# weixiaopassking/GS-LIVM

Hardware: AMD Instinct MI355X
Metric: rasterizer fwd+bwd Mpixels/s @1920x1080, 2000000 Gaussians (ms_per_step = ms/frame) (higher is better)
Workload: dtype f32; 1 GPU; C3: 2000000 Gaussians, 1920x1080, SH degree 0, 1 view per GPU per step, fwd+bwd + Adam step; view_threads=1, camera=one fixed view, near_entries=0, parallelism=view-parallel x1, adam_in_step=True, optimizer=one-kernel tail: activation chain rule + Adam + next activations (HIP), loss=seeded

## Files before the change

### gs-livm_amd/_capi.py

```python
import ctypes as C
import os

import torch

_HERE = os.path.dirname(os.path.abspath(__file__))
LIB_PATH = os.environ.get("GSR_LIB", os.path.join(_HERE, "libgsraster_hip.so"))

ALLOC_FN = C.CFUNCTYPE(C.c_void_p, C.c_void_p, C.c_size_t)


class GeometryView(C.Structure):
    _fields_ = [(n, C.c_void_p) for n in
                ("depths", "radii", "splats", "cov3D", "tiles_touched", "point_offsets", "clamped", "depth_order",
                 "num_rendered", "gpack")]


class BinningView(C.Structure):
    _fields_ = [("point_list", C.c_void_p)]


class ImageView(C.Structure):
    _fields_ = [(n, C.c_void_p) for n in ("ranges", "final_T", "n_contrib", "quad_last", "ranges_far")]


class MailboxEvent(C.Structure):
    _fields_ = [("count", C.c_uint), ("ticket_expected", C.c_uint32), ("ticket_seen_before_query", C.c_uint32),
                ("elapsed_us", C.c_double), ("ticket_seen_after_query", C.c_uint32), ("first_query_result", C.c_int),
                ("visible_at_query", C.c_int), ("queries", C.c_uint), ("longest_query_us", C.c_double),
                ("longest_poll_gap_us", C.c_double)]


class NumRendered(int):

    def __new__(cls, exact, key):
        obj = super().__new__(cls, exact)
        obj.key = int(key)
        return obj


def _key(R):
    return int(getattr(R, "key", R))


_lib = None

EXPORTS = ("gsr_forward", "gsr_backward", "gsr_backward_depth", "gsr_mark_visible", "gsr_geometry_bytes", "gsr_image_bytes",
           "gsr_binning_bytes", "gsr_geometry_view_of", "gsr_binning_view_of", "gsr_image_view_of",
           "gsr_higher_msb", "gsr_last_error", "gsr_abi_version", "gsr_kernel_count", "gsr_kernel_name",
           "gsr_profile_enable", "gsr_profile_enable_only", "gsr_profile_read", "gsr_mailbox_slow_path_hits", "gsr_activate", "gsr_activate_backward", "gsr_adam_step",
           "gsr_photometric_loss", "gsr_photometric_loss_workspace", "gsr_init_gaussians", "gsr_ply_row_floats",
           "gsr_pack_ply_rows", "gsr_model_step", "gsr_set_reference_rects", "gsr_reference_rects",
           "gsr_last_num_rendered", "gsr_set_binning_capacity_hint", "gsr_speculative_forwards",
           "gsr_speculation_overflows", "gsr_emit_guard_trips", "gsr_mailbox_slow_path_last", "gsr_set_near_far", "gsr_near_far",
           "gsr_last_near_far", "gsr_set_near_far_hints", "gsr_near_far_forwards", "gsr_set_far_speculation",
           "gsr_last_far_skipped", "gsr_far_skips", "gsr_far_skip_misses", "gsr_async_far_frames",
           "gsr_near_budget_scale", "gsr_near_budget_feedback", "gsr_near_far_pause", "gsr_set_near_far_thread",
           "gsr_set_reference_rects_thread", "gsr_async_outcomes_pending", "gsr_async_outcomes_lost",
           "gsr_frame_note_misses", "gsr_similarity_loss", "gsr_similarity_loss_workspace")


def lib():
    global _lib
    if _lib is not None:
        return _lib
    if not os.path.exists(LIB_PATH):
        raise RuntimeError(
            "libgsraster_hip.so not built: run `python gs-livm_amd/build.py` (needs hipcc). "
            "gs_livm_amd has no CPU fallback.")
    L = C.CDLL(LIB_PATH)
    vp, ci, cf, sz = C.c_void_p, C.c_int, C.c_float, C.c_size_t
    L.gsr_forward.restype = ci
    L.gsr_forward.argtypes = [ALLOC_FN, vp, ALLOC_FN, vp, ALLOC_FN, vp, ci, ci, ci, vp, ci, ci, vp, vp, vp, vp, vp, cf,
                              vp, vp, vp, vp, vp, cf, cf, ci, vp, vp, vp, vp, ci, vp]
    L.gsr_backward.restype = ci
    L.gsr_backward.argtypes = [ci, ci, ci, ci, vp, ci, ci, vp, vp, vp, vp, cf, vp, vp, vp, vp, vp, cf, cf, vp, vp, vp,
                               vp, vp, vp, vp, vp, vp, vp, vp, vp, vp, vp, vp, ci, vp]
    L.gsr_backward_depth.restype = ci
    L.gsr_backward_depth.argtypes = L.gsr_backward.argtypes[:25] + [vp] + L.gsr_backward.argtypes[25:34] + [vp, ci, vp]
    L.gsr_mark_visible.restype = ci
    L.gsr_mark_visible.argtypes = [ci, vp, vp, vp, vp, vp]
    for n in ("gsr_geometry_bytes", "gsr_binning_bytes"):
        getattr(L, n).restype = sz
        getattr(L, n).argtypes = [ci]
    L.gsr_image_bytes.restype = sz
    L.gsr_image_bytes.argtypes = [ci, ci]
    L.gsr_geometry_view_of.argtypes = [vp, ci, C.POINTER(GeometryView)]
    L.gsr_binning_view_of.argtypes = [vp, ci, C.POINTER(BinningView)]
    L.gsr_image_view_of.argtypes = [vp, ci, ci, C.POINTER(ImageView)]
    L.gsr_higher_msb.restype = C.c_uint32
    L.gsr_higher_msb.argtypes = [C.c_uint32]
    L.gsr_last_error.restype = C.c_char_p
    L.gsr_abi_version.restype = ci
    L.gsr_kernel_count.restype = ci
    L.gsr_kernel_name.restype = C.c_char_p
    L.gsr_kernel_name.argtypes = [ci]
    L.gsr_profile_enable.argtypes = [ci]
    L.gsr_profile_enable_only.argtypes = [C.POINTER(ci), ci]
    L.gsr_set_reference_rects.restype = ci
    L.gsr_set_reference_rects.argtypes = [ci]
    L.gsr_reference_rects.restype = ci
    L.gsr_reference_rects.argtypes = []
    L.gsr_last_num_rendered.restype = ci
    L.gsr_last_num_rendered.argtypes = []
    L.gsr_set_binning_capacity_hint.restype = C.c_longlong
    L.gsr_set_binning_capacity_hint.argtypes = [C.c_longlong]
    for n in ("gsr_speculative_forwards", "gsr_speculation_overflows", "gsr_emit_guard_trips"):
        getattr(L, n).restype = C.c_ulonglong
        getattr(L, n).argtypes = []
    L.gsr_set_near_far.restype = ci
    L.gsr_set_near_far.argtypes = [ci]
    L.gsr_near_far.restype = ci
    L.gsr_near_far.argtypes = []
    L.gsr_last_near_far.restype = ci
    L.gsr_last_near_far.argtypes = [C.POINTER(C.c_uint), C.POINTER(C.c_uint)]
    L.gsr_set_near_far_hints.restype = None
    L.gsr_set_near_far_hints.argtypes = [C.c_longlong, C.c_longlong]
    L.gsr_near_far_forwards.restype = C.c_ulonglong
    L.gsr_near_far_forwards.argtypes = []
    L.gsr_set_far_speculation.restype = ci
    L.gsr_set_far_speculation.argtypes = [ci]
    L.gsr_last_far_skipped.restype = ci
    L.gsr_last_far_skipped.argtypes = []
    L.gsr_near_budget_scale.restype = C.c_uint
    L.gsr_near_budget_scale.argtypes = []
    L.gsr_near_budget_feedback.restype = C.c_uint
    L.gsr_near_budget_feedback.argtypes = [C.c_uint, C.c_uint, C.c_uint]
    L.gsr_near_far_pause.restype = ci
    L.gsr_near_far_pause.argtypes = [ci]
    for n in ("gsr_far_skips", "gsr_far_skip_misses", "gsr_async_far_frames", "gsr_async_outcomes_lost",
              "gsr_frame_note_misses", "gsr_similarity_loss", "gsr_similarity_loss_workspace"):
        getattr(L, n).restype = C.c_ulonglong
        getattr(L, n).argtypes = []
    for n in ("gsr_set_near_far_thread", "gsr_set_reference_rects_thread"):
        getattr(L, n).restype = ci
        getattr(L, n).argtypes = [ci]
    L.gsr_async_outcomes_pending.restype = ci
    L.gsr_async_outcomes_pending.argtypes = []
    L.gsr_mailbox_slow_path_last.restype = ci
    L.gsr_mailbox_slow_path_last.argtypes = [C.POINTER(MailboxEvent)]
    L.gsr_mailbox_slow_path_hits.restype = C.c_ulonglong
    L.gsr_mailbox_slow_path_hits.argtypes = []
    L.gsr_profile_read.restype = ci
    L.gsr_profile_read.argtypes = [ci, C.POINTER(C.c_double), C.POINTER(ci)]
    L.gsr_activate.restype = ci
    L.gsr_activate.argtypes = [ci, ci] + [vp] * 9 + [vp]
    L.gsr_activate_backward.restype = ci
    L.gsr_activate_backward.argtypes = [ci, ci] + [vp] * 12 + [vp]
    L.gsr_photometric_loss_workspace.restype = sz
    L.gsr_photometric_loss_workspace.argtypes = [ci, ci, ci]
    L.gsr_photometric_loss.restype = ci
    L.gsr_photometric_loss.argtypes = [ci, ci, ci, vp, vp, C.POINTER(cf), cf, vp, vp, vp, sz, vp]
    L.gsr_similarity_loss_workspace.restype = sz
    L.gsr_similarity_loss_workspace.argtypes = [ci, ci]
    L.gsr_similarity_loss.restype = ci
    L.gsr_similarity_loss.argtypes = [ci, ci, ci, vp, vp, vp, vp, cf, vp, vp, vp, ci, vp, sz, vp]
    L.gsr_init_gaussians.restype = ci
    L.gsr_init_gaussians.argtypes = [ci, ci, vp, vp, vp, cf] + [vp] * 6 + [vp]
    L.gsr_ply_row_floats.restype = sz
    L.gsr_ply_row_floats.argtypes = [ci]
    L.gsr_pack_ply_rows.restype = ci
    L.gsr_pack_ply_rows.argtypes = [ci, ci] + [vp] * 7 + [vp]
    L.gsr_model_step.restype = ci
    L.gsr_model_step.argtypes = [ci, ci, C.POINTER(vp), C.POINTER(vp), C.POINTER(vp)] + [vp] * 9 + \
        [C.POINTER(cf), C.c_double, C.c_double, C.c_double, ci, vp]
    L.gsr_adam_step.restype = ci
    L.gsr_adam_step.argtypes = [ci, C.POINTER(vp), C.POINTER(vp), C.POINTER(vp), C.POINTER(vp), C.POINTER(sz),
                                C.POINTER(cf), C.c_double, C.c_double, C.c_double, ci, ci, vp]
    _lib = L
    return L


class GsrError(RuntimeError):
    pass


def _check(code):
    if code < 0:
        raise GsrError("libgsraster_hip error %d: %s" % (code, lib().gsr_last_error().decode()))
    return code


def _ptr(t):
    if t is None or t.numel() == 0:
        return None
    assert t.is_cuda and t.is_contiguous(), "expects contiguous device tensors"
    return C.c_void_p(t.data_ptr())


def _stream():
    return C.c_void_p(torch.cuda.current_stream().cuda_stream)


class _Blob:

    def __init__(self, device):
        self.device = device
        self.tensor = torch.empty(0, dtype=torch.uint8, device=device)
        self.fn = ALLOC_FN(self._alloc)

    def _alloc(self, _ctx, nbytes):
        try:
            self.tensor = torch.empty(int(nbytes), dtype=torch.uint8, device=self.device)
            return self.tensor.data_ptr()
        except Exception:
            return None


def rasterize_forward(background, means3D, colors, opacity, scales, rotations, scale_modifier, cov3D_precomp,
                      viewmatrix, projmatrix, tan_fovx, tan_fovy, image_height, image_width, sh, degree, campos,
                      prefiltered=False, debug=False, radii_out=True):
    if means3D.dim() != 2 or means3D.size(1) != 3:
        raise ValueError("means3D must have dimensions (num_points, 3)")
    dev = means3D.device
    P, H, W = int(means3D.size(0)), int(image_height), int(image_width)
    f32 = dict(dtype=torch.float32, device=dev)
    out_color = torch.empty((3, H, W), **f32)
    out_depth = torch.empty((1, H, W), **f32)
    out_acc = torch.empty((1, H, W), **f32)
    radii = torch.empty((P,), dtype=torch.int32, device=dev)
    gb, bb, ib = _Blob(dev), _Blob(dev), _Blob(dev)
    M = int(sh.size(1)) if (sh is not None and sh.numel() != 0) else 0
    L = lib()
    R = _check(L.gsr_forward(gb.fn, None, bb.fn, None, ib.fn, None, P, int(degree), M, _ptr(background), W, H,
                             _ptr(means3D), _ptr(sh), _ptr(colors), _ptr(opacity), _ptr(scales),
                             float(scale_modifier), _ptr(rotations), _ptr(cov3D_precomp), _ptr(viewmatrix),
                             _ptr(projmatrix), _ptr(campos), float(tan_fovx), float(tan_fovy), int(bool(prefiltered)),
                             _ptr(out_color), _ptr(out_depth), _ptr(out_acc), _ptr(radii) if radii_out else None,
                             int(bool(debug)), _stream()))
    R = NumRendered(L.gsr_last_num_rendered() if P else 0, R)
    return R, out_color, out_depth, out_acc, radii, gb.tensor, bb.tensor, ib.tensor


def rasterize_backward(background, means3D, radii, colors, scales, rotations, scale_modifier, cov3D_precomp,
                       viewmatrix, projmatrix, tan_fovx, tan_fovy, dL_dout_color, dL_dout_acc, sh, degree, campos,
                       geomBuffer, R, binningBuffer, imageBuffer, debug=False, return_conic=False, want_cov3D=True,
                       grad_depth=None):
    dev = means3D.device
    P = int(means3D.size(0))
    H, W = int(dL_dout_color.size(1)), int(dL_dout_color.size(2))
    M = int(sh.size(1)) if (sh is not None and sh.numel() != 0) else 0
    f32 = dict(dtype=torch.float32, device=dev)
    mk = torch.zeros if P == 0 else torch.empty
    dL_dmeans3D = mk((P, 3), **f32)
    dL_dmeans2D = mk((P, 3), **f32)
    dL_dcolors = mk((P, 3), **f32)
    dL_dconic = mk((P, 2, 2), **f32)
    dL_dopacity = mk((P, 1), **f32)
    dL_dcov3D = mk((P, 6), **f32) if want_cov3D else None
    dL_dsh = mk((P, M, 3), **f32)
    dL_dscales = mk((P, 3), **f32)
    dL_drotations = mk((P, 4), **f32)
    dL_ddepths = mk((P,), **f32) if grad_depth is not None else None
    if P != 0 and grad_depth is not None:
        dpix = dL_dout_color.contiguous()
        dacc = dL_dout_acc.contiguous()
        if grad_depth.dtype != torch.float32 or grad_depth.device != dev or grad_depth.numel() != H * W:
            raise ValueError("grad_depth must be a float32 tensor of H*W elements on the device of means3D")
        ddep = grad_depth.contiguous()
        _check(lib().gsr_backward_depth(P, int(degree), M, _key(R), _ptr(background), W, H, _ptr(means3D), _ptr(sh),
                                        _ptr(colors), _ptr(scales), float(scale_modifier), _ptr(rotations),
                                        _ptr(cov3D_precomp), _ptr(viewmatrix), _ptr(projmatrix), _ptr(campos),
                                        float(tan_fovx), float(tan_fovy), _ptr(radii), _ptr(geomBuffer),
                                        _ptr(binningBuffer), _ptr(imageBuffer), _ptr(dpix), _ptr(dacc), _ptr(ddep),
                                        _ptr(dL_dmeans2D), _ptr(dL_dconic), _ptr(dL_dopacity), _ptr(dL_dcolors),
                                        _ptr(dL_dmeans3D), _ptr(dL_dcov3D), _ptr(dL_dsh), _ptr(dL_dscales),
                                        _ptr(dL_drotations), _ptr(dL_ddepths), int(bool(debug)), _stream()))
    elif P != 0:
        dpix = dL_dout_color.contiguous()
        dacc = dL_dout_acc.contiguous()
        _check(lib().gsr_backward(P, int(degree), M, _key(R), _ptr(background), W, H, _ptr(means3D), _ptr(sh),
                                  _ptr(colors), _ptr(scales), float(scale_modifier), _ptr(rotations),
                                  _ptr(cov3D_precomp), _ptr(viewmatrix), _ptr(projmatrix), _ptr(campos),
                                  float(tan_fovx), float(tan_fovy), _ptr(radii), _ptr(geomBuffer),
                                  _ptr(binningBuffer), _ptr(imageBuffer), _ptr(dpix), _ptr(dacc), _ptr(dL_dmeans2D),
                                  _ptr(dL_dconic), _ptr(dL_dopacity), _ptr(dL_dcolors), _ptr(dL_dmeans3D),
                                  _ptr(dL_dcov3D), _ptr(dL_dsh), _ptr(dL_dscales), _ptr(dL_drotations),
                                  int(bool(debug)), _stream()))
    out = (dL_dmeans2D, dL_dcolors, dL_dopacity, dL_dmeans3D, dL_dcov3D, dL_dsh, dL_dscales, dL_drotations)
    if return_conic:
        out = out + (dL_dconic,)
    return out + (dL_ddepths,) if grad_depth is not None else out


def last_num_rendered():
    return int(lib().gsr_last_num_rendered())


def set_binning_capacity_hint(capacity):
    return int(lib().gsr_set_binning_capacity_hint(-1 if capacity is None else int(capacity)))


def speculation_stats():
    L = lib()
    return dict(speculative_forwards=int(L.gsr_speculative_forwards()), overflows=int(L.gsr_speculation_overflows()),
                near_far_forwards=int(L.gsr_near_far_forwards()), far_skips=int(L.gsr_far_skips()),
                far_skip_misses=int(L.gsr_far_skip_misses()), async_far_frames=int(L.gsr_async_far_frames()),
                async_outcomes_lost=int(L.gsr_async_outcomes_lost()), frame_note_misses=int(L.gsr_frame_note_misses()),
                near_budget_scale_q8=int(L.gsr_near_budget_scale()),
                mailbox_slow_path_hits=int(L.gsr_mailbox_slow_path_hits()))


def emit_guard_trips():
    return int(lib().gsr_emit_guard_trips())


def mailbox_slow_path_last():
    ev = MailboxEvent()
    _check(lib().gsr_mailbox_slow_path_last(C.byref(ev)))
    return {n: getattr(ev, n) for n, _ in MailboxEvent._fields_}


def set_near_far(on):
    return bool(lib().gsr_set_near_far(int(bool(on))))


def set_near_far_thread(mode):
    prev = int(lib().gsr_set_near_far_thread(-1 if mode is None else int(bool(mode))))
    return None if prev < 0 else bool(prev)


def async_outcomes_pending():
    return int(lib().gsr_async_outcomes_pending())


def set_near_far_hints(near_entries_per_tile=None, far_capacity=None):
    lib().gsr_set_near_far_hints(-1 if near_entries_per_tile is None else int(near_entries_per_tile),
                                 -1 if far_capacity is None else int(far_capacity))


def set_far_speculation(mode):
    return int(lib().gsr_set_far_speculation(-1 if mode is None else int(bool(mode))))


def last_far_skipped():
    return bool(lib().gsr_last_far_skipped())


def last_near_far():
    a, b = C.c_uint(0), C.c_uint(0)
    split = bool(lib().gsr_last_near_far(C.byref(a), C.byref(b)))
    return split, int(a.value), int(b.value)


def set_reference_rects(on):
    return bool(lib().gsr_set_reference_rects(int(bool(on))))


def set_reference_rects_thread(mode):
    prev = int(lib().gsr_set_reference_rects_thread(-1 if mode is None else int(bool(mode))))
    return None if prev < 0 else bool(prev)


def reference_rects():
    return bool(lib().gsr_reference_rects())


def mark_visible(means3D, viewmatrix, projmatrix):
    P = int(means3D.size(0))
    present = torch.zeros((P,), dtype=torch.bool, device=means3D.device)
    if P:
        _check(lib().gsr_mark_visible(P, _ptr(means3D), _ptr(viewmatrix), _ptr(projmatrix),
                                      C.c_void_p(present.data_ptr()), _stream()))
    return present


def _sub(blob, ptr, count, dtype):
    if not ptr or count == 0:
        return None
    off = int(ptr) - blob.data_ptr()
    nbytes = count * torch.empty((), dtype=dtype).element_size()
    return blob[off:off + nbytes].view(dtype)


def state_views(geomBuffer, binningBuffer, imageBuffer, P, R, W, H):
    L = lib()
    gv, bv, iv = GeometryView(), BinningView(), ImageView()
    T = ((W + 15) // 16) * ((H + 15) // 16)
    out = {}
    if P:
        _check(L.gsr_geometry_view_of(_ptr(geomBuffer), P, C.byref(gv)))
        splats = _sub(geomBuffer, gv.splats, P * 12, torch.float32).view(P, 12)
        gpack = _sub(geomBuffer, gv.gpack, P * 2, torch.int32).view(P, 2)
        out.update(depths=splats[:, 9],
                   radii=_sub(geomBuffer, gv.radii, P, torch.int32),
                   splats=splats,
                   cov3D=_sub(geomBuffer, gv.cov3D, P * 6, torch.float32).view(P, 6),
                   tiles_touched=gpack[:, 0],
                   point_offsets=_sub(geomBuffer, gv.point_offsets, P, torch.int32),
                   clamped=_sub(geomBuffer, gv.clamped, P, torch.uint8),
                   depth_order=_sub(geomBuffer, gv.depth_order, P, torch.int32))
        _check(L.gsr_image_view_of(_ptr(imageBuffer), W, H, C.byref(iv)))
        out.update(ranges=_sub(imageBuffer, iv.ranges, T * 2, torch.int32).view(T, 2),
                   final_T=_sub(imageBuffer, iv.final_T, W * H, torch.float32).view(H, W),
                   n_contrib=_sub(imageBuffer, iv.n_contrib, W * H, torch.int32).view(H, W),
                   quad_last=_sub(imageBuffer, iv.quad_last, T * 4, torch.int32).view(T, 4))
        counters = _sub(geomBuffer, gv.num_rendered, 16, torch.int32).cpu().tolist()
        split = counters[12] == 1
        exact = counters[6] + counters[8] if split else counters[0]
        out.update(num_rendered=exact, near_far=split, counters=counters)
        key = _key(R)
        if exact:
            _check(L.gsr_binning_view_of(_ptr(binningBuffer), key, C.byref(bv)))
            raw = _sub(binningBuffer, bv.point_list, key, torch.int32)
            ra = out["ranges"].long()
            rb = _sub(imageBuffer, iv.ranges_far, T * 2, torch.int32).view(T, 2).long()
            seg_start = torch.stack([ra[:, 0], rb[:, 0]], 1).reshape(-1)
            seg_len = torch.stack([ra[:, 1] - ra[:, 0], rb[:, 1] - rb[:, 0]], 1).reshape(-1)
            total = int(seg_len.sum())
            excl = torch.cumsum(seg_len, 0) - seg_len
            idx = torch.repeat_interleave(seg_start - excl, seg_len) + torch.arange(total, device=ra.device)
            point_list = raw[idx]
            ln = seg_len.view(T, 2).sum(1)
            ends = torch.cumsum(ln, 0)
            ranges = torch.stack([ends - ln, ends], 1)
            ranges[ln == 0] = 0
            out.update(ranges_near=out["ranges"], ranges_far=rb.int(), ranges=ranges.int())
            tile_ids = torch.repeat_interleave(torch.arange(T, device=ra.device), ln)
            dbits = out["depths"].view(torch.int32)[point_list.long()].long() & 0xFFFFFFFF
            out.update(tile_ids=tile_ids, point_list=point_list, keys=(tile_ids.long() << 32) | dbits)
    return out


def profile_enable(on=True, only=None):
    L = lib()
    if on and only is not None:
        names = [L.gsr_kernel_name(i).decode() for i in range(L.gsr_kernel_count())]
        ids = [names.index(k) for k in only]
        _check(L.gsr_profile_enable_only((C.c_int * len(ids))(*ids), len(ids)))
    else:
        _check(L.gsr_profile_enable(int(bool(on))))


def profile_read():
    L = lib()
    n = L.gsr_kernel_count()
    ms = (C.c_double * n)()
    cnt = (C.c_int * n)()
    _check(L.gsr_profile_read(n, ms, cnt))
    return {L.gsr_kernel_name(i).decode(): (float(ms[i]), int(cnt[i])) for i in range(n)}


def activate(scaling_raw, rotation_raw, opacity_raw, features_dc, features_rest):
    P = int(scaling_raw.size(0))
    M = 1 + (int(features_rest.size(1)) if features_rest is not None and features_rest.numel() else 0)
    f32 = dict(dtype=torch.float32, device=scaling_raw.device)
    scales, rot = torch.empty((P, 3), **f32), torch.empty((P, 4), **f32)
    opac, shs = torch.empty((P, 1), **f32), torch.empty((P, M, 3), **f32)
    _check(lib().gsr_activate(P, M, _ptr(scaling_raw), _ptr(rotation_raw), _ptr(opacity_raw), _ptr(features_dc),
                              _ptr(features_rest), _ptr(scales), _ptr(rot), _ptr(opac), _ptr(shs), _stream()))
    return scales, rot, opac, shs


def activate_backward(rotation_raw, scales, opacities, g_scales, g_rot, g_opac, g_shs):
    P, M = int(scales.size(0)), int(g_shs.size(1))
    f32 = dict(dtype=torch.float32, device=scales.device)
    gs, gr, go = torch.empty((P, 3), **f32), torch.empty((P, 4), **f32), torch.empty((P, 1), **f32)
    gdc, grest = torch.empty((P, 1, 3), **f32), torch.empty((P, M - 1, 3), **f32)
    _check(lib().gsr_activate_backward(P, M, _ptr(rotation_raw), _ptr(scales), _ptr(opacities), _ptr(g_scales),
                                       _ptr(g_rot), _ptr(g_opac), _ptr(g_shs), _ptr(gs), _ptr(gr), _ptr(go),
                                       _ptr(gdc), _ptr(grest), _stream()))
    return gs, gr, go, gdc, grest


def adam_step(params, grads, exp_avg, exp_avg_sq, lrs, beta1, beta2, eps, step, zero_grads=True):
    n = len(params)
    VP = C.c_void_p * n
    arr = lambda ts: VP(*[t.data_ptr() if t.numel() else None for t in ts])
    numel = (C.c_size_t * n)(*[int(t.numel()) for t in params])
    lr = (C.c_float * n)(*[float(x) for x in lrs])
    for t in list(params) + list(grads) + list(exp_avg) + list(exp_avg_sq):
        assert t.is_cuda and t.is_contiguous() and t.dtype == torch.float32
    _check(lib().gsr_adam_step(n, arr(params), arr(grads), arr(exp_avg), arr(exp_avg_sq), numel, lr, float(beta1),
                               float(beta2), float(eps), int(step), int(bool(zero_grads)), _stream()))


def photometric_loss(img, gt, window11, lambda_dssim, want_grad=True):
    assert img.dim() == 3 and img.shape == gt.shape and img.is_cuda
    Cn, H, W = (int(x) for x in img.shape)
    img, gt = img.contiguous(), gt.contiguous()
    nbytes = int(lib().gsr_photometric_loss_workspace(Cn, H, W))
    ws = torch.empty(nbytes, dtype=torch.uint8, device=img.device)
    out3 = torch.empty(3, dtype=torch.float32, device=img.device)
    grad = torch.empty_like(img) if want_grad else None
    win = (C.c_float * 11)(*[float(x) for x in window11])
    _check(lib().gsr_photometric_loss(Cn, H, W, _ptr(img), _ptr(gt), win, float(lambda_dssim), _ptr(out3), _ptr(grad),
                                      _ptr(ws), nbytes, _stream()))
    return out3, grad


def similarity_loss(points, sel, xyz, scaling, lambda_, grad_xyz=None, grad_scaling=None, accumulate=False):
    P, m, n = int(xyz.size(0)), int(points.size(0)), int(sel.size(0))
    assert xyz.is_cuda and xyz.shape == (P, 3) and scaling.shape == (P, 3) and points.shape == (m, 3)
    assert sel.dtype == torch.int32 and sel.dim() == 1
    for t in (points, xyz, scaling, grad_xyz, grad_scaling):
        assert t is None or (t.is_cuda and t.is_contiguous() and t.dtype == torch.float32)
    assert sel.is_cuda and sel.is_contiguous()
    for g in (grad_xyz, grad_scaling):
        assert g is None or g.shape == (P, 3)
    nbytes = int(lib().gsr_similarity_loss_workspace(m, n))
    ws = torch.empty(max(nbytes, 1), dtype=torch.uint8, device=xyz.device)
    out3 = torch.empty(3, dtype=torch.float32, device=xyz.device)
    _check(lib().gsr_similarity_loss(P, m, n, _ptr(points), _ptr(sel), _ptr(xyz), _ptr(scaling), float(lambda_),
                                     _ptr(out3), _ptr(grad_xyz), _ptr(grad_scaling), int(bool(accumulate)), _ptr(ws),
                                     nbytes, _stream()))
    return out3


def init_gaussians(xyz, covs, rgbs, scale_factor, out_xyz, out_features_dc, out_features_rest, out_scaling,
                   out_rotation, out_opacity):
    n = int(xyz.size(0))
    M = 1 + (int(out_features_rest.size(1)) if out_features_rest is not None and out_features_rest.numel() else 0)
    for t in (xyz, covs, rgbs, out_xyz, out_features_dc, out_scaling, out_rotation, out_opacity):
        assert t.is_cuda and t.is_contiguous() and t.dtype == torch.float32
    assert covs.shape == (n, 3, 3) and rgbs.shape == (n, 3)
    _check(lib().gsr_init_gaussians(n, M, _ptr(xyz), _ptr(covs), _ptr(rgbs), float(scale_factor), _ptr(out_xyz),
                                    _ptr(out_features_dc), _ptr(out_features_rest), _ptr(out_scaling),
                                    _ptr(out_rotation), _ptr(out_opacity), _stream()))


def pack_ply_rows(xyz, features_dc, features_rest, opacity, scaling, rotation):
    P = int(xyz.size(0))
    M = 1 + (int(features_rest.size(1)) if features_rest is not None and features_rest.numel() else 0)
    rf = int(lib().gsr_ply_row_floats(M))
    rows = torch.empty((P, rf), dtype=torch.float32, device=xyz.device)
    args = [t.contiguous() for t in (xyz, features_dc, features_rest, opacity, scaling, rotation)]
    _check(lib().gsr_pack_ply_rows(P, M, *[_ptr(t) for t in args], _ptr(rows), _stream()))
    return rows


def model_step(params6, exp_avg6, exp_avg_sq6, g_xyz, g_scales, g_rot, g_opac, g_shs, lrs6, beta1, beta2, eps, step,
               want_activated=True):
    xyz, fdc, frest = params6[0], params6[1], params6[2]
    P = int(xyz.size(0))
    M = 1 + (int(frest.size(1)) if frest.numel() else 0)
    for t in list(params6) + list(exp_avg6) + list(exp_avg_sq6) + [g_xyz, g_scales, g_rot, g_opac, g_shs]:
        assert t.is_cuda and t.is_contiguous() and t.dtype == torch.float32
    outs = None
    if want_activated:
        f32 = dict(dtype=torch.float32, device=xyz.device)
        outs = (torch.empty((P, 3), **f32), torch.empty((P, 4), **f32), torch.empty((P, 1), **f32),
                torch.empty((P, M, 3), **f32))
    VP = C.c_void_p * 6
    arr = lambda ts: VP(*[t.data_ptr() if t.numel() else None for t in ts])
    lr = (C.c_float * 6)(*[float(x) for x in lrs6])
    o = outs if outs is not None else (None, None, None, None)
    _check(lib().gsr_model_step(P, M, arr(params6), arr(exp_avg6), arr(exp_avg_sq6), _ptr(g_xyz), _ptr(g_scales),
                                _ptr(g_rot), _ptr(g_opac), _ptr(g_shs), _ptr(o[0]), _ptr(o[1]), _ptr(o[2]), _ptr(o[3]), lr,
                                float(beta1), float(beta2), float(eps), int(step), _stream()))
    return outs
# ... 1 lines not shown
```

### gs-livm_amd/csrc/api.hip

```cpp
#include "../../include/gsraster.h"

#include <algorithm>
#include <atomic>
#include <mutex>
#include <cstdarg>
#include <cstdio>
#include <cstdlib>
#include <cstring>
#include <chrono>
#include <unordered_map>
#include <vector>

#include "gsr_internal.hpp"

using namespace gsr;

static thread_local char g_err[512] = "";

static int fail(int code, const char* fmt, ...) {
  va_list ap;
  va_start(ap, fmt);
  vsnprintf(g_err, sizeof(g_err), fmt, ap);
  va_end(ap);
  return code;
// ... 862 lines not shown
    capB = (uint32_t)c.far_hint_override;
    c.far_hint_override = -1;
  } else if (f.h.have_far) {
    capB = f.h.recent_far.max();
    capB = (uint32_t)std::min<unsigned long long>(0x7fffffffull - capA, (unsigned long long)capB * 3 / 2 + 131072);
    capB = std::min(round_capacity(capB), 0x7fffffffu - capA);
  } else {
    capB = behind;
  }
  const bool lazy_cap = async_far && !capB_forced;
  const uint32_t far_expect = std::max<uint32_t>(capB, 1u << 20);
  if (lazy_cap) capB = std::max(capB, behind);
  if (capB < 4096u) capB = 4096u;
  if ((unsigned long long)capA + capB > 0x7fffffffull) capB = 0x7fffffffu - capA;
  r->key = (int)(capA + capB);
  BinningState b;
  int rc;
  if ((rc = carve_binning(f, r->key, &b)) != GSR_OK) return rc;
  AsyncWords aw;
  if (async_far) {
    if (c.async_seq >= 0x3FFFFFF0u) {
      HIP_TRY(hipStreamSynchronize(stream));
      HIP_TRY(hipStreamSynchronize(c.far_stream));
      HIP_TRY(hipMemset(c.sig_decide, 0, 8));
      HIP_TRY(hipMemset(c.sig_go, 0, 8));
      HIP_TRY(hipMemset(c.done_counter + 2, 0, 8));
      c.async_seq = 0;
    }
    aw.decide = c.sig_decide;
    aw.go = c.sig_go;
    aw.gate_dev = reinterpret_cast<uint32_t*>(c.done_counter + 2);
    aw.seq = ++c.async_seq;
  }
  if (lazy_cap) {
    c.w_live = 16 + 2 * (int)(++c.lazy_seq & 7u);
    c.w_far = c.w_live + 1;
  }
  if ((rc = enqueue_chain(f, b, Chain{1, Count{g.total + 6, (int)capA}, budget, 0u}, stream, aw)) != GSR_OK) return rc;
  Chain far_chain{2, Count{g.total + 8, (int)capB}, 0xFFFFFFFFu, capA, far_expect};
  far_chain.cnt.bounded = lazy_cap;
  uint32_t live = 0;
  c.last_far_skipped = false;
  if (async_far) {
    far_chain.cnt.gate = aw.gate_dev;
    far_chain.cnt.gate_open = 2u * aw.seq + 1u;
    HIP_TRY(launch_decide_far(g.total + 13, aw, stream));
    HIP_TRY(hipStreamWaitValue32(c.far_stream, c.sig_decide, 2u * aw.seq, hipStreamWaitValueGte));
    t_prof_suppress = true;
    rc = enqueue_chain(f, b, far_chain, c.far_stream);
    t_prof_suppress = false;
    if (rc != GSR_OK) return rc;
    HIP_TRY(launch_release_go(far_chain.cnt, c.sig_go, aw.seq, c.far_stream));
    HIP_TRY(hipStreamWaitValue32(stream, c.sig_go, aw.seq, hipStreamWaitValueGte));
    HIP_TRY(launch_tile_order(f.fp, f.im, stream));
    order_remember(f.iblob);
    ++g_async_frames;
  } else if (skip_far) {
    if (launch_tile_order(f.fp, f.im, stream) != hipSuccess) return fail(GSR_ERR_HIP, "k_tile_order launch failed");
  } else {
    if ((rc = enqueue_chain(f, b, far_chain, stream)) != GSR_OK) return rc;
  }
  const std::chrono::steady_clock::time_point tw = std::chrono::steady_clock::now();
  if ((rc = wait_num_rendered(c, stream, &r->R)) != GSR_OK) return rc;
  if ((rc = wait_num_rendered(c, stream, &r->near, 2)) != GSR_OK) return rc;
  bool know_far = true;
  if (lazy_cap && (unsigned long long)r->R - r->near <= (unsigned long long)capB) {
    know_far = false;
    lazy_push(c, c.ticket, r->near, r->R, async_far);
  } else {
    if ((rc = wait_num_rendered(c, stream, &live, c.w_live)) != GSR_OK) return rc;
    if (p.speculate_far && live == 0u) {
      if (skip_far) order_remember(f.iblob);
    } else {
      if (skip_far && (rc = enqueue_chain(f, b, far_chain, stream)) != GSR_OK) return rc;
      if ((rc = wait_num_rendered(c, stream, &r->far, c.w_far)) != GSR_OK) return rc;
    }
    record_far_outcome(c, &f.h, live, r->near, r->far, r->R, p.speculate_far, true);
  }
  if (env().host_trace)
    fprintf(stderr, "[gsr] near/far forward: capacity %u + %u, near %u, far %u of %u instances, %u unfinished quads%s, "
                    "enqueue %.1f us, then waited %.1f us\n", capA, capB, r->near, r->far, r->R, live,
            async_far ? (know_far ? " (asynchronous far chain, checked by the host)" : " (asynchronous far chain)")
            : skip_far ? (live ? " (far chain enqueued late)" : " (far chain not enqueued)")
            : "",
            std::chrono::duration<double, std::micro>(tw - f.t_enq).count(),
            std::chrono::duration<double, std::micro>(std::chrono::steady_clock::now() - tw).count());
  ++g_speculative_forwards;
  ++g_near_far_forwards;
  c.last_was_near_far = true;
  r->redo = r->far > capB;
  if (!r->redo) frame_note(f.iblob, NOTE_SPLIT);
  return GSR_OK;
}

static int redo_frame(const Forward& f, FrameResult* r) {
  GeomState& g = f.g;
  const hipStream_t stream = f.stream;
  ++g_speculation_overflows;
  order_forget(f.iblob);
  const size_t nscan = ((size_t)f.fp.P + SCAN_TILE - 1) / SCAN_TILE;
  HIP_TRY(hipMemsetAsync(g.dsort.tickets() + 4, 0, 2 * sizeof(uint32_t), stream));
  HIP_TRY(hipMemsetAsync(g.dsort.scan_status(), 0, sizeof(unsigned long long) * 2 * nscan, stream));
  HIP_TRY(hipMemsetAsync(g.total + 11, 0, sizeof(uint32_t), stream));
  const int rc = enqueue_exact(f, r->R, false);
  if (rc != GSR_OK) return rc;
  f.c.last_was_near_far = false;
  r->key = (int)r->R;
  r->near = r->R;
  r->far = 0;
  return GSR_OK;
}

int gsr_forward(gsr_alloc_fn geometry_alloc, void* geometry_ctx, gsr_alloc_fn binning_alloc, void* binning_ctx,
                gsr_alloc_fn image_alloc, void* image_ctx, int P, int D, int M, const float* background, int width,
                int height, const float* means3D, const float* shs, const float* colors_precomp,
                const float* opacities, const float* scales, float scale_modifier, const float* rotations,
                const float* cov3D_precomp, const float* viewmatrix, const float* projmatrix, const float* cam_pos,
                float tan_fovx, float tan_fovy, int prefiltered, float* out_color, float* out_depth, float* out_acc,
                int* radii, int debug, void* stream_) {
  (void)prefiltered;
  hipStream_t stream = (hipStream_t)stream_;
  g_err[0] = 0;
  if (P < 0 || width <= 0 || height <= 0) return fail(GSR_ERR_INVALID_ARGUMENT, "bad P/width/height");
  if (!out_color || !out_depth || !out_acc) return fail(GSR_ERR_INVALID_ARGUMENT, "null output image");
  const size_t N = (size_t)width * height;
  if (P == 0) {
    HIP_TRY(hipMemsetAsync(out_color, 0, 3 * N * sizeof(float), stream));
    HIP_TRY(hipMemsetAsync(out_depth, 0, N * sizeof(float), stream));
    HIP_TRY(hipMemsetAsync(out_acc, 0, N * sizeof(float), stream));
    g_ctx.last_R = 0;
    return 0;
  }
  if (!geometry_alloc || !binning_alloc || !image_alloc) return fail(GSR_ERR_INVALID_ARGUMENT, "null allocator");
  if (!means3D || !opacities || !background || !viewmatrix || !projmatrix || !cam_pos)
    return fail(GSR_ERR_INVALID_ARGUMENT, "null required input");
  if (!colors_precomp && !shs)
    return fail(GSR_ERR_INVALID_ARGUMENT, "provide SHs or precomputed colours");
  if (!cov3D_precomp && (!scales || !rotations))
    return fail(GSR_ERR_INVALID_ARGUMENT, "provide scales+rotations or a precomputed 3D covariance");
  if (!colors_precomp && (D < 0 || D > 3 || M < (D + 1) * (D + 1) || M > 16))
    return fail(GSR_ERR_UNSUPPORTED, "SH degree %d with %d coefficients is not supported (D<=3, (D+1)^2<=M<=16)", D, M);
  if (width > 1023 * TILE || height > 1023 * TILE) return fail(GSR_ERR_UNSUPPORTED, "image larger than 16368 px");
  if (P >= (1 << 30)) return fail(GSR_ERR_UNSUPPORTED, "2^30 or more Gaussians");
  if (!(tan_fovx > 0.f) || !(tan_fovy > 0.f)) return fail(GSR_ERR_INVALID_ARGUMENT, "tan_fov must be > 0");

  const FrameParams fp = make_params(P, D, M, width, height, tan_fovx, tan_fovy, scale_modifier);
  char* gblob = geometry_alloc(geometry_ctx, gsr_geometry_bytes(P));
  if (!gblob) return fail(GSR_ERR_ALLOC, "geometry allocator returned NULL");
  char* iblob = image_alloc(image_ctx, gsr_image_bytes(width, height));
  if (!iblob) return fail(GSR_ERR_ALLOC, "image allocator returned NULL");
  GeomState g = GeomState::carve(gblob, (size_t)P);
  ImageState im = ImageState::carve(iblob, width, height);
  order_forget(iblob);

  ThreadCtx& c = g_ctx;
  const bool multi_thread = several_threads_render(&c);
  lazy_resolve(c);
  c.w_live = 3;
  c.w_far = 1;
  if (c.near_count_pending) {
    uint32_t nn = 0;
    ViewHist& hv = c.views[c.near_count_view];
    if (peek_word(c, 4, c.near_count_ticket, &nn) && hv.generation == c.near_count_gen)
      hv.near_list_too_long = (unsigned long long)nn * 3ull > (unsigned long long)P;
    c.near_count_pending = false;
  }
  ViewHist& h = view_hist(c, viewmatrix, width, height);
  int rc = ctx_prepare(c, stream);
  if (rc != GSR_OK) return rc;
  const bool own_hist_pass = env().depth_hist_pass || !preprocess_counts_depth_digits(fp, shs, colors_precomp);
  uint32_t* const ghist2 = reinterpret_cast<uint32_t*>(reinterpret_cast<char*>(c.done_counter) + 64);
  if (!own_hist_pass) c.hist_flip ^= 1u;
  uint32_t* const ghist_acc = own_hist_pass ? nullptr : ghist2 + 1280 * c.hist_flip;
  uint32_t* const ghist_clear = own_hist_pass ? nullptr : ghist2 + 1280 * (c.hist_flip ^ 1u);
  STAGE(launch_preprocess(fp, means3D, scales, rotations, opacities, shs, cov3D_precomp, colors_precomp, viewmatrix,
                          projmatrix, cam_pos, g, radii, debug != 0, c.done_counter, c.mailbox_dev, c.ticket,
                          ghist_acc, ghist_clear, stream));
  c.top_hist = ghist_acc ? ghist_acc + 3 * 256 : nullptr;
  if (debug) STAGE(launch_point_offsets(fp, g, stream));

  const FramePlan plan = plan_frame(c, h, fp, debug);
  Forward f{fp, g, im, c, h, DepthOrder{}, background, out_color, out_depth, out_acc, debug, stream, iblob,
            binning_alloc, binning_ctx, std::chrono::steady_clock::now()};
  c.last_was_near_far = false;
  if ((rc = enqueue_depth_order(f, plan, ghist_acc)) != GSR_OK) return rc;
  FrameResult r;
  rc = !plan.speculate ? sync_frame(f, &r)
       : plan.near_far ? near_far_frame(f, plan, multi_thread, &r)
                       : one_chain_frame(f, plan.hint, &r);
  if (rc != GSR_OK) return rc;
  if (r.R > 0x7fffffffu) return fail(GSR_ERR_UNSUPPORTED, "more than 2^31 splat instances");
  if (r.redo && (rc = redo_frame(f, &r)) != GSR_OK) return rc;
  c.last_near = r.near;
  c.last_far = r.far;
  if (env().host_trace)
    fprintf(stderr, "[gsr] forward returns at %.1f us (process clock)\n",
            std::chrono::duration<double, std::micro>(std::chrono::steady_clock::now().time_since_epoch()).count());
  frame_note(iblob, NOTE_PRESENT);
  h.recent.push(r.R);
  c.last_R = c.last_near + c.last_far;
  return r.key;
}

int gsr_last_num_rendered(void) {
  lazy_resolve(g_ctx);
  return (int)g_ctx.last_R;
}
int gsr_set_near_far(int on) { return near_far_flag().exchange(on != 0 ? 1 : 0); }
int gsr_set_near_far_thread(int mode) {
  const int prev = t_near_far;
  t_near_far = mode < 0 ? -1 : (mode ? 1 : 0);
  return prev;
}
int gsr_near_far(void) { return t_near_far >= 0 ? t_near_far : near_far_flag().load(); }
int gsr_last_near_far(unsigned* near_instances, unsigned* far_instances) {
  lazy_resolve(g_ctx);
  if (near_instances) *near_instances = g_ctx.last_near;
  if (far_instances) *far_instances = g_ctx.last_far;
  return g_ctx.last_was_near_far ? 1 : 0;
}
void gsr_set_near_far_hints(long long near_entries_per_tile, long long far_capacity) {
  g_ctx.near_entries_override = near_entries_per_tile < 0 ? -1 : near_entries_per_tile;
  g_ctx.far_hint_override = far_capacity < 0 ? -1 : (far_capacity > 0x7fffffffll ? 0x7fffffffll : far_capacity);
  if (far_capacity < 0)
    for (auto& v : g_ctx.views) v.have_far = false;
}
unsigned long long gsr_near_far_forwards(void) { return g_near_far_forwards.load(); }
int gsr_set_far_speculation(int mode) {
  const int prev = g_ctx.far_skip_override;
  g_ctx.far_skip_override = mode < 0 ? -1 : (mode ? 1 : 0);
  if (mode < 0)
    for (auto& v : g_ctx.views) v.far_idle_streak = 0;
  return prev;
}
int gsr_last_far_skipped(void) {
  lazy_resolve(g_ctx);
  return g_ctx.last_far_skipped ? 1 : 0;
}
unsigned long long gsr_async_far_frames(void) { return g_async_frames.load(); }
unsigned gsr_near_budget_scale(void) {
  lazy_resolve(g_ctx);
  return g_ctx.views[g_ctx.cur].near_scale_q8;
}
unsigned gsr_near_budget_feedback(unsigned unfinished_quads, unsigned near_instances, unsigned far_instances) {
  budget_feedback(g_ctx, g_ctx.views[g_ctx.cur], unfinished_quads, near_instances, far_instances);
  return g_ctx.views[g_ctx.cur].near_scale_q8;
}
int gsr_near_far_pause(int frames) {
  const int prev = g_ctx.views[g_ctx.cur].split_pause;
  if (frames >= 0) g_ctx.views[g_ctx.cur].split_pause = frames;
  return prev;
}
unsigned long long gsr_far_skips(void) { return g_far_skips.load(); }
unsigned long long gsr_far_skip_misses(void) { return g_far_skip_misses.load(); }
long long gsr_set_binning_capacity_hint(long long capacity) {
  const long long prev = g_ctx.hint_override;
  g_ctx.hint_override = capacity < 0 ? -1 : (capacity > 0x7fffffffll ? 0x7fffffffll : capacity);
  if (capacity == 0)
    for (auto& v : g_ctx.views) v.recent.clear();
  return prev;
}
unsigned long long gsr_speculative_forwards(void) { return g_speculative_forwards.load(); }
unsigned long long gsr_speculation_overflows(void) { return g_speculation_overflows.load(); }
unsigned long long gsr_emit_guard_trips(void) { return emit_guard_trips(); }
int gsr_mailbox_slow_path_last(gsr_mailbox_event* out) {
  if (!out) return fail(GSR_ERR_INVALID_ARGUMENT, "null pointer");
  std::lock_guard<std::mutex> lk(g_slow_mu);
  *out = g_slow_last;
  return GSR_OK;
}

int gsr_set_reference_rects(int on) { return reference_rects_flag().exchange(on != 0 ? 1 : 0); }
int gsr_reference_rects(void) { return t_reference_rects >= 0 ? t_reference_rects : reference_rects_flag().load(); }
int gsr_set_reference_rects_thread(int mode) {
  const int prev = t_reference_rects;
  t_reference_rects = mode < 0 ? -1 : (mode ? 1 : 0);
  return prev;
}
unsigned long long gsr_frame_note_misses(void) { return g_note_misses.load(); }
unsigned long long gsr_async_outcomes_lost(void) { return g_async_outcomes_lost.load(); }
int gsr_async_outcomes_pending(void) {
  lazy_resolve(g_ctx);
  return g_ctx.pending_n;
}

unsigned long long gsr_mailbox_slow_path_hits(void) { return g_mailbox_slow_hits.load(); }

static int backward_impl(bool with_depth, int P, int D, int M, int R, const float* background, int width, int height,
                         const float* means3D, const float* shs, const float* colors_precomp, const float* scales,
                         float scale_modifier, const float* rotations, const float* cov3D_precomp,
                         const float* viewmatrix, const float* projmatrix, const float* campos, float tan_fovx,
                         float tan_fovy, const int* radii, char* geom_buffer, char* binning_buffer, char* image_buffer,
                         const float* dL_dpix, const float* dL_dacc, const float* dL_ddepth, float* dL_dmean2D,
                         float* dL_dconic, float* dL_dopacity, float* dL_dcolor, float* dL_dmean3D, float* dL_dcov3D,
                         float* dL_dsh, float* dL_dscale, float* dL_drot, float* dL_ddepths, int debug,
                         void* stream_) {
  hipStream_t stream = (hipStream_t)stream_;
  g_err[0] = 0;
  if (P < 0 || R < 0 || width <= 0 || height <= 0) return fail(GSR_ERR_INVALID_ARGUMENT, "bad P/R/width/height");
  if (P == 0) return GSR_OK;
  if (!geom_buffer || !binning_buffer || !image_buffer) return fail(GSR_ERR_INVALID_ARGUMENT, "null state blob");
  if (!means3D || !background || !viewmatrix || !projmatrix || !campos || !dL_dpix || !dL_dacc)
    return fail(GSR_ERR_INVALID_ARGUMENT, "null required input");
  if (!dL_dmean2D || !dL_dconic || !dL_dopacity || !dL_dcolor || !dL_dmean3D || (!dL_dcov3D && cov3D_precomp) ||
      !dL_dscale || !dL_drot || (M > 0 && !dL_dsh))
    return fail(GSR_ERR_INVALID_ARGUMENT, "null gradient output");
  if (with_depth && !dL_ddepth) return fail(GSR_ERR_INVALID_ARGUMENT, "null dL_ddepth");
  if (with_depth && !dL_ddepths) return fail(GSR_ERR_INVALID_ARGUMENT, "null dL_ddepths");
  if (env().host_trace)
    fprintf(stderr, "[gsr] backward entered at %.1f us (process clock)\n",
            std::chrono::duration<double, std::micro>(std::chrono::steady_clock::now().time_since_epoch()).count());
  const FrameParams fp = make_params(P, D, M, width, height, tan_fovx, tan_fovy, scale_modifier);
  GeomState g = GeomState::carve(geom_buffer, (size_t)P);
  BinningState b = BinningState::carve(binning_buffer, (size_t)R);
  ImageState im = ImageState::carve(image_buffer, width, height);
  if (!radii) radii = g.radii;

  if (R > 0) {
    const unsigned notes = frame_notes(image_buffer);
    STAGE(launch_blend_backward(fp, g, b, im, background, dL_dpix, dL_dacc, dL_ddepth, (notes & NOTE_ORDER) != 0u,
                                stream));
    STAGE(launch_gather_records(fp, g, b, dL_dmean2D, dL_dconic, dL_dopacity, dL_dcolor, dL_ddepths,
                                (notes & NOTE_SPLIT) != 0u, stream));
  }
  STAGE(launch_gaussian_backward(fp, g, b, radii, means3D, scales, rotations, colors_precomp ? nullptr : shs,
                                 cov3D_precomp, viewmatrix, projmatrix, campos, colors_precomp != nullptr, dL_dmean2D,
                                 dL_dconic, dL_dopacity, dL_dcolor, dL_dmean3D, dL_dcov3D, dL_dsh, dL_dscale, dL_drot,
                                 dL_ddepths, stream));
  return GSR_OK;
}

int gsr_backward(int P, int D, int M, int R, const float* background, int width, int height, const float* means3D,
                 const float* shs, const float* colors_precomp, const float* scales, float scale_modifier,
                 const float* rotations, const float* cov3D_precomp, const float* viewmatrix,
                 const float* projmatrix, const float* campos, float tan_fovx, float tan_fovy, const int* radii,
                 char* geom_buffer, char* binning_buffer, char* image_buffer, const float* dL_dpix,
                 const float* dL_dacc, float* dL_dmean2D, float* dL_dconic, float* dL_dopacity, float* dL_dcolor,
                 float* dL_dmean3D, float* dL_dcov3D, float* dL_dsh, float* dL_dscale, float* dL_drot, int debug,
                 void* stream_) {
  return backward_impl(false, P, D, M, R, background, width, height, means3D, shs, colors_precomp, scales,
                       scale_modifier, rotations, cov3D_precomp, viewmatrix, projmatrix, campos, tan_fovx, tan_fovy, radii,
                       geom_buffer, binning_buffer, image_buffer, dL_dpix, dL_dacc, nullptr, dL_dmean2D, dL_dconic,
                       dL_dopacity, dL_dcolor, dL_dmean3D, dL_dcov3D, dL_dsh, dL_dscale, dL_drot, nullptr, debug, stream_);
}

int gsr_backward_depth(int P, int D, int M, int R, const float* background, int width, int height,
                       const float* means3D, const float* shs, const float* colors_precomp, const float* scales,
                       float scale_modifier, const float* rotations, const float* cov3D_precomp,
                       const float* viewmatrix, const float* projmatrix, const float* campos, float tan_fovx,
                       float tan_fovy, const int* radii, char* geom_buffer, char* binning_buffer, char* image_buffer,
                       const float* dL_dpix, const float* dL_dacc, const float* dL_ddepth, float* dL_dmean2D,
                       float* dL_dconic, float* dL_dopacity, float* dL_dcolor, float* dL_dmean3D, float* dL_dcov3D,
                       float* dL_dsh, float* dL_dscale, float* dL_drot, float* dL_ddepths, int debug, void* stream_) {
  return backward_impl(true, P, D, M, R, background, width, height, means3D, shs, colors_precomp, scales, scale_modifier,
                       rotations, cov3D_precomp, viewmatrix, projmatrix, campos, tan_fovx, tan_fovy, radii, geom_buffer,
                       binning_buffer, image_buffer, dL_dpix, dL_dacc, dL_ddepth, dL_dmean2D, dL_dconic, dL_dopacity,
                       dL_dcolor, dL_dmean3D, dL_dcov3D, dL_dsh, dL_dscale, dL_drot, dL_ddepths, debug, stream_);
}

int gsr_mark_visible(int P, const float* means3D, const float* viewmatrix, const float* projmatrix,
                     unsigned char* present, void* stream_) {
  (void)projmatrix;
  g_err[0] = 0;
  if (P < 0) return fail(GSR_ERR_INVALID_ARGUMENT, "bad P");
  if (P == 0) return GSR_OK;
  if (!means3D || !viewmatrix || !present) return fail(GSR_ERR_INVALID_ARGUMENT, "null pointer");
  HIP_TRY(launch_mark_visible(P, means3D, viewmatrix, present, (hipStream_t)stream_));
  return GSR_OK;
}

int gsr_activate(int P, int M, const float* scaling_raw, const float* rotation_raw, const float* opacity_raw,
                 const float* features_dc, const float* features_rest, float* scales, float* rotations,
                 float* opacities, float* shs, void* stream_) {
  g_err[0] = 0;
  if (P < 0 || M < 1 || M > 16) return fail(GSR_ERR_INVALID_ARGUMENT, "bad P/M");
  if (P == 0) return GSR_OK;
  if (!scaling_raw || !rotation_raw || !opacity_raw || !features_dc || (M > 1 && !features_rest) || !scales ||
      !rotations || !opacities || !shs)
    return fail(GSR_ERR_INVALID_ARGUMENT, "null pointer");
  HIP_TRY(launch_activate(P, M, scaling_raw, rotation_raw, opacity_raw, features_dc, features_rest, scales, rotations,
                          opacities, shs, (hipStream_t)stream_));
  return GSR_OK;
}

int gsr_activate_backward(int P, int M, const float* rotation_raw, const float* scales, const float* opacities,
                          const float* dL_dscales, const float* dL_drotations, const float* dL_dopacities,
                          const float* dL_dshs, float* dL_dscaling_raw, float* dL_drotation_raw,
                          float* dL_dopacity_raw, float* dL_dfeatures_dc, float* dL_dfeatures_rest, void* stream_) {
  g_err[0] = 0;
  if (P < 0 || M < 1 || M > 16) return fail(GSR_ERR_INVALID_ARGUMENT, "bad P/M");
  if (P == 0) return GSR_OK;
  if (!rotation_raw || !scales || !opacities || !dL_dscales || !dL_drotations || !dL_dopacities || !dL_dshs ||
      !dL_dscaling_raw || !dL_drotation_raw || !dL_dopacity_raw || !dL_dfeatures_dc || (M > 1 && !dL_dfeatures_rest))
    return fail(GSR_ERR_INVALID_ARGUMENT, "null pointer");
  HIP_TRY(launch_activate_backward(P, M, rotation_raw, scales, opacities, dL_dscales, dL_drotations, dL_dopacities,
                                   dL_dshs, dL_dscaling_raw, dL_drotation_raw, dL_dopacity_raw, dL_dfeatures_dc,
                                   dL_dfeatures_rest, (hipStream_t)stream_));
  return GSR_OK;
}

int gsr_adam_step(int n_tensors, float* const* params, float* const* grads, float* const* exp_avg,
                  float* const* exp_avg_sq, const size_t* numel, const float* lr, double beta1, double beta2, double eps,
                  int step, int zero_grads, void* stream_) {
  g_err[0] = 0;
  if (n_tensors < 0 || n_tensors > 8) return fail(GSR_ERR_INVALID_ARGUMENT, "1..8 tensors per call");
  if (step < 1) return fail(GSR_ERR_INVALID_ARGUMENT, "step counts from 1");
  if (n_tensors == 0) return GSR_OK;
  if (!params || !grads || !exp_avg || !exp_avg_sq || !numel || !lr) return fail(GSR_ERR_INVALID_ARGUMENT, "null array");
  for (int k = 0; k < n_tensors; k++)
    if (numel[k] && (!params[k] || !grads[k] || !exp_avg[k] || !exp_avg_sq[k]))
      return fail(GSR_ERR_INVALID_ARGUMENT, "null tensor pointer");
  HIP_TRY(launch_adam(n_tensors, params, grads, exp_avg, exp_avg_sq, numel, lr, beta1, beta2, eps, step, zero_grads,
                      (hipStream_t)stream_));
  return GSR_OK;
}

size_t gsr_photometric_loss_workspace(int channels, int height, int width) {
  if (channels <= 0 || height <= 0 || width <= 0) return 0;
  return loss_workspace_bytes(channels, height, width);
}

int gsr_photometric_loss(int channels, int height, int width, const float* img, const float* gt,
                         const float* window11_host, float lambda_dssim, float* loss_out3, float* dL_dimg,
                         char* workspace, size_t workspace_bytes, void* stream_) {
  g_err[0] = 0;
  if (channels <= 0 || height <= 0 || width <= 0) return fail(GSR_ERR_INVALID_ARGUMENT, "bad image shape");
  if ((unsigned long long)height * (unsigned long long)width >= 0x7fffffffull)
    return fail(GSR_ERR_INVALID_ARGUMENT, "image plane too large");
  if (!img || !gt || !window11_host || !loss_out3 || !workspace) return fail(GSR_ERR_INVALID_ARGUMENT, "null pointer");
  if (workspace_bytes < loss_workspace_bytes(channels, height, width))
    return fail(GSR_ERR_INVALID_ARGUMENT, "workspace too small: need %zu bytes",
                loss_workspace_bytes(channels, height, width));
  HIP_TRY(launch_photometric_loss(channels, height, width, img, gt, window11_host, lambda_dssim, loss_out3, dL_dimg,
                                  workspace, (hipStream_t)stream_));
  return GSR_OK;
}

size_t gsr_similarity_loss_workspace(int m, int n) {
  if (m <= 0 || n <= 0 || n > 0x7fffffff - 1024) return 0;
  return simi_workspace_bytes(m, n);
}

int gsr_similarity_loss(int P, int m, int n, const float* points, const int* sel, const float* xyz,
                        const float* scaling, float lambda, float* out3, float* grad_xyz, float* grad_scaling,
                        int accumulate, char* workspace, size_t workspace_bytes, void* stream_) {
  g_err[0] = 0;
  if (P < 0 || m < 0 || n < 0) return fail(GSR_ERR_INVALID_ARGUMENT, "bad P/m/n");
  if (n > P) return fail(GSR_ERR_INVALID_ARGUMENT, "n = %d selected rows of P = %d (the selection is unique)", n, P);
  if (n > 0x7fffffff - 1024) return fail(GSR_ERR_INVALID_ARGUMENT, "n too large");
  if (!out3) return fail(GSR_ERR_INVALID_ARGUMENT, "null pointer");
  if (m > 0 && n > 0) {
    if (!points || !sel || !xyz || !scaling || !workspace) return fail(GSR_ERR_INVALID_ARGUMENT, "null pointer");
    if (workspace_bytes < simi_workspace_bytes(m, n))
      return fail(GSR_ERR_INVALID_ARGUMENT, "workspace too small: need %zu bytes", simi_workspace_bytes(m, n));
  }
  HIP_TRY(launch_similarity_loss(P, m, n, points, sel, xyz, scaling, lambda, out3, grad_xyz, grad_scaling,
                                 accumulate ? 1 : 0, workspace, (hipStream_t)stream_));
  return GSR_OK;
}

int gsr_model_step(int P, int M, float* const* params6, float* const* exp_avg6, float* const* exp_avg_sq6,
                   const float* dL_dxyz, const float* dL_dscales, const float* dL_drotations, const float* dL_dopacities,
                   const float* dL_dshs, float* scales_out, float* rotations_out, float* opacities_out, float* shs_out,
                   const float* lr6, double beta1, double beta2, double eps, int step, void* stream_) {
  g_err[0] = 0;
  if (P < 0 || M < 1 || M > 16) return fail(GSR_ERR_INVALID_ARGUMENT, "bad P/M");
  if (step < 1) return fail(GSR_ERR_INVALID_ARGUMENT, "step counts from 1");
  if (P == 0) return GSR_OK;
  if (!params6 || !exp_avg6 || !exp_avg_sq6 || !lr6 || !dL_dxyz || !dL_dscales || !dL_drotations || !dL_dopacities ||
      !dL_dshs)
    return fail(GSR_ERR_INVALID_ARGUMENT, "null pointer");
  for (int k = 0; k < 6; k++)
    if ((k != 2 || M > 1) && (!params6[k] || !exp_avg6[k] || !exp_avg_sq6[k]))
      return fail(GSR_ERR_INVALID_ARGUMENT, "null tensor pointer (group %d)", k);
  HIP_TRY(launch_model_step(P, M, params6, exp_avg6, exp_avg_sq6, dL_dxyz, dL_dscales, dL_drotations, dL_dopacities,
                            dL_dshs, scales_out, rotations_out, opacities_out, shs_out, lr6, beta1, beta2, eps, step,
                            (hipStream_t)stream_));
  return GSR_OK;
}

int gsr_init_gaussians(int n, int M, const float* xyz, const float* covs, const float* rgbs, float scale_factor,
                       float* xyz_out, float* features_dc_out, float* features_rest_out, float* scaling_out,
                       float* rotation_out, float* opacity_out, void* stream_) {
  g_err[0] = 0;
  if (n < 0 || M < 1 || M > 16) return fail(GSR_ERR_INVALID_ARGUMENT, "bad n/M");
  if (n == 0) return GSR_OK;
  if (!xyz || !covs || !rgbs || !xyz_out || !features_dc_out || (M > 1 && !features_rest_out) || !scaling_out ||
      !rotation_out || !opacity_out)
    return fail(GSR_ERR_INVALID_ARGUMENT, "null pointer");
  HIP_TRY(launch_init_gaussians(n, M, xyz, covs, rgbs, scale_factor, xyz_out, features_dc_out, features_rest_out,
                                scaling_out, rotation_out, opacity_out, (hipStream_t)stream_));
  return GSR_OK;
}

size_t gsr_ply_row_floats(int M) { return M >= 1 ? (size_t)(14 + 3 * M) : 0; }

int gsr_pack_ply_rows(int P, int M, const float* xyz, const float* features_dc, const float* features_rest,
                      const float* opacity, const float* scaling, const float* rotation, float* rows, void* stream_) {
  g_err[0] = 0;
  if (P < 0 || M < 1 || M > 16) return fail(GSR_ERR_INVALID_ARGUMENT, "bad P/M");
  if (P == 0) return GSR_OK;
  if (!xyz || !features_dc || (M > 1 && !features_rest) || !opacity || !scaling || !rotation || !rows)
    return fail(GSR_ERR_INVALID_ARGUMENT, "null pointer");
  HIP_TRY(launch_pack_ply_rows(P, M, xyz, features_dc, features_rest, opacity, scaling, rotation, rows,
                               (hipStream_t)stream_));
  return GSR_OK;
}

int gsr_geometry_view_of(char* geom_buffer, int P, gsr_geometry_view* out) {
  if (!geom_buffer || !out || P < 0) return fail(GSR_ERR_INVALID_ARGUMENT, "bad argument");
  GeomState g = GeomState::carve(geom_buffer, (size_t)P);
  out->depths = nullptr;
  out->radii = g.radii;
  out->splats = reinterpret_cast<const float*>(g.splats);
  out->cov3D = g.cov3D;
  out->tiles_touched = nullptr;
  out->gpack = reinterpret_cast<const uint32_t*>(g.gpack);
  out->point_offsets = g.point_offsets;
  out->clamped = g.clamped;
  out->depth_order = g.order;
  out->num_rendered = g.total;
  return GSR_OK;
}

int gsr_binning_view_of(char* binning_buffer, int R, gsr_binning_view* out) {
  if (!binning_buffer || !out || R < 0) return fail(GSR_ERR_INVALID_ARGUMENT, "bad argument");
  BinningState b = BinningState::carve(binning_buffer, (size_t)R);
  out->point_list = b.point_list;
  return GSR_OK;
}

int gsr_image_view_of(char* image_buffer, int width, int height, gsr_image_view* out) {
  if (!image_buffer || !out || width <= 0 || height <= 0) return fail(GSR_ERR_INVALID_ARGUMENT, "bad argument");
  ImageState im = ImageState::carve(image_buffer, width, height);
  out->ranges = reinterpret_cast<const uint32_t*>(im.ranges);
  out->final_T = im.final_T;
  out->n_contrib = im.n_contrib;
  out->quad_last = im.quad_last;
  out->ranges_far = reinterpret_cast<const uint32_t*>(im.rangesB);
  return GSR_OK;
}

}
```

### gs-livm_amd/csrc/preprocess.hip

```cpp

#include "gsr_internal.hpp"
#include "sort_core.hpp"

namespace gsr {

__device__ __forceinline__ float fmin_(float a, float b) { return fminf(a, b); }
__device__ __forceinline__ float fmax_(float a, float b) { return fmaxf(a, b); }

__device__ __forceinline__ float ndc_to_pix(float v, int S) {
  return (float)((((double)v + 1.0) * (double)S - 1.0) * 0.5);
}

__device__ __forceinline__ uint32_t wave_sum_u32(uint32_t v) {
#pragma unroll
  for (int o = 32; o > 0; o >>= 1) v += __shfl_xor(v, o, 64);
  return v;
}

__device__ __forceinline__ unsigned long long wave_sum_u64(unsigned long long v) {
#pragma unroll
  for (int o = 32; o > 0; o >>= 1) v += __shfl_xor(v, o, 64);
  return v;
}

__device__ __forceinline__ uint32_t wave_incl_scan_u32(uint32_t v, int lane) {
#pragma unroll
  for (int o = 1; o < 64; o <<= 1) {
    uint32_t t = __shfl_up(v, o, 64);
    if (lane >= o) v += t;
  }
  return v;
}

constexpr float SH0 = 0.28209479177387814f;
constexpr float SH1 = 0.4886025119029199f;
__device__ const float SH2c[5] = {1.0925484305920792f, -1.0925484305920792f, 0.31539156525252005f,
                                  -1.0925484305920792f, 0.5462742152960396f};
__device__ const float SH3c[7] = {-0.5900435899266435f, 2.890611442640554f, -0.4570457994644658f, 0.3731763325901154f,
                                  -0.4570457994644658f, 1.445305721320277f,  -0.5900435899266435f};

__device__ __forceinline__ void cov3d_from_scale_rot(const float s0, const float s1, const float s2, const float4 q,
                                                     float* c6) {
  const float r = q.x, x = q.y, y = q.z, z = q.w;
  const float R00 = 1.f - 2.f * (y * y + z * z), R01 = 2.f * (x * y - r * z), R02 = 2.f * (x * z + r * y);
  const float R10 = 2.f * (x * y + r * z), R11 = 1.f - 2.f * (x * x + z * z), R12 = 2.f * (y * z - r * x);
  const float R20 = 2.f * (x * z - r * y), R21 = 2.f * (y * z + r * x), R22 = 1.f - 2.f * (x * x + y * y);
  const float M00 = s0 * R00, M01 = s1 * R01, M02 = s2 * R02;
  const float M10 = s0 * R10, M11 = s1 * R11, M12 = s2 * R12;
  const float M20 = s0 * R20, M21 = s1 * R21, M22 = s2 * R22;
  c6[0] = M00 * M00 + M01 * M01 + M02 * M02;
  c6[1] = M10 * M00 + M11 * M01 + M12 * M02;
  c6[2] = M20 * M00 + M21 * M01 + M22 * M02;
  c6[3] = M10 * M10 + M11 * M11 + M12 * M12;
  c6[4] = M20 * M10 + M21 * M11 + M22 * M12;
  c6[5] = M20 * M20 + M21 * M21 + M22 * M22;
}

struct Ewa {
  float T00, T01, T02, T10, T11, T12;
  float tx, ty, tz, txtz, tytz;
  float cxx, cxy, cyy;
};

__device__ __forceinline__ Ewa ewa_project(const float mx, const float my, const float mz, const FrameParams& fp,
                                           const float* __restrict__ c6, const float* __restrict__ V) {
  Ewa e;
  float t0 = V[0] * mx + V[4] * my + V[8] * mz + V[12];
  float t1 = V[1] * mx + V[5] * my + V[9] * mz + V[13];
  const float t2 = V[2] * mx + V[6] * my + V[10] * mz + V[14];
  const float limx = 1.3f * fp.tan_fovx, limy = 1.3f * fp.tan_fovy;
  e.txtz = t0 / t2;
  e.tytz = t1 / t2;
  t0 = fmin_(limx, fmax_(-limx, e.txtz)) * t2;
  t1 = fmin_(limy, fmax_(-limy, e.tytz)) * t2;
  e.tx = t0; e.ty = t1; e.tz = t2;
  const float J00 = fp.focal_x / t2, J02 = -(fp.focal_x * t0) / (t2 * t2);
  const float J11 = fp.focal_y / t2, J12 = -(fp.focal_y * t1) / (t2 * t2);
  e.T00 = V[0] * J00 + V[2] * J02;
  e.T01 = V[4] * J00 + V[6] * J02;
  e.T02 = V[8] * J00 + V[10] * J02;
  e.T10 = V[1] * J11 + V[2] * J12;
  e.T11 = V[5] * J11 + V[6] * J12;
  e.T12 = V[9] * J11 + V[10] * J12;
  const float S00 = c6[0], S01 = c6[1], S02 = c6[2], S11 = c6[3], S12 = c6[4], S22 = c6[5];
  const float A00 = e.T00 * S00 + e.T01 * S01 + e.T02 * S02;
  const float A10 = e.T00 * S01 + e.T01 * S11 + e.T02 * S12;
  const float A20 = e.T00 * S02 + e.T01 * S12 + e.T02 * S22;
  const float A01 = e.T10 * S00 + e.T11 * S01 + e.T12 * S02;
  const float A11 = e.T10 * S01 + e.T11 * S11 + e.T12 * S12;
  const float A21 = e.T10 * S02 + e.T11 * S12 + e.T12 * S22;
  e.cxx = A00 * e.T00 + A10 * e.T01 + A20 * e.T02;
  e.cxy = A01 * e.T00 + A11 * e.T01 + A21 * e.T02;
  e.cyy = A01 * e.T10 + A11 * e.T11 + A21 * e.T12;
  return e;
}

__device__ __forceinline__ int sh_row_stride(int C) { return C | 1; }

__device__ __forceinline__ void rows_to_lds(float* lds, const float* __restrict__ src, const int nrows, const int C) {
  const int n = nrows * C, S = sh_row_stride(C);
  if ((C & 3) == 0 && (reinterpret_cast<uintptr_t>(src) & 15u) == 0) {
    const int C4 = C >> 2, n4 = n >> 2;
    const int dr = PRE_BLOCK / C4, dc = PRE_BLOCK - dr * C4;
    int r = (int)threadIdx.x / C4, c4 = (int)threadIdx.x - r * C4;
    for (int j = threadIdx.x; j < n4; j += PRE_BLOCK) {
      const float4 v = reinterpret_cast<const float4*>(src)[j];
      float* d = lds + r * S + 4 * c4;
      d[0] = v.x; d[1] = v.y; d[2] = v.z; d[3] = v.w;
      r += dr; c4 += dc;
      if (c4 >= C4) { c4 -= C4; r++; }
    }
  } else {
    const int dr = PRE_BLOCK / C, dc = PRE_BLOCK - dr * C;
    int r = (int)threadIdx.x / C, c = (int)threadIdx.x - r * C;
    for (int e = threadIdx.x; e < n; e += PRE_BLOCK) {
      lds[r * S + c] = src[e];
      r += dr; c += dc;
      if (c >= C) { c -= C; r++; }
    }
  }
}

__device__ __forceinline__ void lds_to_rows(float* __restrict__ dst, const float* lds, const int nrows, const int C) {
  const int n = nrows * C, S = sh_row_stride(C);
  if ((C & 3) == 0 && (reinterpret_cast<uintptr_t>(dst) & 15u) == 0) {
    const int C4 = C >> 2, n4 = n >> 2;
    const int dr = PRE_BLOCK / C4, dc = PRE_BLOCK - dr * C4;
    int r = (int)threadIdx.x / C4, c4 = (int)threadIdx.x - r * C4;
    for (int j = threadIdx.x; j < n4; j += PRE_BLOCK) {
      const float* d = lds + r * S + 4 * c4;
      reinterpret_cast<float4*>(dst)[j] = make_float4(d[0], d[1], d[2], d[3]);
      r += dr; c4 += dc;
      if (c4 >= C4) { c4 -= C4; r++; }
    }
  } else {
    const int dr = PRE_BLOCK / C, dc = PRE_BLOCK - dr * C;
    int r = (int)threadIdx.x / C, c = (int)threadIdx.x - r * C;
    for (int e = threadIdx.x; e < n; e += PRE_BLOCK) {
      dst[e] = lds[r * S + c];
      r += dr; c += dc;
      if (c >= C) { c -= C; r++; }
    }
  }
}

__device__ __forceinline__ void listed_rows_to_lds(float* lds, const float* __restrict__ src, const uint32_t* list,
                                                   const int nlist, const int C) {
  const int S = sh_row_stride(C);
  if ((C & 3) == 0 && (reinterpret_cast<uintptr_t>(src) & 15u) == 0) {
    const int C4 = C >> 2;
    for (int k = threadIdx.x; k < nlist * C4; k += PRE_BLOCK) {
      const int r = (int)list[k / C4], c4 = k % C4;
      const float4 v = reinterpret_cast<const float4*>(src + (size_t)r * C)[c4];
      float* d = lds + r * S + 4 * c4;
      d[0] = v.x; d[1] = v.y; d[2] = v.z; d[3] = v.w;
    }
  } else {
    for (int k = threadIdx.x; k < nlist * C; k += PRE_BLOCK) {
      const int r = (int)list[k / C], c = k % C;
      lds[r * S + c] = src[(size_t)r * C + c];
    }
  }
}

static inline size_t sh_stage_bytes(int M) {
  if (M <= 1) return 0;
  const size_t b = (size_t)PRE_BLOCK * (size_t)((3 * M) | 1) * sizeof(float);
  return b <= 64 * 1024 ? b : 0;
}

template <bool STAGED, bool PLAIN = false, bool PIN = PLAIN, int ROWK = 0>
__global__ __launch_bounds__(PRE_BLOCK) void k_preprocess(
    const FrameParams fp, const float* __restrict__ means3D, const float* __restrict__ scales,
    const float* __restrict__ rotations, const float* __restrict__ opacities, const float* __restrict__ shs,
    const float* __restrict__ cov3D_precomp, const float* __restrict__ colors_precomp,
    const float* __restrict__ V, const float* __restrict__ Pm, const float* __restrict__ campos, GeomState g,
    int* __restrict__ radii_out, const bool write_cov3D, unsigned long long* __restrict__ done_word,
    unsigned long long* __restrict__ publish,
    const uint32_t ticket, uint32_t* __restrict__ ghist_acc, uint32_t* __restrict__ ghist_clear) {
  if (blockIdx.x == 0 && threadIdx.x == 0) { g.total[2] = 0u; g.total[11] = 0u; }
  float Vc[16], Pc[16];
#pragma unroll
  for (int k = 0; k < 16; k++) { Vc[k] = V[k]; Pc[k] = Pm[k]; }
  const float cam0 = campos[0], cam1 = campos[1], cam2 = campos[2];
  extern __shared__ float sh_rows[];
  __shared__ uint32_t dhist[5][256];
  __shared__ float4 s_rec[PRE_BLOCK / 64][64 * SPLAT_F4];
  if (ghist_acc) {
#pragma unroll
    for (int k = 0; k < 5; k++) dhist[k][threadIdx.x] = 0u;
    if (blockIdx.x == 0)
#pragma unroll
      for (int k = 0; k < 5; k++) ghist_clear[k * 256 + threadIdx.x] = 0u;
    __syncthreads();
  }
  struct In { float mx, my, mz, s0, s1, s2, op, dc0, dc1, dc2; float4 q; };
  const bool dc_direct = PLAIN || (!STAGED && shs && !colors_precomp);
  const int D = PLAIN ? 0 : fp.D;
  auto fetch = [&](const int i_) {
    In v;
    const int i = i_ < fp.P ? i_ : fp.P - 1;
    v.s0 = v.s1 = v.s2 = v.dc0 = v.dc1 = v.dc2 = 0.f;
    v.q = make_float4(0.f, 0.f, 0.f, 0.f);
    v.mx = means3D[3 * i]; v.my = means3D[3 * i + 1]; v.mz = means3D[3 * i + 2];
    if (PIN || scales) { v.s0 = scales[3 * i]; v.s1 = scales[3 * i + 1]; v.s2 = scales[3 * i + 2]; }
    if (PIN || !cov3D_precomp) v.q = reinterpret_cast<const float4*>(rotations)[i];
    v.op = opacities[i];
    if (dc_direct) {
      const float* r = shs + (size_t)i * fp.M * 3;
      v.dc0 = r[0]; v.dc1 = r[1]; v.dc2 = r[2];
    }
    return v;
  };
  uint32_t tiles_wg = 0;
  const int nblk = (fp.P + PRE_BLOCK - 1) / PRE_BLOCK;
  auto work = [&](const In& in, const int blk, auto&& before_stores) {
  const int idx_raw = blk * PRE_BLOCK + threadIdx.x;
  const bool dup = idx_raw >= fp.P;
  const int idx = dup ? fp.P - 1 : idx_raw;
  if (STAGED && !(ROWK > 0 && (blk + 1) * PRE_BLOCK <= fp.P)) {
    const int row0 = blk * PRE_BLOCK;
    if (blk != (int)blockIdx.x) __syncthreads();
    if (row0 < fp.P) rows_to_lds(sh_rows, shs + (size_t)row0 * fp.M * 3, min(PRE_BLOCK, fp.P - row0), fp.M * 3);
    __syncthreads();
  }
  uint32_t tiles = 0, rect_packed = 0, dkey = 0xFFFFFFFFu;
  int radius = 0;
  float4 rec0 = make_float4(0.f, 0.f, 0.f, 0.f), rec1 = rec0, rec2 = rec0;
  uint8_t clamp_out = 0;
  {
    const float mx = in.mx, my = in.my, mz = in.mz;
    const float pvz = Vc[2] * mx + Vc[6] * my + Vc[10] * mz + Vc[14];
    bool alive = !(pvz <= 0.2f);
    float s0 = 0, s1 = 0, s2 = 0;
    if (alive && (PIN || scales)) {
      s0 = fp.scale_modifier * in.s0;
      s1 = fp.scale_modifier * in.s1;
      s2 = fp.scale_modifier * in.s2;
      alive = !(s0 > 0.3f || s1 > 0.3f || s2 > 0.3f);
    }
    if (alive) {
      const float ph0 = Pc[0] * mx + Pc[4] * my + Pc[8] * mz + Pc[12];
      const float ph1 = Pc[1] * mx + Pc[5] * my + Pc[9] * mz + Pc[13];
      const float ph3 = Pc[3] * mx + Pc[7] * my + Pc[11] * mz + Pc[15];
      const float pw = 1.0f / (ph3 + 0.0000001f);
      const float ppx = ph0 * pw, ppy = ph1 * pw;
      float c6[6];
      if (!PIN && cov3D_precomp) {
#pragma unroll
        for (int k = 0; k < 6; k++) c6[k] = cov3D_precomp[6 * idx + k];
      } else {
        cov3d_from_scale_rot(s0, s1, s2, in.q, c6);
        if (!PIN && write_cov3D) {
#pragma unroll
          for (int k = 0; k < 6; k++) g.cov3D[6 * (size_t)idx + k] = c6[k];
        }
      }
      const Ewa e = ewa_project(mx, my, mz, fp, c6, Vc);
      const float cx = e.cxx + 0.3f, cy = e.cxy, cz = e.cyy + 0.3f;
      const float det = cx * cz - cy * cy;
      if (det != 0.0f) {
        const float det_inv = 1.f / det;
        const float conx = cz * det_inv, cony = -cy * det_inv, conz = cx * det_inv;
        const float mid = 0.5f * (cx + cz);
        const float disc = sqrtf(fmax_(0.1f, mid * mid - det));
        const float lambda1 = mid + disc, lambda2 = mid - disc;
        const float my_radius = ceilf(3.f * sqrtf(fmax_(lambda1, lambda2)));
        const float pixx = ndc_to_pix(ppx, fp.W), pixy = ndc_to_pix(ppy, fp.H);
        int x0, y0, x1, y1;
        tile_rect(pixx, pixy, (int)my_radius, fp.gx, fp.gy, x0, y0, x1, y1);
        const int area = (x1 - x0) * (y1 - y0);
        if (area != 0) {
          float rgb[3];
          uint8_t clampbits = 0;
          if (!PIN && colors_precomp) {
            rgb[0] = colors_precomp[3 * idx];
            rgb[1] = colors_precomp[3 * idx + 1];
            rgb[2] = colors_precomp[3 * idx + 2];
          } else {
            float x = 0.f, y = 0.f, z = 0.f;
            if (D > 0) {
              const float d0 = mx - cam0, d1 = my - cam1, d2 = mz - cam2;
              const float len = sqrtf(d0 * d0 + d1 * d1 + d2 * d2);
              x = d0 / len; y = d1 / len; z = d2 / len;
            }
            const float* sh = STAGED ? sh_rows + (idx - blk * PRE_BLOCK) * sh_row_stride(fp.M * 3)
                                     : shs + (size_t)idx * fp.M * 3;
            const float dc[3] = {dc_direct ? in.dc0 : sh[0], dc_direct ? in.dc1 : sh[1], dc_direct ? in.dc2 : sh[2]};
#pragma unroll
            for (int ch = 0; ch < 3; ch++) {
              float res = SH0 * dc[ch];
              if (D > 0) {
                res = res - SH1 * y * sh[3 + ch] + SH1 * z * sh[6 + ch] - SH1 * x * sh[9 + ch];
                if (D > 1) {
                  const float xx = x * x, yy = y * y, zz = z * z, xy = x * y, yz = y * z, xz = x * z;
                  res = res + SH2c[0] * xy * sh[12 + ch] + SH2c[1] * yz * sh[15 + ch] +
                        SH2c[2] * (2.0f * zz - xx - yy) * sh[18 + ch] + SH2c[3] * xz * sh[21 + ch] +
                        SH2c[4] * (xx - yy) * sh[24 + ch];
                  if (D > 2) {
                    res = res + SH3c[0] * y * (3.0f * xx - yy) * sh[27 + ch] + SH3c[1] * xy * z * sh[30 + ch] +
                          SH3c[2] * y * (4.0f * zz - xx - yy) * sh[33 + ch] +
                          SH3c[3] * z * (2.0f * zz - 3.0f * xx - 3.0f * yy) * sh[36 + ch] +
                          SH3c[4] * x * (4.0f * zz - xx - yy) * sh[39 + ch] + SH3c[5] * z * (xx - yy) * sh[42 + ch] +
                          SH3c[6] * x * (xx - 3.0f * yy) * sh[45 + ch];
                  }
                }
              }
              res += 0.5f;
              if (res < 0) clampbits |= (uint8_t)(1u << ch);
              rgb[ch] = fmax_(res, 0.0f);
            }
          }
          const float op = in.op;
          float hx, hy;
          if (op < 1.0f / 255.0f) {
            hx = hy = -1e30f;
          } else {
            const float tau = footprint_tau(op);
            const float dc = conx * conz - cony * cony;
            if (conx > 0.0f && conz > 0.0f && dc > 0.0f) {
              hx = sqrtf(2.0f * tau * conz / dc) + 0.05f;
              hy = sqrtf(2.0f * tau * conx / dc) + 0.05f;
            } else {
              hx = hy = 1e30f;
            }
          }
          if (fp.ref_rects) {
          } else if (hx < 0.0f) {
            x1 = x0;
          } else if (hx < 1e6f) {
            const float lim = 1e6f;
            const int bx0 = (int)ceilf(fmax_(-lim, fmin_(lim, (pixx - hx - 15.0f) * 0.0625f)));
            const int bx1 = (int)floorf(fmax_(-lim, fmin_(lim, (pixx + hx) * 0.0625f))) + 1;
            const int by0 = (int)ceilf(fmax_(-lim, fmin_(lim, (pixy - hy - 15.0f) * 0.0625f)));
            const int by1 = (int)floorf(fmax_(-lim, fmin_(lim, (pixy + hy) * 0.0625f))) + 1;
            x0 = max(x0, bx0); x1 = min(x1, bx1);
            y0 = max(y0, by0); y1 = min(y1, by1);
          }
          radius = (int)my_radius;
          tiles = (x1 > x0 && y1 > y0) ? (uint32_t)((x1 - x0) * (y1 - y0)) : 0u;
          rect_packed = (uint32_t)x0 | ((uint32_t)y0 << 10) | ((uint32_t)(x1 - x0) << 20);
          if (tiles) dkey = __float_as_uint(pvz);
          rec0 = make_float4(pixx, pixy, conx, cony);
          rec1 = make_float4(conz, op, rgb[0], rgb[1]);
          rec2 = make_float4(rgb[2], pvz, hx, hy);
          clamp_out = clampbits;

        }
      }
    }
  }
  before_stores();
  radii_out[idx] = radius;
  g.gpack[idx] = make_uint2(tiles, tiles ? rect_packed : 0u);
  g.touched[idx] = 0;
  g.clamped[idx] = clamp_out;
  g.dkeysA[idx] = dkey;
  if (dup) { tiles = 0u; dkey = 0xFFFFFFFFu; }
  {
    float4* img = s_rec[threadIdx.x >> 6];
    const int lane = threadIdx.x & 63;
    img[3 * lane + 0] = rec0;
    img[3 * lane + 1] = rec1;
    img[3 * lane + 2] = rec2;
    __builtin_amdgcn_fence(__ATOMIC_RELEASE, "wavefront");
    __builtin_amdgcn_wave_barrier();
    __builtin_amdgcn_fence(__ATOMIC_ACQUIRE, "wavefront");
    const int first = min(blk * PRE_BLOCK + (int)(threadIdx.x & ~63u), fp.P - 1);
    const int nrec = min(64, fp.P - first) * SPLAT_F4;
    float4* dst = g.splats + (size_t)first * SPLAT_F4;
#pragma unroll
    for (int k = 0; k < 3; k++) {
      const int j = min(lane + 64 * k, nrec - 1);
      dst[j] = img[j];
    }
    __builtin_amdgcn_fence(__ATOMIC_RELEASE, "wavefront");
    __builtin_amdgcn_wave_barrier();
  }
  if (ghist_acc) {
    const bool has = !dup, none = has && dkey == 0xFFFFFFFFu;
    const uint64_t nm = __ballot(none);
    if (has && !none) {
#pragma unroll
      for (int k = 0; k < 4; k++) atomicAdd(&dhist[k][(dkey >> (8 * k)) & 255u], 1u);
      atomicAdd(&dhist[4][dkey >> 24], tiles);
    }
    if (nm != 0ull && (threadIdx.x & 63) == 0) {
      const uint32_t c = (uint32_t)__popcll(nm);
#pragma unroll
      for (int k = 0; k < 4; k++) atomicAdd(&dhist[k][255], c);
    }
  }
  tiles_wg += tiles;
  };
  {
    auto pin = [](In& v) {
      asm volatile("" : "+v"(v.mx), "+v"(v.my), "+v"(v.mz), "+v"(v.s0), "+v"(v.s1), "+v"(v.s2), "+v"(v.op));
      asm volatile("" : "+v"(v.dc0), "+v"(v.dc1), "+v"(v.dc2), "+v"(v.q.x), "+v"(v.q.y), "+v"(v.q.z), "+v"(v.q.w));
    };
    In a = fetch(blockIdx.x * PRE_BLOCK + threadIdx.x);
    pin(a);
    constexpr int NPRE = ROWK > 0 ? ROWK : 1;
    float4 pre[NPRE];
    const int lane_ = threadIdx.x & 63, wave0 = (int)(threadIdx.x & ~63u);
    auto rows_fetch = [&](const int blk) {
      const int first = min(blk * PRE_BLOCK + wave0, fp.P - 1);
      const int n4 = min(64, fp.P - first) * NPRE;
      const float4* src = reinterpret_cast<const float4*>(shs + (size_t)first * (4 * NPRE));
#pragma unroll
      for (int k = 0; k < NPRE; k++) pre[k] = src[min(lane_ + 64 * k, n4 - 1)];
    };
    auto rows_commit = [&]() {
      float* img = sh_rows + wave0 * sh_row_stride(4 * NPRE);
      __builtin_amdgcn_fence(__ATOMIC_RELEASE, "wavefront");
      __builtin_amdgcn_wave_barrier();
#pragma unroll
      for (int k = 0; k < NPRE; k++) {
        const int j = lane_ + 64 * k, r = j / NPRE, c4 = j - r * NPRE;
        float* d = img + r * sh_row_stride(4 * NPRE) + 4 * c4;
        d[0] = pre[k].x; d[1] = pre[k].y; d[2] = pre[k].z; d[3] = pre[k].w;
      }
      __builtin_amdgcn_fence(__ATOMIC_RELEASE, "wavefront");
      __builtin_amdgcn_wave_barrier();
      __builtin_amdgcn_fence(__ATOMIC_ACQUIRE, "wavefront");
    };
    if constexpr (ROWK > 0) rows_fetch(blockIdx.x);
    for (int blk = blockIdx.x; blk < nblk; blk += (int)gridDim.x) {
      if constexpr (ROWK > 0) {
        if ((blk + 1) * PRE_BLOCK <= fp.P) rows_commit();
      }
      const In n = fetch((blk + (int)gridDim.x) * PRE_BLOCK + threadIdx.x);
      if constexpr (ROWK > 0) rows_fetch(blk + (int)gridDim.x);
      work(a, blk, [&] {
        a = n;
        pin(a);
      });
    }
  }
  for (size_t w = (size_t)blockIdx.x * PRE_BLOCK + threadIdx.x; w < g.dsort.nwords; w += (size_t)gridDim.x * PRE_BLOCK)
    g.dsort.words[w] = 0u;
  __shared__ uint32_t wsum[PRE_BLOCK / 64];
  const uint32_t ws = wave_sum_u32(tiles_wg);
  if ((threadIdx.x & 63) == 0) wsum[threadIdx.x >> 6] = ws;
  __syncthreads();
  if (ghist_acc) {
#pragma unroll
    for (int k = 0; k < 5; k++) {
      const uint32_t c = dhist[k][threadIdx.x];
      if (c) (void)__hip_atomic_fetch_add(ghist_acc + k * 256 + threadIdx.x, c, __ATOMIC_RELAXED, __HIP_MEMORY_SCOPE_AGENT);
    }
  }
  if (threadIdx.x == 0) {
    const uint32_t mine = wsum[0] + wsum[1] + wsum[2] + wsum[3];
    const unsigned long long old = atomicAdd(done_word, (1ull << 40) | (unsigned long long)mine);
    if ((old >> 40) == (unsigned long long)gridDim.x - 1ull) {
      const unsigned long long tot = (old & ((1ull << 40) - 1ull)) + mine;
      const uint32_t r = tot > 0xFFFFFFFFull ? 0xFFFFFFFFu : (uint32_t)tot;
      g.total[0] = r;
      __hip_atomic_store(done_word, 0ull, __ATOMIC_RELAXED, __HIP_MEMORY_SCOPE_AGENT);
      if (publish)
        __hip_atomic_store(publish, ((unsigned long long)ticket << 32) | r, __ATOMIC_RELAXED,
                           __HIP_MEMORY_SCOPE_SYSTEM);
// ... 528 lines not shown
      *reinterpret_cast<uint4*>(sm.L.lval + sl) = make_uint4(iv[r][0], iv[r][1], iv[r][2], iv[r][3]);
      *reinterpret_cast<uint4*>(sm.L.lval + sl + 4) = make_uint4(iv[r][4], iv[r][5], iv[r][6], iv[r][7]);
    } else {
      for (int k = 0; k < 8 && t0 + k < (size_t)R; k++) {
        sm.L.lkey[sl + k] = (uint16_t)tk[r][k];
        sm.L.lval[sl + k] = iv[r][k];
      }
    }
  }
  __syncthreads();
  uint32_t key[NSTEP], val[NSTEP];
#pragma unroll
  for (int s = 0; s < NSTEP; s++) {
    const uint32_t p = (uint32_t)(w * (TSORT_TILE / TSORT_WAVES) + s * 64 + lane);
    const bool valid = (size_t)tile * TSORT_TILE + p < (size_t)R;
    key[s] = valid ? (uint32_t)sm.L.lkey[p] : 0u;
    val[s] = valid ? sm.L.lval[p] : 0u;
  }
  __syncthreads();
  scatter_core<uint16_t, false, ARANK, TSORT_WAVES, TSORT_TILE>(sm.L, key, val, tile, keys_out, vals_out, R, shift0, nbits0,
                                                                counts, chunk_base, digit_total, nullptr);
  });
}

template <typename K, bool STORE>
__global__ __launch_bounds__(256) void k_emit(const FrameParams fp, const uint4* __restrict__ sdesc, const Count cnt,
                                              const uint32_t* __restrict__ chunk_first,
                                              K* __restrict__ tkeys_out, uint32_t* __restrict__ ivals_out,
                                              uint8_t* __restrict__ inst_flag, uint32_t* __restrict__ counts0,
                                              const uint32_t digit_shift0, const uint32_t digit_mask0) {
  __shared__ EmitStage st;
  __shared__ uint32_t hist[256];
  const int tid = threadIdx.x;
  if (cnt.closed()) return;
  const int R = cnt.get();
  for_each_unit(units_of(R, EMIT_CHUNK), [&](const int chunk) {
  hist[tid] = 0;
  const uint32_t c0 = (uint32_t)chunk * EMIT_CHUNK;
  const uint32_t c1 = c0 + EMIT_CHUNK < (uint32_t)R ? c0 + EMIT_CHUNK : (uint32_t)R;
  const int S = emit_stage(sdesc, chunk_first, chunk, c1, R, fp.P, tid, st);
  __syncthreads();
  const uint32_t t0 = c0 + (uint32_t)tid * 8u;
  if (t0 < c1) {
  uint32_t tk[8], iv[8];
  emit_walk8(t0, c1, S, st, (uint32_t)fp.gx, tk, iv);
  if (!STORE) {
    if (t0 + 8u <= c1) {
      *reinterpret_cast<uint2*>(inst_flag + t0) = make_uint2(0u, 0u);
    } else {
      for (int k = 0; k < 8 && t0 + (uint32_t)k < c1; k++) inst_flag[t0 + k] = 0;
    }
  } else if (t0 + 8u <= c1) {
    uint4* vo = reinterpret_cast<uint4*>(ivals_out + t0);
    if (sizeof(K) == 2) {
      *reinterpret_cast<uint4*>(tkeys_out + t0) = make_uint4(tk[0] | (tk[1] << 16), tk[2] | (tk[3] << 16),
                                                             tk[4] | (tk[5] << 16), tk[6] | (tk[7] << 16));
    } else {
      uint4* ko = reinterpret_cast<uint4*>(tkeys_out + t0);
      ko[0] = make_uint4(tk[0], tk[1], tk[2], tk[3]);
      ko[1] = make_uint4(tk[4], tk[5], tk[6], tk[7]);
    }
    vo[0] = make_uint4(iv[0], iv[1], iv[2], iv[3]);
    vo[1] = make_uint4(iv[4], iv[5], iv[6], iv[7]);
    *reinterpret_cast<uint2*>(inst_flag + t0) = make_uint2(0u, 0u);
  } else {
    for (int k = 0; k < 8 && t0 + (uint32_t)k < c1; k++) {
      tkeys_out[t0 + k] = (K)tk[k];
      ivals_out[t0 + k] = iv[k];
      inst_flag[t0 + k] = 0;
    }
  }
#pragma unroll
  for (int k = 0; k < 8; k++)
    if (t0 + (uint32_t)k < c1) atomicAdd(&hist[(tk[k] >> digit_shift0) & digit_mask0], 1u);
  }
  __syncthreads();
  const uint32_t hc = hist[tid];
  if (hc) atomicAdd(&counts0[(size_t)(c0 / TSORT_TILE) * 256 + tid], hc);
  });
}

__global__ __launch_bounds__(PRE_BLOCK) void k_compact_touched(const int P, const uint8_t* __restrict__ touched,
                                                               uint32_t* __restrict__ list,
                                                               uint32_t* __restrict__ count) {
  __shared__ uint32_t wtot[PRE_BLOCK / 64];
  __shared__ uint32_t wg_base;
  const int idx0 = (blockIdx.x * PRE_BLOCK + threadIdx.x) * 16;
  const int lane = threadIdx.x & 63, w = threadIdx.x >> 6;
  uint32_t f[4] = {0u, 0u, 0u, 0u};
  if (idx0 + 15 < P) {
    const uint4 v = *reinterpret_cast<const uint4*>(touched + idx0);
    f[0] = v.x; f[1] = v.y; f[2] = v.z; f[3] = v.w;
  } else {
    for (int k = 0; k < 16 && idx0 + k < P; k++) f[k >> 2] |= (uint32_t)touched[idx0 + k] << (8 * (k & 3));
  }
  uint32_t c = 0;
#pragma unroll
  for (int k = 0; k < 16; k++) c += ((f[k >> 2] >> (8 * (k & 3))) & 0xFFu) ? 1u : 0u;
  const uint32_t inc = wave_incl_scan_u32(c, lane);
  if (lane == 63) wtot[w] = inc;
  __syncthreads();
  if (threadIdx.x == 0) {
    const uint32_t tot = wtot[0] + wtot[1] + wtot[2] + wtot[3];
    wg_base = tot ? atomicAdd(count, tot) : 0u;
  }
  __syncthreads();
  if (!c) return;
  uint32_t base = wg_base + inc - c;
  for (int k = 0; k < w; k++) base += wtot[k];
#pragma unroll
  for (int k = 0; k < 16; k++)
    if ((f[k >> 2] >> (8 * (k & 3))) & 0xFFu) list[base++] = (uint32_t)(idx0 + k);
}

template <int CTRL, int ROW_MASK>
__device__ __forceinline__ float dpp_get_(float v) {
  return __int_as_float(__builtin_amdgcn_update_dpp(0, __float_as_int(v), CTRL, ROW_MASK, 0xF, false));
}
__device__ __forceinline__ float row_allsum_(float v) {
  v += dpp_get_<0xB1, 0xF>(v);
  v += dpp_get_<0x4E, 0xF>(v);
  v += dpp_get_<0x124, 0xF>(v);
  v += dpp_get_<0x128, 0xF>(v);
  return v;
}
__device__ __forceinline__ void swap_add32_(float& a, float& b) {
  const auto r = __builtin_amdgcn_permlane32_swap(__float_as_uint(a), __float_as_uint(b), false, false);
  a = __uint_as_float(r[0]) + __uint_as_float(r[1]);
}
__device__ __forceinline__ void swap_add16_(float& a, float& b) {
  const auto r = __builtin_amdgcn_permlane16_swap(__float_as_uint(a), __float_as_uint(b), false, false);
  a = __uint_as_float(r[0]) + __uint_as_float(r[1]);
}

struct RecordSums {
  static constexpr bool depth = false;
  float v0 = 0, v1 = 0, v2 = 0, v3 = 0, v4 = 0, v5 = 0, v6 = 0, v7 = 0, v8 = 0;
};
struct RecordSumsDepth : RecordSums {
  static constexpr bool depth = true;
  float v9 = 0;
};
constexpr uint32_t GATHER_CHUNK = 512;
constexpr uint32_t GATHER_SHARED_FROM = 2048;
template <class Sums>
__device__ __forceinline__ void gather_chunk(const size_t first, const uint32_t n, const uint32_t base, const int lane,
                                             const float4* __restrict__ grad_inst, uint8_t* __restrict__ inst_flag,
                                             Sums& r) {
  uint8_t f[8];
#pragma unroll
  for (int j = 0; j < 8; j++) {
    const uint32_t k = base + 64 * j + lane;
    f[j] = k < n ? inst_flag[first + k] : (uint8_t)0;
  }
#pragma unroll
  for (int q = 0; q < 2; q++) {
    if (base + 256u * q >= n) break;
    float4 a[4], b[4], c[4];
#pragma unroll
    for (int j = 0; j < 4; j++) {
      if (f[4 * q + j]) {
        const size_t slot = first + base + 64 * (4 * q + j) + lane;
        inst_flag[slot] = 0;
        a[j] = grad_inst[slot * GRAD_F4 + 0];
        b[j] = grad_inst[slot * GRAD_F4 + 1];
        c[j] = grad_inst[slot * GRAD_F4 + 2];
      }
    }
#pragma unroll
    for (int j = 0; j < 4; j++) {
      if (f[4 * q + j]) {
        r.v0 += a[j].x; r.v1 += a[j].y; r.v2 += a[j].z; r.v3 += a[j].w;
        r.v4 += b[j].x; r.v5 += b[j].y; r.v6 += b[j].z; r.v7 += b[j].w;
        if constexpr (Sums::depth) {
          r.v8 += c[j].x + c[j].y;
          r.v9 += c[j].z + c[j].w;
        } else {
          r.v8 += (c[j].x + c[j].y) + (c[j].z + c[j].w);
        }
      }
    }
  }
}
template <class Sums>
__device__ __forceinline__ void gather_finish(Sums r, const uint32_t id, const int lane, const float cx, const float cy,
                                              const float cz, const float op, const float ddelx_dx, const float ddely_dy,
                                              float* __restrict__ dL_dmean2D, float* __restrict__ dL_dconic,
                                              float* __restrict__ dL_dopacity, float* __restrict__ dL_dcolor,
                                              float* __restrict__ dL_ddepths) {
  swap_add32_(r.v0, r.v4);
  swap_add32_(r.v1, r.v5);
  swap_add32_(r.v2, r.v6);
  swap_add32_(r.v3, r.v7);
  swap_add16_(r.v0, r.v2);
  swap_add16_(r.v1, r.v3);
  const float w0 = row_allsum_(r.v0), w1 = row_allsum_(r.v1);
  float v8 = row_allsum_(r.v8);
  v8 += dpp_get_<0x142, 0xA>(v8);
  v8 += dpp_get_<0x143, 0xC>(v8);
  const float S3 = __int_as_float(__builtin_amdgcn_readlane(__float_as_int(w1), 16));
  const float S4 = __int_as_float(__builtin_amdgcn_readlane(__float_as_int(w0), 32));
  const float mc = -0.5f * op;
  if (lane == 0) { dL_dcolor[3 * id] = w0; dL_dcolor[3 * id + 1] = w1; }
  if (lane == 16) { dL_dcolor[3 * id + 2] = w0; dL_dmean2D[3 * id] = -(cx * S3 + cy * S4) * (op * ddelx_dx); }
  if (lane == 32) { dL_dmean2D[3 * id + 1] = -(cz * S4 + cy * S3) * (op * ddely_dy); dL_dconic[4 * id] = w1 * mc; }
  if (lane == 48) { dL_dconic[4 * id + 1] = w0 * mc; dL_dconic[4 * id + 3] = w1 * mc; }
  if (lane == 63) dL_dopacity[id] = v8;
  if constexpr (Sums::depth) {
    float v9 = row_allsum_(r.v9);
    v9 += dpp_get_<0x142, 0xA>(v9);
    v9 += dpp_get_<0x143, 0xC>(v9);
    if (lane == 63) dL_ddepths[id] = v9;
  }
}

template <class Sums = RecordSums>
__global__ __launch_bounds__(PRE_BLOCK) __attribute__((amdgpu_num_vgpr(96))) void k_gather_records(
    GeomState g, const float4* __restrict__ grad_inst, uint8_t* __restrict__ inst_flag,
    float* __restrict__ dL_dmean2D, float* __restrict__ dL_dconic, float* __restrict__ dL_dopacity,
    float* __restrict__ dL_dcolor, const float ddelx_dx, const float ddely_dy, const int P, const bool from_descriptors,
    float* __restrict__ dL_ddepths) {
  constexpr int NW = PRE_BLOCK / 64;
  constexpr int NS = Sums::depth ? 10 : 9;
  __shared__ uint32_t s_long[PRE_BLOCK];
  __shared__ uint32_t s_nlong;
  __shared__ float s_part[NW][NS][64];
  const int lane = threadIdx.x & 63, w = threadIdx.x >> 6;
  const uint32_t nwaves = gridDim.x * NW;
  const uint32_t nA = from_descriptors ? g.total[7] : 0u;
  const uint32_t count = from_descriptors ? nA + g.total[10] : g.total[2];
  for (uint32_t base = 0; base < count; base += 64u * nwaves) {
    if (threadIdx.x == 0) s_nlong = 0u;
    __syncthreads();
    const uint32_t qc = base + ((uint32_t)lane * NW + (uint32_t)w) * gridDim.x + blockIdx.x;
    uint32_t cand = 0xFFFFFFFFu;
    if (qc < count) cand = !from_descriptors ? g.tlist[qc] : qc < nA ? g.sdesc[qc].y : g.sdescB[qc - nA].y;
    const bool has = cand < (uint32_t)P && (!from_descriptors || g.touched[cand] != 0);
    uint32_t my_first = 0u, my_n = 0u;
    float4 my_ra = make_float4(0.f, 0.f, 0.f, 0.f), my_rb = my_ra;
    if (has) {
      my_first = g.slotinfo[cand].x;
      my_n = g.gpack[cand].x;
      my_ra = g.splats[(size_t)cand * SPLAT_F4 + 0];
      my_rb = g.splats[(size_t)cand * SPLAT_F4 + 1];
    }
    const bool is_long = has && my_n > GATHER_SHARED_FROM;
    if (is_long) s_long[atomicAdd(&s_nlong, 1u)] = cand;
    for (uint64_t todo = __ballot(has && !is_long); todo != 0ull; todo &= todo - 1ull) {
      const int src = __builtin_ctzll(todo);
      const uint32_t id = (uint32_t)__builtin_amdgcn_readlane((int)cand, src);
      const size_t first = (uint32_t)__builtin_amdgcn_readlane((int)my_first, src);
      const uint32_t n = (uint32_t)__builtin_amdgcn_readlane((int)my_n, src);
      Sums r;
      for (uint32_t cb = 0; cb < n; cb += GATHER_CHUNK) gather_chunk(first, n, cb, lane, grad_inst, inst_flag, r);
      gather_finish(r, id, lane, __int_as_float(__builtin_amdgcn_readlane(__float_as_int(my_ra.z), src)),
                    __int_as_float(__builtin_amdgcn_readlane(__float_as_int(my_ra.w), src)),
                    __int_as_float(__builtin_amdgcn_readlane(__float_as_int(my_rb.x), src)),
                    __int_as_float(__builtin_amdgcn_readlane(__float_as_int(my_rb.y), src)), ddelx_dx, ddely_dy, dL_dmean2D,
                    dL_dconic, dL_dopacity, dL_dcolor, dL_ddepths);
    }
    __syncthreads();
    const uint32_t nlong = s_nlong;
    for (uint32_t i = 0; i < nlong; i++) {
      const uint32_t id = s_long[i];
      const size_t first = g.slotinfo[id].x;
      const uint32_t n = g.gpack[id].x;
      Sums r;
      for (uint32_t cb = (uint32_t)w * GATHER_CHUNK; cb < n; cb += NW * GATHER_CHUNK)
        gather_chunk(first, n, cb, lane, grad_inst, inst_flag, r);
      s_part[w][0][lane] = r.v0; s_part[w][1][lane] = r.v1; s_part[w][2][lane] = r.v2;
      s_part[w][3][lane] = r.v3; s_part[w][4][lane] = r.v4; s_part[w][5][lane] = r.v5;
      s_part[w][6][lane] = r.v6; s_part[w][7][lane] = r.v7; s_part[w][8][lane] = r.v8;
      if constexpr (Sums::depth) s_part[w][9][lane] = r.v9;
      __syncthreads();
      if (w == 0) {
        Sums t;
        float* tv[9] = {&t.v0, &t.v1, &t.v2, &t.v3, &t.v4, &t.v5, &t.v6, &t.v7, &t.v8};
#pragma unroll
        for (int k = 0; k < 9; k++) {
          float acc = s_part[0][k][lane];
#pragma unroll
          for (int ww = 1; ww < NW; ww++) acc += s_part[ww][k][lane];
          *tv[k] = acc;
        }
        if constexpr (Sums::depth) {
          float acc = s_part[0][9][lane];
#pragma unroll
          for (int ww = 1; ww < NW; ww++) acc += s_part[ww][9][lane];
          t.v9 = acc;
        }
        const float4 ra = g.splats[(size_t)id * SPLAT_F4 + 0];
        const float4 rb = g.splats[(size_t)id * SPLAT_F4 + 1];
        gather_finish(t, id, lane, ra.z, ra.w, rb.x, rb.y, ddelx_dx, ddely_dy, dL_dmean2D, dL_dconic, dL_dopacity, dL_dcolor,
                      dL_ddepths);
      }
      __syncthreads();
    }
    __syncthreads();
  }
}

template <bool DEPTH>
__device__ __forceinline__ void gaussian_backward_one(
    const int idx, float* row,
    const FrameParams& fp, GeomState& g, const int* __restrict__ radii, const float* __restrict__ means3D, const float* __restrict__ scales,
    const float* __restrict__ rotations, const float* __restrict__ shs, const float* __restrict__ cov3D_precomp,
    const float* __restrict__ V, const float* __restrict__ Pm, const float* __restrict__ campos,
    const int colors_are_precomp, float* dL_dmean2D, float* dL_dconic, float* dL_dopacity, float* dL_dcolor,
    float* __restrict__ dL_dmean3D,
    float* __restrict__ dL_dcov3D, float* __restrict__ dL_dsh, float* __restrict__ dL_dscale,
    float* __restrict__ dL_drot, float* dL_ddepths, const bool skip_recordless) {
  const int rad_in = radii[idx];
  const uint8_t touched_in = g.touched[idx];
  const bool vis = rad_in > 0;
  const int M = fp.M;
  float* gs = row ? row : dL_dsh + (size_t)idx * fp.M * 3;
  if (idx == 0) g.total[2] = 0u;
  const bool was_touched = touched_in != 0;
  if (was_touched) g.touched[idx] = 0;
  const bool rec = vis && was_touched;
  if (!rec && (skip_recordless || !vis)) {
    dL_dmean2D[3 * idx] = 0.f; dL_dmean2D[3 * idx + 1] = 0.f; dL_dmean2D[3 * idx + 2] = 0.f;
    dL_dconic[4 * idx] = 0.f; dL_dconic[4 * idx + 1] = 0.f; dL_dconic[4 * idx + 2] = 0.f; dL_dconic[4 * idx + 3] = 0.f;
    dL_dopacity[idx] = 0.f;
    if constexpr (DEPTH) dL_ddepths[idx] = 0.f;
    dL_dcolor[3 * idx] = 0.f; dL_dcolor[3 * idx + 1] = 0.f; dL_dcolor[3 * idx + 2] = 0.f;
    dL_dmean3D[3 * idx] = 0.f; dL_dmean3D[3 * idx + 1] = 0.f; dL_dmean3D[3 * idx + 2] = 0.f;
    if (dL_dcov3D) {
#pragma unroll
      for (int k = 0; k < 6; k++) dL_dcov3D[6 * (size_t)idx + k] = 0.f;
    }
    for (int k = 0; k < 3 * M; k++) gs[k] = 0.f;
    dL_dscale[3 * idx] = 0.f; dL_dscale[3 * idx + 1] = 0.f; dL_dscale[3 * idx + 2] = 0.f;
    dL_drot[4 * idx] = 0.f; dL_drot[4 * idx + 1] = 0.f; dL_drot[4 * idx + 2] = 0.f; dL_drot[4 * idx + 3] = 0.f;
    return;
  }
  const float gcol0 = rec ? dL_dcolor[3 * idx] : 0.f, gcol1 = rec ? dL_dcolor[3 * idx + 1] : 0.f, gcol2 = rec ? dL_dcolor[3 * idx + 2] : 0.f;
  const float gmx = rec ? dL_dmean2D[3 * idx] : 0.f, gmy = rec ? dL_dmean2D[3 * idx + 1] : 0.f;
  const float gca = rec ? dL_dconic[4 * idx] : 0.f, gcb = rec ? dL_dconic[4 * idx + 1] : 0.f, gcc = rec ? dL_dconic[4 * idx + 3] : 0.f;
  float gz = 0.f;
  if constexpr (DEPTH) {
    if (rec) gz = dL_ddepths[idx];
    else dL_ddepths[idx] = 0.f;
  }
  if (!rec) {
    dL_dmean2D[3 * idx] = 0.f; dL_dmean2D[3 * idx + 1] = 0.f;
    dL_dconic[4 * idx] = 0.f; dL_dconic[4 * idx + 1] = 0.f; dL_dconic[4 * idx + 3] = 0.f;
    dL_dopacity[idx] = 0.f;
    dL_dcolor[3 * idx] = 0.f; dL_dcolor[3 * idx + 1] = 0.f; dL_dcolor[3 * idx + 2] = 0.f;
  }
  const float mx = means3D[3 * idx], my = means3D[3 * idx + 1], mz = means3D[3 * idx + 2];
  const uint8_t clamped_in = g.clamped[idx];
  float4 q_in = make_float4(0.f, 0.f, 0.f, 0.f);
  float sc_in[3] = {0.f, 0.f, 0.f};
  if (scales) {
    q_in = reinterpret_cast<const float4*>(rotations)[idx];
    sc_in[0] = scales[3 * idx]; sc_in[1] = scales[3 * idx + 1]; sc_in[2] = scales[3 * idx + 2];
  }
  float c6[6];
  if (cov3D_precomp) {
#pragma unroll
    for (int k = 0; k < 6; k++) c6[k] = cov3D_precomp[6 * (size_t)idx + k];
  } else {
    cov3d_from_scale_rot(fp.scale_modifier * sc_in[0], fp.scale_modifier * sc_in[1], fp.scale_modifier * sc_in[2], q_in, c6);
  }
  const float* sh = row ? row : shs + (size_t)idx * fp.M * 3;
  dL_dmean2D[3 * idx + 2] = 0.f;
  dL_dconic[4 * idx + 2] = 0.f;
  const Ewa e = ewa_project(mx, my, mz, fp, c6, V);
  const float limx = 1.3f * fp.tan_fovx, limy = 1.3f * fp.tan_fovy;
  const float xmul = (e.txtz < -limx || e.txtz > limx) ? 0.f : 1.f;
  const float ymul = (e.tytz < -limy || e.tytz > limy) ? 0.f : 1.f;
  const float a = e.cxx + 0.3f, b = e.cxy, c = e.cyy + 0.3f;
  const float denom = a * c - b * b;
  float dL_da = 0, dL_db = 0, dL_dc = 0;
  const float denom2inv = 1.0f / ((denom * denom) + 0.0000001f);
  float dcov[6] = {0, 0, 0, 0, 0, 0};
  if (denom2inv != 0) {
    dL_da = denom2inv * (-c * c * gca + 2 * b * c * gcb + (denom - a * c) * gcc);
    dL_dc = denom2inv * (-a * a * gcc + 2 * a * b * gcb + (denom - a * c) * gca);
    dL_db = denom2inv * 2 * (b * c * gca - (denom + 2 * b * b) * gcb + a * b * gcc);
    dcov[0] = (e.T00 * e.T00 * dL_da + e.T00 * e.T10 * dL_db + e.T10 * e.T10 * dL_dc);
    dcov[3] = (e.T01 * e.T01 * dL_da + e.T01 * e.T11 * dL_db + e.T11 * e.T11 * dL_dc);
    dcov[5] = (e.T02 * e.T02 * dL_da + e.T02 * e.T12 * dL_db + e.T12 * e.T12 * dL_dc);
    dcov[1] = 2 * e.T00 * e.T01 * dL_da + (e.T00 * e.T11 + e.T01 * e.T10) * dL_db + 2 * e.T10 * e.T11 * dL_dc;
    dcov[2] = 2 * e.T00 * e.T02 * dL_da + (e.T00 * e.T12 + e.T02 * e.T10) * dL_db + 2 * e.T10 * e.T12 * dL_dc;
    dcov[4] = 2 * e.T02 * e.T01 * dL_da + (e.T01 * e.T12 + e.T02 * e.T11) * dL_db + 2 * e.T11 * e.T12 * dL_dc;
  }
  if (dL_dcov3D) {
#pragma unroll
    for (int k = 0; k < 6; k++) dL_dcov3D[6 * (size_t)idx + k] = dcov[k];
  }
  const float S00 = c6[0], S01 = c6[1], S02 = c6[2], S11 = c6[3], S12 = c6[4], S22 = c6[5];
  const float u0 = e.T00 * S00 + e.T01 * S01 + e.T02 * S02, u1 = e.T00 * S01 + e.T01 * S11 + e.T02 * S12,
              u2 = e.T00 * S02 + e.T01 * S12 + e.T02 * S22;
  const float v0 = e.T10 * S00 + e.T11 * S01 + e.T12 * S02, v1 = e.T10 * S01 + e.T11 * S11 + e.T12 * S12,
              v2 = e.T10 * S02 + e.T11 * S12 + e.T12 * S22;
  const float dT00 = 2 * u0 * dL_da + v0 * dL_db, dT01 = 2 * u1 * dL_da + v1 * dL_db, dT02 = 2 * u2 * dL_da + v2 * dL_db;
  const float dT10 = 2 * v0 * dL_dc + u0 * dL_db, dT11 = 2 * v1 * dL_dc + u1 * dL_db, dT12 = 2 * v2 * dL_dc + u2 * dL_db;
  const float dJ00 = V[0] * dT00 + V[4] * dT01 + V[8] * dT02;
  const float dJ02 = V[2] * dT00 + V[6] * dT01 + V[10] * dT02;
  const float dJ11 = V[1] * dT10 + V[5] * dT11 + V[9] * dT12;
  const float dJ12 = V[2] * dT10 + V[6] * dT11 + V[10] * dT12;
  const float tz = 1.f / e.tz, tz2 = tz * tz, tz3 = tz2 * tz;
  const float hx = fp.focal_x, hy = fp.focal_y;
  const float dtx = xmul * -hx * tz2 * dJ02;
  const float dty = ymul * -hy * tz2 * dJ12;
  const float dtz = -hx * tz2 * dJ00 - hy * tz2 * dJ11 + (2 * hx * e.tx) * tz3 * dJ02 + (2 * hy * e.ty) * tz3 * dJ12;
  float dm0 = V[0] * dtx + V[1] * dty + V[2] * dtz;
  float dm1 = V[4] * dtx + V[5] * dty + V[6] * dtz;
  float dm2 = V[8] * dtx + V[9] * dty + V[10] * dtz;
  {
    const float mh3 = Pm[3] * mx + Pm[7] * my + Pm[11] * mz + Pm[15];
    const float m_w = 1.0f / (mh3 + 0.0000001f);
    const float mul1 = (Pm[0] * mx + Pm[4] * my + Pm[8] * mz + Pm[12]) * m_w * m_w;
    const float mul2 = (Pm[1] * mx + Pm[5] * my + Pm[9] * mz + Pm[13]) * m_w * m_w;
    dm0 += (Pm[0] * m_w - Pm[3] * mul1) * gmx + (Pm[1] * m_w - Pm[3] * mul2) * gmy;
    dm1 += (Pm[4] * m_w - Pm[7] * mul1) * gmx + (Pm[5] * m_w - Pm[7] * mul2) * gmy;
    dm2 += (Pm[8] * m_w - Pm[11] * mul1) * gmx + (Pm[9] * m_w - Pm[11] * mul2) * gmy;
  }
  if (shs && !colors_are_precomp) {
    const uint8_t cb = clamped_in;
    const float gr[3] = {(cb & 1) ? 0.f : gcol0, (cb & 2) ? 0.f : gcol1, (cb & 4) ? 0.f : gcol2};
    const float q0 = mx - campos[0], q1 = my - campos[1], q2 = mz - campos[2];
    const float len = sqrtf(q0 * q0 + q1 * q1 + q2 * q2);
    const float x = q0 / len, y = q1 / len, z = q2 / len;
    float ddx = 0, ddy = 0, ddz = 0;
    const int D = fp.D;
    const int used = (D + 1) * (D + 1);
#pragma unroll
    for (int ch = 0; ch < 3; ch++) {
      const float gch = gr[ch];
      float c_[16];
#pragma unroll
      for (int k = 1; k < 16; k++) c_[k] = k < used ? sh[3 * k + ch] : 0.f;
      float dx_ = 0, dy_ = 0, dz_ = 0;
      gs[ch] = SH0 * gch;
      if (D > 0) {
        gs[3 + ch] = (-SH1 * y) * gch;
        gs[6 + ch] = (SH1 * z) * gch;
        gs[9 + ch] = (-SH1 * x) * gch;
        dx_ = -SH1 * c_[3];
        dy_ = -SH1 * c_[1];
        dz_ = SH1 * c_[2];
        if (D > 1) {
          const float xx = x * x, yy = y * y, zz = z * z, xy = x * y, yz = y * z, xz = x * z;
          gs[12 + ch] = (SH2c[0] * xy) * gch;
          gs[15 + ch] = (SH2c[1] * yz) * gch;
          gs[18 + ch] = (SH2c[2] * (2.f * zz - xx - yy)) * gch;
          gs[21 + ch] = (SH2c[3] * xz) * gch;
          gs[24 + ch] = (SH2c[4] * (xx - yy)) * gch;
          dx_ += SH2c[0] * y * c_[4] + SH2c[2] * 2.f * -x * c_[6] + SH2c[3] * z * c_[7] +
                 SH2c[4] * 2.f * x * c_[8];
          dy_ += SH2c[0] * x * c_[4] + SH2c[1] * z * c_[5] + SH2c[2] * 2.f * -y * c_[6] +
                 SH2c[4] * 2.f * -y * c_[8];
          dz_ += SH2c[1] * y * c_[5] + SH2c[2] * 2.f * 2.f * z * c_[6] + SH2c[3] * x * c_[7];
          if (D > 2) {
            gs[27 + ch] = (SH3c[0] * y * (3.f * xx - yy)) * gch;
            gs[30 + ch] = (SH3c[1] * xy * z) * gch;
            gs[33 + ch] = (SH3c[2] * y * (4.f * zz - xx - yy)) * gch;
            gs[36 + ch] = (SH3c[3] * z * (2.f * zz - 3.f * xx - 3.f * yy)) * gch;
            gs[39 + ch] = (SH3c[4] * x * (4.f * zz - xx - yy)) * gch;
            gs[42 + ch] = (SH3c[5] * z * (xx - yy)) * gch;
            gs[45 + ch] = (SH3c[6] * x * (xx - 3.f * yy)) * gch;
            dx_ += (SH3c[0] * c_[9] * 3.f * 2.f * xy + SH3c[1] * c_[10] * yz +
                    SH3c[2] * c_[11] * -2.f * xy + SH3c[3] * c_[12] * -3.f * 2.f * xz +
                    SH3c[4] * c_[13] * (-3.f * xx + 4.f * zz - yy) + SH3c[5] * c_[14] * 2.f * xz +
                    SH3c[6] * c_[15] * 3.f * (xx - yy));
            dy_ += (SH3c[0] * c_[9] * 3.f * (xx - yy) + SH3c[1] * c_[10] * xz +
                    SH3c[2] * c_[11] * (-3.f * yy + 4.f * zz - xx) + SH3c[3] * c_[12] * -3.f * 2.f * yz +
                    SH3c[4] * c_[13] * -2.f * xy + SH3c[5] * c_[14] * -2.f * yz +
                    SH3c[6] * c_[15] * -3.f * 2.f * xy);
            dz_ += (SH3c[1] * c_[10] * xy + SH3c[2] * c_[11] * 4.f * 2.f * yz +
                    SH3c[3] * c_[12] * 3.f * (2.f * zz - xx - yy) + SH3c[4] * c_[13] * 4.f * 2.f * xz +
                    SH3c[5] * c_[14] * (xx - yy));
          }
        }
      }
      ddx += dx_ * gch;
      ddy += dy_ * gch;
      ddz += dz_ * gch;
    }
    for (int k = used * 3; k < M * 3; k++) gs[k] = 0.f;
    const float sum2 = q0 * q0 + q1 * q1 + q2 * q2;
    const float inv32 = 1.0f / sqrtf(sum2 * sum2 * sum2);
    dm0 += ((+sum2 - q0 * q0) * ddx - q1 * q0 * ddy - q2 * q0 * ddz) * inv32;
    dm1 += (-q0 * q1 * ddx + (sum2 - q1 * q1) * ddy - q2 * q1 * ddz) * inv32;
    dm2 += (-q0 * q2 * ddx - q1 * q2 * ddy + (sum2 - q2 * q2) * ddz) * inv32;
  } else {
    for (int k = 0; k < M * 3; k++) gs[k] = 0.f;
  }
  if constexpr (DEPTH) {
    dm0 += V[2] * gz; dm1 += V[6] * gz; dm2 += V[10] * gz;
  }
  dL_dmean3D[3 * idx] = dm0; dL_dmean3D[3 * idx + 1] = dm1; dL_dmean3D[3 * idx + 2] = dm2;
  if (scales) {
    const float4 q = q_in;
    const float r = q.x, x = q.y, y = q.z, z = q.w;
    const float s[3] = {fp.scale_modifier * sc_in[0], fp.scale_modifier * sc_in[1], fp.scale_modifier * sc_in[2]};
    float R[3][3];
    R[0][0] = 1.f - 2.f * (y * y + z * z); R[0][1] = 2.f * (x * y - r * z); R[0][2] = 2.f * (x * z + r * y);
    R[1][0] = 2.f * (x * y + r * z); R[1][1] = 1.f - 2.f * (x * x + z * z); R[1][2] = 2.f * (y * z - r * x);
    R[2][0] = 2.f * (x * z - r * y); R[2][1] = 2.f * (y * z + r * x); R[2][2] = 1.f - 2.f * (x * x + y * y);
    const float dS[3][3] = {{dcov[0], 0.5f * dcov[1], 0.5f * dcov[2]},
                            {0.5f * dcov[1], dcov[3], 0.5f * dcov[4]},
                            {0.5f * dcov[2], 0.5f * dcov[4], dcov[5]}};
    float dMt[3][3];
#pragma unroll
    for (int cc = 0; cc < 3; cc++)
#pragma unroll
      for (int rr = 0; rr < 3; rr++) {
        const float v = (2.0f * (s[rr] * R[0][rr])) * dS[cc][0] + (2.0f * (s[rr] * R[1][rr])) * dS[cc][1] +
                        (2.0f * (s[rr] * R[2][rr])) * dS[cc][2];
        dMt[rr][cc] = v;
      }
    float ds[3];
#pragma unroll
    for (int k = 0; k < 3; k++) ds[k] = R[0][k] * dMt[k][0] + R[1][k] * dMt[k][1] + R[2][k] * dMt[k][2];
    dL_dscale[3 * idx] = ds[0]; dL_dscale[3 * idx + 1] = ds[1]; dL_dscale[3 * idx + 2] = ds[2];
#pragma unroll
    for (int k = 0; k < 3; k++)
#pragma unroll
      for (int rr = 0; rr < 3; rr++) dMt[k][rr] *= s[k];
#define Dm(ci, ri) dMt[ci][ri]
    const float dq0 = 2 * z * (Dm(0, 1) - Dm(1, 0)) + 2 * y * (Dm(2, 0) - Dm(0, 2)) + 2 * x * (Dm(1, 2) - Dm(2, 1));
    const float dq1 = 2 * y * (Dm(1, 0) + Dm(0, 1)) + 2 * z * (Dm(2, 0) + Dm(0, 2)) + 2 * r * (Dm(1, 2) - Dm(2, 1)) -
                      4 * x * (Dm(2, 2) + Dm(1, 1));
    const float dq2 = 2 * x * (Dm(1, 0) + Dm(0, 1)) + 2 * r * (Dm(2, 0) - Dm(0, 2)) + 2 * z * (Dm(1, 2) + Dm(2, 1)) -
                      4 * y * (Dm(2, 2) + Dm(0, 0));
    const float dq3 = 2 * r * (Dm(0, 1) - Dm(1, 0)) + 2 * x * (Dm(2, 0) + Dm(0, 2)) + 2 * y * (Dm(1, 2) + Dm(2, 1)) -
                      4 * z * (Dm(1, 1) + Dm(0, 0));
#undef Dm
    dL_drot[4 * idx] = dq0; dL_drot[4 * idx + 1] = dq1; dL_drot[4 * idx + 2] = dq2; dL_drot[4 * idx + 3] = dq3;
  } else {
    dL_dscale[3 * idx] = 0.f; dL_dscale[3 * idx + 1] = 0.f; dL_dscale[3 * idx + 2] = 0.f;
    dL_drot[4 * idx] = 0.f; dL_drot[4 * idx + 1] = 0.f; dL_drot[4 * idx + 2] = 0.f; dL_drot[4 * idx + 3] = 0.f;
  }
}

template <bool STAGED, bool DEPTH = false>
__global__ __launch_bounds__(PRE_BLOCK) void k_gaussian_backward(
    const FrameParams fp, GeomState g, const int* __restrict__ radii, const float* __restrict__ means3D, const float* __restrict__ scales,
    const float* __restrict__ rotations, const float* __restrict__ shs, const float* __restrict__ cov3D_precomp,
    const float* __restrict__ V, const float* __restrict__ Pm, const float* __restrict__ campos,
    const int colors_are_precomp, float* dL_dmean2D, float* dL_dconic, float* dL_dopacity, float* dL_dcolor,
    float* __restrict__ dL_dmean3D,
    float* __restrict__ dL_dcov3D, float* __restrict__ dL_dsh, float* __restrict__ dL_dscale,
    float* __restrict__ dL_drot, const bool skip_recordless, float* dL_ddepths) {
  extern __shared__ float sh_rows[];
  __shared__ uint32_t s_rec[PRE_BLOCK];
  __shared__ uint32_t s_nrec;
  const int row0 = blockIdx.x * PRE_BLOCK, idx = row0 + threadIdx.x;
  const int C = fp.M * 3, nrows = min(PRE_BLOCK, fp.P - row0);
  if (STAGED) {
    if (threadIdx.x == 0) s_nrec = 0u;
    __syncthreads();
    if (idx < fp.P && radii[idx] > 0 && (g.touched[idx] != 0 || !skip_recordless)) s_rec[atomicAdd(&s_nrec, 1u)] = threadIdx.x;
    __syncthreads();
    listed_rows_to_lds(sh_rows, shs + (size_t)row0 * C, s_rec, (int)s_nrec, C);
    __syncthreads();
  }
  if (idx < fp.P)
    gaussian_backward_one<DEPTH>(idx, STAGED ? sh_rows + threadIdx.x * sh_row_stride(C) : nullptr, fp, g, radii, means3D,
                                 scales, rotations, shs, cov3D_precomp, V, Pm, campos, colors_are_precomp, dL_dmean2D,
                                 dL_dconic, dL_dopacity, dL_dcolor, dL_dmean3D, dL_dcov3D, dL_dsh, dL_dscale, dL_drot,
                                 dL_ddepths, skip_recordless);
  if (STAGED) {
    __syncthreads();
    lds_to_rows(dL_dsh + (size_t)row0 * C, sh_rows, nrows, C);
  }
}

__global__ __launch_bounds__(PRE_BLOCK) void k_mark_visible(int P, const float* __restrict__ means3D,
                                                            const float* __restrict__ V,
                                                            unsigned char* __restrict__ present) {
  const int idx = blockIdx.x * PRE_BLOCK + threadIdx.x;
  if (idx >= P) return;
  const float z = V[2] * means3D[3 * idx] + V[6] * means3D[3 * idx + 1] + V[10] * means3D[3 * idx + 2] + V[14];
  present[idx] = !(z <= 0.2f);
}

bool preprocess_counts_depth_digits(const FrameParams& fp, const float* shs, const float* colors_precomp) {
  const long given = env().pre_hist_min_p;
  const bool staged = shs && !colors_precomp && sh_stage_bytes(fp.M) != 0;
  return fp.P > (given >= 0 ? given : staged ? (1L << 20) : (1L << 17));
}

hipError_t launch_preprocess(const FrameParams& fp, const float* means3D, const float* scales, const float* rotations,
                             const float* opacities, const float* shs, const float* cov3D_precomp,
                             const float* colors_precomp, const float* view, const float* proj, const float* campos,
                             GeomState g, int* radii_out, bool write_cov3D, unsigned long long* done_word,
                             unsigned long long* publish, uint32_t ticket, uint32_t* ghist_acc, uint32_t* ghist_clear,
                             hipStream_t s) {
  if (!radii_out) radii_out = g.radii;
  const int nb = (fp.P + PRE_BLOCK - 1) / PRE_BLOCK;
  ProfScope ps_k_preprocess(K_PREPROCESS, s);
  const size_t stage = (shs && !colors_precomp) ? sh_stage_bytes(fp.M) : 0;
  const bool few_wg = ghist_acc != nullptr && fp.P <= (1 << 20);
  const int max_wg = (few_wg && !stage ? 1 : 3) * 256, rounds = (nb + max_wg - 1) / max_wg;
  const dim3 grid(rounds ? (nb + rounds - 1) / rounds : 1);
  const bool plain_in = shs && scales && rotations && !cov3D_precomp && !colors_precomp && !write_cov3D;
  const bool rows16 = plain_in && (reinterpret_cast<uintptr_t>(shs) & 15u) == 0;
  if (stage && rows16 && fp.M == 16)
    hipLaunchKernelGGL((k_preprocess<true, false, true, 12>), grid, dim3(PRE_BLOCK), stage, s, fp, means3D, scales, rotations,
                       opacities, shs, cov3D_precomp, colors_precomp, view, proj, campos, g, radii_out, write_cov3D,
                       done_word, publish, ticket, ghist_acc, ghist_clear);
  else if (stage && rows16 && fp.M == 4)
    hipLaunchKernelGGL((k_preprocess<true, false, true, 3>), grid, dim3(PRE_BLOCK), stage, s, fp, means3D, scales, rotations,
                       opacities, shs, cov3D_precomp, colors_precomp, view, proj, campos, g, radii_out, write_cov3D,
                       done_word, publish, ticket, ghist_acc, ghist_clear);
  else if (stage)
    hipLaunchKernelGGL(k_preprocess<true>, grid, dim3(PRE_BLOCK), stage, s, fp, means3D, scales, rotations, opacities,
                       shs, cov3D_precomp, colors_precomp, view, proj, campos, g, radii_out, write_cov3D, done_word, publish, ticket,
                       ghist_acc, ghist_clear);
  else if (fp.D == 0 && shs && scales && rotations && !cov3D_precomp && !colors_precomp && !write_cov3D)
    hipLaunchKernelGGL((k_preprocess<false, true>), grid, dim3(PRE_BLOCK), 0, s, fp, means3D, scales, rotations, opacities,
                       shs, cov3D_precomp, colors_precomp, view, proj, campos, g, radii_out, write_cov3D, done_word, publish, ticket,
                       ghist_acc, ghist_clear);
  else
    hipLaunchKernelGGL(k_preprocess<false>, grid, dim3(PRE_BLOCK), 0, s, fp, means3D, scales, rotations, opacities,
                       shs, cov3D_precomp, colors_precomp, view, proj, campos, g, radii_out, write_cov3D, done_word, publish, ticket,
                       ghist_acc, ghist_clear);
  return hipGetLastError();
}

hipError_t launch_point_offsets(const FrameParams& fp, GeomState g, hipStream_t s) {
  ProfScope ps(K_POINT_OFFSETS, s);
  hipLaunchKernelGGL(k_point_offsets, dim3(1), dim3(1024), 0, s, fp.P, g.gpack, g.point_offsets);
  return hipGetLastError();
}

hipError_t launch_scan_offsets(const FrameParams& fp, GeomState g, Count R, uint32_t* chunk_first, uint2* ranges,
                               uint2* rangesB, uint32_t* counts0, uint32_t near_budget,
                               unsigned long long* publish_near, uint32_t ticket, const uint32_t* top_hist,
                               const uint32_t* order, bool order_is_near_list, hipStream_t s) {
  const size_t ncounts0 = (size_t)((R.cap + TSORT_TILE - 1) / TSORT_TILE) * 256;
  ProfScope ps(K_SCAN_OFFSETS, s);
  hipLaunchKernelGGL(k_scan_offsets, dim3((fp.P + SCAN_TILE - 1) / SCAN_TILE), dim3(PRE_BLOCK), 0, s, fp, g, R,
                     chunk_first, ranges, rangesB, counts0, ncounts0, near_budget, publish_near, ticket, top_hist, order,
                     order_is_near_list);
  return hipGetLastError();
}

hipError_t launch_compact_near(const FrameParams& fp, GeomState g, const uint32_t* top_hist, uint32_t near_budget,
                               uint32_t* keys_out, uint32_t* vals_out, uint32_t* n_out, uint32_t* ghist_near,
                               unsigned long long* publish, uint32_t ticket, hipStream_t s) {
  ProfScope ps(K_COMPACT_NEAR, s);
  hipLaunchKernelGGL(k_compact_near, dim3((fp.P + COMPACT_TILE - 1) / COMPACT_TILE), dim3(PRE_BLOCK), 0, s, fp.P, g.dkeysA,
                     top_hist, near_budget, keys_out, vals_out, n_out, ghist_near, g.dsort.scanC_status(),
                     g.dsort.tickets() + 6, publish, ticket);
  return hipGetLastError();
}

hipError_t launch_scan_offsets_far(const FrameParams& fp, GeomState g, Count capB, uint32_t slot_base, const uint32_t* sat,
                                   uint32_t* chunk_firstB, uint32_t* counts0, unsigned long long* publish,
                                   uint32_t ticket, hipStream_t s) {
  const size_t ncounts0 = (size_t)((capB.cap + TSORT_TILE - 1) / TSORT_TILE) * 256;
  ProfScope ps(K_SCAN_OFFSETS, s);
  hipLaunchKernelGGL(k_scan_offsets_far, dim3((fp.P + SCAN_TILE - 1) / SCAN_TILE), dim3(PRE_BLOCK), 0, s, fp, g, capB,
                     slot_base, sat, chunk_firstB, counts0, ncounts0, publish, ticket);
  return hipGetLastError();
}

hipError_t launch_emit(const FrameParams& fp, const uint4* sdesc, Count R, uint32_t* chunk_first, uint32_t* tkeys_out,
                       uint32_t* ivals_out, uint8_t* inst_flag, uint32_t* counts0, uint32_t digit_shift0,
                       uint32_t digit_mask0, bool key16, bool store_pairs, hipStream_t s) {
  if (R.cap <= 0) return hipSuccess;
  ProfScope ps(K_EMIT, s);
  const dim3 grid(chain_grid(R, EMIT_CHUNK));
  if (key16 && store_pairs)
    hipLaunchKernelGGL((k_emit<uint16_t, true>), grid, dim3(256), 0, s, fp, sdesc, R, chunk_first,
                       reinterpret_cast<uint16_t*>(tkeys_out), ivals_out, inst_flag, counts0, digit_shift0, digit_mask0);
  else if (key16)
    hipLaunchKernelGGL((k_emit<uint16_t, false>), grid, dim3(256), 0, s, fp, sdesc, R, chunk_first,
                       reinterpret_cast<uint16_t*>(tkeys_out), ivals_out, inst_flag, counts0, digit_shift0, digit_mask0);
  else
    hipLaunchKernelGGL((k_emit<uint32_t, true>), grid, dim3(256), 0, s, fp, sdesc, R, chunk_first, tkeys_out, ivals_out,
                       inst_flag, counts0, digit_shift0, digit_mask0);
  return hipGetLastError();
}

hipError_t launch_emit_scatter(const EmitFusion& ef, uint16_t* keys_out, uint32_t* vals_out, int shift0, int nbits0,
                               const uint32_t* counts, const uint32_t* chunk_base, const uint32_t* digit_total,
                               bool arank, hipStream_t s) {
  const dim3 grid(chain_grid(ef.R, TSORT_TILE));
  if (arank)
    hipLaunchKernelGGL(k_emit_scatter<true>, grid, dim3(256), 0, s, ef.fp, ef.sdesc, ef.R, ef.chunk_first, keys_out, vals_out,
                       shift0, nbits0, counts, chunk_base, digit_total);
  else
    hipLaunchKernelGGL(k_emit_scatter<false>, grid, dim3(256), 0, s, ef.fp, ef.sdesc, ef.R, ef.chunk_first, keys_out,
                       vals_out, shift0, nbits0, counts, chunk_base, digit_total);
  return hipGetLastError();
}

hipError_t launch_gather_records(const FrameParams& fp, GeomState g, BinningState b, float* dL_dmean2D,
                                 float* dL_dconic, float* dL_dopacity, float* dL_dcolor, float* dL_ddepths,
                                 bool split_frame, hipStream_t s) {
  const int nb = (fp.P + PRE_BLOCK - 1) / PRE_BLOCK;
  if (!split_frame) {
    ProfScope ps(K_COMPACT_TOUCHED, s);
    hipLaunchKernelGGL(k_compact_touched, dim3((nb + 15) / 16), dim3(PRE_BLOCK), 0, s, fp.P, g.touched, g.tlist,
                       g.total + 2);
  }
  {
    ProfScope ps(K_GATHER_RECORDS, s);
    const int want = (fp.P + PRE_BLOCK / 64 - 1) / (PRE_BLOCK / 64);
    const int grid = want < 4096 ? want : 4096;
    if (dL_ddepths)
      hipLaunchKernelGGL(k_gather_records<RecordSumsDepth>, dim3(grid), dim3(PRE_BLOCK), 0, s, g, b.grad_inst,
                         b.inst_flag, dL_dmean2D, dL_dconic, dL_dopacity, dL_dcolor, 0.5f * (float)fp.W,
                         0.5f * (float)fp.H, fp.P, split_frame, dL_ddepths);
    else
      hipLaunchKernelGGL(k_gather_records<>, dim3(grid), dim3(PRE_BLOCK), 0, s, g, b.grad_inst, b.inst_flag, dL_dmean2D,
                         dL_dconic, dL_dopacity, dL_dcolor, 0.5f * (float)fp.W, 0.5f * (float)fp.H, fp.P, split_frame,
                         nullptr);
  }
  return hipGetLastError();
}

hipError_t launch_gaussian_backward(const FrameParams& fp, GeomState g, BinningState b, const int* radii,
                                    const float* means3D, const float* scales, const float* rotations,
                                    const float* shs, const float* cov3D_precomp, const float* view, const float* proj,
                                    const float* campos, bool colors_precomp, float* dL_dmean2D, float* dL_dconic,
                                    float* dL_dopacity, float* dL_dcolor, float* dL_dmean3D, float* dL_dcov3D,
                                    float* dL_dsh, float* dL_dscale, float* dL_drot, float* dL_ddepths,
                                    hipStream_t s) {
  const int nb = (fp.P + PRE_BLOCK - 1) / PRE_BLOCK;
  ProfScope ps_k_gaussian_bwd(K_GAUSSIAN_BWD, s);
  const size_t stage = (shs && !colors_precomp) ? sh_stage_bytes(fp.M) : 0;
  const bool skip_recordless = !env().gbwd_all;
  if (dL_ddepths) {
    if (stage)
      hipLaunchKernelGGL((k_gaussian_backward<true, true>), dim3(nb), dim3(PRE_BLOCK), stage, s, fp, g, radii, means3D,
                         scales, rotations, shs, cov3D_precomp, view, proj, campos, 0, dL_dmean2D, dL_dconic, dL_dopacity,
                         dL_dcolor, dL_dmean3D, dL_dcov3D, dL_dsh, dL_dscale, dL_drot, skip_recordless, dL_ddepths);
    else
      hipLaunchKernelGGL((k_gaussian_backward<false, true>), dim3(nb), dim3(PRE_BLOCK), 0, s, fp, g, radii, means3D,
                         scales, rotations, shs, cov3D_precomp, view, proj, campos, colors_precomp ? 1 : 0, dL_dmean2D,
                         dL_dconic, dL_dopacity, dL_dcolor, dL_dmean3D, dL_dcov3D, dL_dsh, dL_dscale, dL_drot,
                         skip_recordless, dL_ddepths);
  } else if (stage)
    hipLaunchKernelGGL(k_gaussian_backward<true>, dim3(nb), dim3(PRE_BLOCK), stage, s, fp, g, radii,
                       means3D, scales, rotations, shs, cov3D_precomp, view, proj, campos, 0,
                       dL_dmean2D, dL_dconic, dL_dopacity, dL_dcolor, dL_dmean3D, dL_dcov3D, dL_dsh, dL_dscale, dL_drot,
                       skip_recordless, nullptr);
  else
    hipLaunchKernelGGL(k_gaussian_backward<false>, dim3(nb), dim3(PRE_BLOCK), 0, s, fp, g, radii,
                       means3D, scales, rotations, shs, cov3D_precomp, view, proj, campos, colors_precomp ? 1 : 0,
                       dL_dmean2D, dL_dconic, dL_dopacity, dL_dcolor, dL_dmean3D, dL_dcov3D, dL_dsh, dL_dscale, dL_drot,
                       skip_recordless, nullptr);
  return hipGetLastError();
}

hipError_t launch_mark_visible(int P, const float* means3D, const float* view, unsigned char* present,
                               hipStream_t s) {
  const int nb = (P + PRE_BLOCK - 1) / PRE_BLOCK;
  ProfScope ps_k_mark_visible(K_MARK_VISIBLE, s);
  hipLaunchKernelGGL(k_mark_visible, dim3(nb), dim3(PRE_BLOCK), 0, s, P, means3D, view, present);
  return hipGetLastError();
}

}
```

### gs-livm_amd/csrc/torch_binding.cpp

```cpp
#include <torch/extension.h>

#include <c10/hip/HIPStream.h>

#include <stdexcept>
#include <string>
#include <tuple>

#include "gsraster.h"
#include "gsr_torch_next.hpp"

#ifdef GSR_REFERENCE_HEADER
#include GSR_REFERENCE_HEADER
#else
#include "gsr_torch_surface.hpp"
#endif

namespace {

void* current_stream() { return static_cast<void*>(c10::hip::getCurrentHIPStream().stream()); }

const float* fptr(const torch::Tensor& t) { return t.defined() && t.numel() ? t.data_ptr<float>() : nullptr; }

void check(int code, const char* what) {
  if (code < 0) throw std::runtime_error(std::string(what) + ": " + gsr_last_error());
}

char* resize_blob(void* ctx, size_t bytes) {
  auto* t = static_cast<torch::Tensor*>(ctx);
  if (t->numel() != 0)
    *t = torch::empty({static_cast<long long>(bytes)}, t->options());
  else
    t->resize_({static_cast<long long>(bytes)});
  return reinterpret_cast<char*>(t->data_ptr());
}

thread_local bool t_depth_gradient = false;

}

bool gsr_torch::set_depth_gradient(bool on) {
  const bool prev = t_depth_gradient;
  t_depth_gradient = on;
  return prev;
}

std::tuple<int, torch::Tensor, torch::Tensor, torch::Tensor, torch::Tensor, torch::Tensor, torch::Tensor, torch::Tensor>
RasterizeGaussiansCUDA(const torch::Tensor& background, const torch::Tensor& means3D, const torch::Tensor& colors,
                       const torch::Tensor& opacity, const torch::Tensor& scales, const torch::Tensor& rotations,
                       const float scale_modifier, const torch::Tensor& cov3D_precomp, const torch::Tensor& viewmatrix,
                       const torch::Tensor& projmatrix, const float tan_fovx, const float tan_fovy,
                       const int image_height, const int image_width, const torch::Tensor& sh, const int degree,
                       const torch::Tensor& campos, const bool prefiltered, const bool debug) {
  if (means3D.ndimension() != 2 || means3D.size(1) != 3) {
    AT_ERROR("means3D must have dimensions (num_points, 3)");
  }
  const int P = means3D.size(0);
  const int H = image_height;
  const int W = image_width;
  auto float_opts = means3D.options().dtype(torch::kFloat32);
  torch::Tensor out_color = torch::empty({3, H, W}, float_opts);
  torch::Tensor out_depth = torch::empty({1, H, W}, float_opts);
  torch::Tensor out_acc = torch::empty({1, H, W}, float_opts);
  torch::Tensor radii = P ? torch::empty({P}, means3D.options().dtype(torch::kInt32))
                          : torch::zeros({0}, means3D.options().dtype(torch::kInt32));
  auto byte_opts = means3D.options().dtype(torch::kByte);
  torch::Tensor geomBuffer = torch::empty({0}, byte_opts);
  torch::Tensor binningBuffer = torch::empty({0}, byte_opts);
  torch::Tensor imgBuffer = torch::empty({0}, byte_opts);

  int M = 0;
  if (sh.defined() && sh.numel() != 0) M = sh.size(1);
  auto bg = background.contiguous(), m3 = means3D.contiguous(), shc = sh.contiguous(), col = colors.contiguous(),
       op = opacity.contiguous(), sc = scales.contiguous(), rot = rotations.contiguous(),
       cov = cov3D_precomp.contiguous(), view = viewmatrix.contiguous(), proj = projmatrix.contiguous(),
       cam = campos.contiguous();
  const int rendered = gsr_forward(
      resize_blob, &geomBuffer, resize_blob, &binningBuffer, resize_blob, &imgBuffer, P, degree, M, fptr(bg), W, H,
      fptr(m3), fptr(shc), fptr(col), fptr(op), fptr(sc), scale_modifier, fptr(rot), fptr(cov), fptr(view), fptr(proj),
      fptr(cam), tan_fovx, tan_fovy, prefiltered ? 1 : 0, out_color.data_ptr<float>(), out_depth.data_ptr<float>(),
      out_acc.data_ptr<float>(), P ? radii.data_ptr<int>() : nullptr, debug ? 1 : 0, current_stream());
  check(rendered, "gsr_forward");
  return std::make_tuple(rendered, out_color, out_depth, out_acc, radii, geomBuffer, binningBuffer, imgBuffer);
}

static std::tuple<torch::Tensor, torch::Tensor, torch::Tensor, torch::Tensor, torch::Tensor, torch::Tensor, torch::Tensor,
                  torch::Tensor, torch::Tensor>
rasterize_backward_impl(const torch::Tensor& background, const torch::Tensor& means3D, const torch::Tensor& radii,
                        const torch::Tensor& colors, const torch::Tensor& scales, const torch::Tensor& rotations,
                        const float scale_modifier, const torch::Tensor& cov3D_precomp, const torch::Tensor& viewmatrix,
                        const torch::Tensor& projmatrix, const float tan_fovx, const float tan_fovy,
                        const torch::Tensor& dL_dout_color, const torch::Tensor& dL_dout_acc, const torch::Tensor& sh,
                        const int degree, const torch::Tensor& campos, const torch::Tensor& geomBuffer, const int R,
                        const torch::Tensor& binningBuffer, const torch::Tensor& imageBuffer, const bool debug,
                        const bool want_cov3D, const torch::Tensor& dL_dout_depth = torch::Tensor()) {
  const int P = means3D.size(0);
  const int H = dL_dout_color.size(1);
  const int W = dL_dout_color.size(2);
  int M = 0;
  if (sh.defined() && sh.numel() != 0) M = sh.size(1);
  auto o = means3D.options();
  auto mk = [&](std::initializer_list<int64_t> shape) { return P ? torch::empty(shape, o) : torch::zeros(shape, o); };
  torch::Tensor dL_dmeans3D = mk({P, 3});
  torch::Tensor dL_dmeans2D = mk({P, 3});
  torch::Tensor dL_dcolors = mk({P, 3});
  torch::Tensor dL_dconic = mk({P, 2, 2});
  torch::Tensor dL_dopacity = mk({P, 1});
  torch::Tensor dL_dcov3D = want_cov3D ? mk({P, 6}) : torch::Tensor();
  torch::Tensor dL_dsh = mk({P, M, 3});
  torch::Tensor dL_dscales = mk({P, 3});
  torch::Tensor dL_drotations = mk({P, 4});
  const bool with_depth = dL_dout_depth.defined();
  torch::Tensor dL_ddepths = with_depth ? mk({P}) : torch::Tensor();
  if (with_depth && dL_dout_depth.numel() != static_cast<int64_t>(H) * W) {
    AT_ERROR("dL_dout_depth must have H*W elements");
  }
  if (P != 0) {
    auto bg = background.contiguous(), m3 = means3D.contiguous(), shc = sh.contiguous(), col = colors.contiguous(),
         sc = scales.contiguous(), rot = rotations.contiguous(), cov = cov3D_precomp.contiguous(),
         view = viewmatrix.contiguous(), proj = projmatrix.contiguous(), cam = campos.contiguous(),
         dpix = dL_dout_color.contiguous(), dacc = dL_dout_acc.contiguous(), rad = radii.contiguous();
    if (with_depth) {
      auto ddep = dL_dout_depth.contiguous();
      check(gsr_backward_depth(P, degree, M, R, fptr(bg), W, H, fptr(m3), fptr(shc), fptr(col), fptr(sc), scale_modifier,
                               fptr(rot), fptr(cov), fptr(view), fptr(proj), fptr(cam), tan_fovx, tan_fovy,
                               rad.data_ptr<int>(), reinterpret_cast<char*>(geomBuffer.data_ptr()),
                               reinterpret_cast<char*>(binningBuffer.data_ptr()),
                               reinterpret_cast<char*>(imageBuffer.data_ptr()), fptr(dpix), fptr(dacc), fptr(ddep),
                               dL_dmeans2D.data_ptr<float>(), dL_dconic.data_ptr<float>(),
                               dL_dopacity.data_ptr<float>(), dL_dcolors.data_ptr<float>(),
                               dL_dmeans3D.data_ptr<float>(),
                               dL_dcov3D.defined() ? dL_dcov3D.data_ptr<float>() : nullptr,
                               M ? dL_dsh.data_ptr<float>() : nullptr, dL_dscales.data_ptr<float>(),
                               dL_drotations.data_ptr<float>(), dL_ddepths.data_ptr<float>(), debug ? 1 : 0,
                               current_stream()),
            "gsr_backward_depth");
    } else
    check(gsr_backward(P, degree, M, R, fptr(bg), W, H, fptr(m3), fptr(shc), fptr(col), fptr(sc), scale_modifier,
                       fptr(rot), fptr(cov), fptr(view), fptr(proj), fptr(cam), tan_fovx, tan_fovy,
                       rad.data_ptr<int>(), reinterpret_cast<char*>(geomBuffer.data_ptr()),
                       reinterpret_cast<char*>(binningBuffer.data_ptr()),
                       reinterpret_cast<char*>(imageBuffer.data_ptr()), fptr(dpix), fptr(dacc),
                       dL_dmeans2D.data_ptr<float>(), dL_dconic.data_ptr<float>(), dL_dopacity.data_ptr<float>(),
                       dL_dcolors.data_ptr<float>(), dL_dmeans3D.data_ptr<float>(),
                       dL_dcov3D.defined() ? dL_dcov3D.data_ptr<float>() : nullptr,
                       M ? dL_dsh.data_ptr<float>() : nullptr, dL_dscales.data_ptr<float>(),
                       dL_drotations.data_ptr<float>(), debug ? 1 : 0, current_stream()),
          "gsr_backward");
  }
  return std::make_tuple(dL_dmeans2D, dL_dcolors, dL_dopacity, dL_dmeans3D, dL_dcov3D, dL_dsh, dL_dscales,
                         dL_drotations, dL_ddepths);
}

std::tuple<torch::Tensor, torch::Tensor, torch::Tensor, torch::Tensor, torch::Tensor, torch::Tensor, torch::Tensor,
           torch::Tensor>
RasterizeGaussiansBackwardCUDA(const torch::Tensor& background, const torch::Tensor& means3D, const torch::Tensor& radii,
                               const torch::Tensor& colors, const torch::Tensor& scales, const torch::Tensor& rotations,
                               const float scale_modifier, const torch::Tensor& cov3D_precomp,
                               const torch::Tensor& viewmatrix, const torch::Tensor& projmatrix, const float tan_fovx,
                               const float tan_fovy, const torch::Tensor& dL_dout_color,
                               const torch::Tensor& dL_dout_acc, const torch::Tensor& sh, const int degree,
                               const torch::Tensor& campos, const torch::Tensor& geomBuffer, const int R,
                               const torch::Tensor& binningBuffer, const torch::Tensor& imageBuffer, const bool debug) {
  auto [g0, g1, g2, g3, g4, g5, g6, g7, unused] =
      rasterize_backward_impl(background, means3D, radii, colors, scales, rotations, scale_modifier, cov3D_precomp,
                              viewmatrix, projmatrix, tan_fovx, tan_fovy, dL_dout_color, dL_dout_acc, sh, degree, campos,
                              geomBuffer, R, binningBuffer, imageBuffer, debug, true);
  (void)unused;
  return std::make_tuple(g0, g1, g2, g3, g4, g5, g6, g7);
}

std::tuple<torch::Tensor, torch::Tensor, torch::Tensor, torch::Tensor, torch::Tensor, torch::Tensor, torch::Tensor,
           torch::Tensor, torch::Tensor>
RasterizeGaussiansBackwardDepthCUDA(const torch::Tensor& background, const torch::Tensor& means3D,
                                    const torch::Tensor& radii, const torch::Tensor& colors, const torch::Tensor& scales,
                                    const torch::Tensor& rotations, const float scale_modifier,
                                    const torch::Tensor& cov3D_precomp, const torch::Tensor& viewmatrix,
                                    const torch::Tensor& projmatrix, const float tan_fovx, const float tan_fovy,
                                    const torch::Tensor& dL_dout_color, const torch::Tensor& dL_dout_acc,
                                    const torch::Tensor& dL_dout_depth, const torch::Tensor& sh, const int degree,
                                    const torch::Tensor& campos, const torch::Tensor& geomBuffer, const int R,
                                    const torch::Tensor& binningBuffer, const torch::Tensor& imageBuffer,
                                    const bool debug) {
  if (!dL_dout_depth.defined()) AT_ERROR("dL_dout_depth must be defined");
  return rasterize_backward_impl(background, means3D, radii, colors, scales, rotations, scale_modifier, cov3D_precomp,
                                 viewmatrix, projmatrix, tan_fovx, tan_fovy, dL_dout_color, dL_dout_acc, sh, degree, campos,
                                 geomBuffer, R, binningBuffer, imageBuffer, debug, true, dL_dout_depth);
}

torch::Tensor markVisible(torch::Tensor& means3D, torch::Tensor& viewmatrix, torch::Tensor& projmatrix) {
  const int P = means3D.size(0);
  torch::Tensor present = torch::full({P}, false, means3D.options().dtype(at::kBool));
  if (P != 0) {
    auto m3 = means3D.contiguous(), view = viewmatrix.contiguous(), proj = projmatrix.contiguous();
    check(gsr_mark_visible(P, fptr(m3), fptr(view), fptr(proj),
                           reinterpret_cast<unsigned char*>(present.data_ptr<bool>()), current_stream()),
          "gsr_mark_visible");
  }
  return present;
}

torch::autograd::tensor_list _RasterizeGaussians::forward(
    torch::autograd::AutogradContext* ctx, torch::Tensor means3D, torch::Tensor means2D, torch::Tensor sh,
    torch::Tensor colors_precomp, torch::Tensor opacities, torch::Tensor scales, torch::Tensor rotations,
    torch::Tensor cov3Ds_precomp, torch::Tensor image_height, torch::Tensor image_width, torch::Tensor tanfovx,
    torch::Tensor tanfovy, torch::Tensor bg, torch::Tensor scale_modifier, torch::Tensor viewmatrix,
    torch::Tensor projmatrix, torch::Tensor sh_degree, torch::Tensor camera_center, torch::Tensor prefiltered) {
  const int image_height_val = image_height.item<int>();
  const int image_width_val = image_width.item<int>();
  const float tanfovx_val = tanfovx.item<float>();
  const float tanfovy_val = tanfovy.item<float>();
  const float scale_modifier_val = scale_modifier.item<float>();
  const int sh_degree_val = sh_degree.item<int>();
  const bool prefiltered_val = prefiltered.item<bool>();
  auto [num_rendered, color, out_depth, out_acc, radii, geomBuffer, binningBuffer, imgBuffer] =
      RasterizeGaussiansCUDA(bg, means3D, colors_precomp, opacities, scales, rotations, scale_modifier_val,
                             cov3Ds_precomp, viewmatrix, projmatrix, tanfovx_val, tanfovy_val, image_height_val,
                             image_width_val, sh, sh_degree_val, camera_center, prefiltered_val, false);
  ctx->save_for_backward(
      {colors_precomp, means3D, scales, rotations, cov3Ds_precomp, radii, sh, geomBuffer, binningBuffer, imgBuffer});
  ctx->saved_data["num_rendered"] = num_rendered;
  ctx->saved_data["background"] = bg;
  ctx->saved_data["scale_modifier"] = scale_modifier_val;
  ctx->saved_data["viewmatrix"] = viewmatrix;
  ctx->saved_data["projmatrix"] = projmatrix;
  ctx->saved_data["tanfovx"] = tanfovx_val;
  ctx->saved_data["tanfovy"] = tanfovy_val;
  ctx->saved_data["image_height"] = image_height_val;
  ctx->saved_data["image_width"] = image_width_val;
  ctx->saved_data["sh_degree"] = sh_degree_val;
  ctx->saved_data["camera_center"] = camera_center;
  ctx->saved_data["prefiltered"] = prefiltered_val;
  ctx->saved_data["depth_gradient"] = t_depth_gradient;
  ctx->mark_non_differentiable({radii});
  ctx->set_materialize_grads(false);
  return {color, radii, out_depth, out_acc};
}

torch::autograd::tensor_list _RasterizeGaussians::backward(torch::autograd::AutogradContext* ctx,
                                                           torch::autograd::tensor_list grad_outputs) {
  auto grad_out_color = grad_outputs[0];
  auto grad_acc = grad_outputs[3];
  const torch::Tensor grad_depth = ctx->saved_data["depth_gradient"].toBool() ? grad_outputs[2] : torch::Tensor();
  const int num_rendered = ctx->saved_data["num_rendered"].to<int>();
  auto saved = ctx->get_saved_variables();
  auto colors_precomp = saved[0], means3D = saved[1], scales = saved[2], rotations = saved[3],
       cov3Ds_precomp = saved[4], radii = saved[5], sh = saved[6], geomBuffer = saved[7], binningBuffer = saved[8],
       imgBuffer = saved[9];
  const int H = ctx->saved_data["image_height"].to<int>(), W = ctx->saved_data["image_width"].to<int>();
  if (!grad_out_color.defined()) grad_out_color = torch::zeros({3, H, W}, means3D.options());
  if (!grad_acc.defined()) grad_acc = torch::zeros({1, H, W}, means3D.options());
  auto [grad_means2D, grad_colors_precomp, grad_opacities, grad_means3D, grad_cov3Ds_precomp, grad_sh, grad_scales,
        grad_rotations, grad_depths] =
      rasterize_backward_impl(
          ctx->saved_data["background"].to<torch::Tensor>(), means3D, radii, colors_precomp, scales, rotations,
          ctx->saved_data["scale_modifier"].to<double>(), cov3Ds_precomp,
          ctx->saved_data["viewmatrix"].to<torch::Tensor>(), ctx->saved_data["projmatrix"].to<torch::Tensor>(),
          ctx->saved_data["tanfovx"].to<double>(), ctx->saved_data["tanfovy"].to<double>(), grad_out_color, grad_acc,
          sh, ctx->saved_data["sh_degree"].to<int>(), ctx->saved_data["camera_center"].to<torch::Tensor>(),
          geomBuffer, num_rendered, binningBuffer, imgBuffer, false, cov3Ds_precomp.numel() != 0,
          grad_depth);
  (void)grad_depths;
  auto opt = [](const torch::Tensor& g, const torch::Tensor& x) { return x.numel() ? g : torch::Tensor(); };
  return {grad_means3D,
          grad_means2D,
          opt(grad_sh, sh),
          opt(grad_colors_precomp, colors_precomp),
          grad_opacities,
          opt(grad_scales, scales),
          opt(grad_rotations, rotations),
          opt(grad_cov3Ds_precomp, cov3Ds_precomp),
          torch::Tensor(), torch::Tensor(), torch::Tensor(), torch::Tensor(), torch::Tensor(), torch::Tensor(),
          torch::Tensor(), torch::Tensor(), torch::Tensor(), torch::Tensor(), torch::Tensor()};
}

torch::Tensor GaussianRasterizer::mark_visible(torch::Tensor positions) {
  torch::NoGradGuard no_grad;
  return markVisible(positions, raster_settings_.viewmatrix, raster_settings_.projmatrix);
}

torch::autograd::tensor_list GaussianRasterizer::rasterize_gaussians(
    torch::Tensor means3D, torch::Tensor means2D, torch::Tensor sh, torch::Tensor colors_precomp,
    torch::Tensor opacities, torch::Tensor scales, torch::Tensor rotations, torch::Tensor cov3Ds_precomp,
    GaussianRasterizationSettings raster_settings) {
  torch::Device device = means3D.is_cuda() ? means3D.device() : torch::Device(torch::kCUDA);
  auto image_height = torch::tensor(raster_settings.image_height);
  auto image_width = torch::tensor(raster_settings.image_width);
  auto tanfovx = torch::tensor(raster_settings.tanfovx);
  auto tanfovy = torch::tensor(raster_settings.tanfovy);
  auto scale_modifier = torch::tensor(raster_settings.scale_modifier);
  auto sh_degree = torch::tensor(raster_settings.sh_degree);
  auto prefiltered = torch::tensor(raster_settings.prefiltered);
  auto mv = [&](torch::Tensor t) { return (t.defined() && t.device() != device) ? t.to(device) : t; };
  return _RasterizeGaussians::apply(mv(means3D), mv(means2D), mv(sh), mv(colors_precomp), mv(opacities), mv(scales),
                                    mv(rotations), mv(cov3Ds_precomp), image_height, image_width, tanfovx, tanfovy,
                                    mv(raster_settings.bg), scale_modifier, mv(raster_settings.viewmatrix),
                                    mv(raster_settings.projmatrix), sh_degree, mv(raster_settings.camera_center),
                                    prefiltered);
}

std::tuple<torch::Tensor, torch::Tensor, torch::Tensor, torch::Tensor> GaussianRasterizer::forward(
    torch::Tensor means3D, torch::Tensor means2D, torch::Tensor opacities, torch::Tensor shs,
    torch::Tensor colors_precomp, torch::Tensor scales, torch::Tensor rotations, torch::Tensor cov3D_precomp) {
  if ((shs.defined() && colors_precomp.defined()) || (!shs.defined() && !colors_precomp.defined())) {
    throw std::invalid_argument("Please provide exactly one of either SHs or precomputed colors!");
  }
  if (((scales.defined() || rotations.defined()) && cov3D_precomp.defined()) ||
      (!scales.defined() && !rotations.defined() && !cov3D_precomp.defined())) {
    throw std::invalid_argument(
        "Please provide exactly one of either scale/rotation pair or "
        "precomputed 3D covariance!");
  }
  if ((scales.defined() != rotations.defined()) && !cov3D_precomp.defined()) {
    throw std::invalid_argument("scales and rotations must be provided together");
  }
  auto empty = [&]() { return torch::empty({0}, means3D.options().dtype(torch::kFloat32)); };
  if (!shs.defined()) shs = empty();
  if (!colors_precomp.defined()) colors_precomp = empty();
  if (!scales.defined()) scales = empty();
  if (!rotations.defined()) rotations = empty();
  if (!cov3D_precomp.defined()) cov3D_precomp = empty();
  auto result = rasterize_gaussians(means3D, means2D, shs, colors_precomp, opacities, scales, rotations,
                                    cov3D_precomp, raster_settings_);
  return {result[0], result[1], result[2], result[3]};
}

#ifndef GSR_NO_PYBIND
namespace py = pybind11;

PYBIND11_MODULE(TORCH_EXTENSION_NAME, m) {
  m.doc() = "C++/LibTorch operator surface of gs_livm_amd (mirror of GS-LIVM's src/gs/rasterizer.cu)";
  m.def("RasterizeGaussiansCUDA", &RasterizeGaussiansCUDA);
  m.def("RasterizeGaussiansBackwardCUDA", &RasterizeGaussiansBackwardCUDA);
  m.def("RasterizeGaussiansBackwardDepthCUDA", &RasterizeGaussiansBackwardDepthCUDA);
  m.def("set_depth_gradient", &gsr_torch::set_depth_gradient, py::arg("on"));
  m.def("markVisible", [](torch::Tensor a, torch::Tensor b, torch::Tensor c) { return markVisible(a, b, c); });
  m.def("last_num_rendered", []() { return gsr_last_num_rendered(); });
  py::class_<GaussianRasterizationSettings>(m, "GaussianRasterizationSettings")
      .def(py::init([](int h, int w, float tx, float ty, torch::Tensor bg, float sm, torch::Tensor view,
                       torch::Tensor proj, int deg, torch::Tensor cam, bool pre) {
             return GaussianRasterizationSettings{h, w, tx, ty, bg, sm, view, proj, deg, cam, pre};
           }),
           py::arg("image_height"), py::arg("image_width"), py::arg("tanfovx"), py::arg("tanfovy"), py::arg("bg"),
           py::arg("scale_modifier"), py::arg("viewmatrix"), py::arg("projmatrix"), py::arg("sh_degree"),
           py::arg("camera_center"), py::arg("prefiltered") = false);
  auto opt = [](const py::object& o) { return o.is_none() ? torch::Tensor() : o.cast<torch::Tensor>(); };
  struct PyRasterizer {
    GaussianRasterizer impl;
    explicit PyRasterizer(GaussianRasterizationSettings s) : impl(std::move(s)) {}
  };
  py::class_<PyRasterizer>(m, "GaussianRasterizer")
      .def(py::init<GaussianRasterizationSettings>())
      .def("mark_visible", [](PyRasterizer& self, torch::Tensor p) { return self.impl.mark_visible(p); })
      .def("forward",
           [opt](PyRasterizer& self, torch::Tensor means3D, torch::Tensor means2D, torch::Tensor opacities,
                 py::object shs, py::object colors_precomp, py::object scales, py::object rotations,
                 py::object cov3D_precomp) {
             const torch::Tensor a = opt(shs), b = opt(colors_precomp), c = opt(scales), d = opt(rotations),
                                 e = opt(cov3D_precomp);
             py::gil_scoped_release unlocked;
             return self.impl.forward(means3D, means2D, opacities, a, b, c, d, e);
           },
           py::arg("means3D"), py::arg("means2D"), py::arg("opacities"), py::arg("shs") = py::none(),
           py::arg("colors_precomp") = py::none(), py::arg("scales") = py::none(), py::arg("rotations") = py::none(),
           py::arg("cov3D_precomp") = py::none());

  namespace nx = gsr_torch;
  auto n = m.def_submodule("next", "C++/LibTorch hosts of the fused loss, activations + Adam, growth and PLY export");
  n.def("reference_window_1d", &nx::reference_window_1d, py::arg("window_size") = 11, py::arg("sigma") = 1.5f);
  n.def("photometric_loss",
        [opt](torch::Tensor image, torch::Tensor gt, float lambda_dssim, py::object window) {
          return nx::photometric_loss(image, gt, lambda_dssim, opt(window));
        },
        py::arg("image"), py::arg("gt"), py::arg("lambda_dssim") = 0.2f, py::arg("window1d") = py::none());
  n.def("photometric_loss_parts",
        [opt](torch::Tensor image, torch::Tensor gt, float lambda_dssim, py::object window) {
          return nx::photometric_loss_parts(image, gt, lambda_dssim, opt(window));
        },
        py::arg("image"), py::arg("gt"), py::arg("lambda_dssim") = 0.2f, py::arg("window1d") = py::none());
  n.def("similarity_loss", &nx::similarity_loss, py::arg("points"), py::arg("sel"), py::arg("xyz"), py::arg("scaling"),
        py::arg("lambda_") = 0.2f);
  py::class_<nx::VoxelIndex>(n, "VoxelIndex")
      .def(py::init<>())
      .def("add", &nx::VoxelIndex::add, py::arg("keys"), py::arg("counts"), py::arg("first_row"))
      .def("select",
           [](const nx::VoxelIndex& self, const std::unordered_map<std::size_t, torch::Tensor>& losses,
              int64_t max_points, const std::string& device) -> py::object {
             torch::Tensor points, sel;
             if (!self.select(losses, points, sel, max_points, torch::Device(device))) return py::none();
             return py::make_tuple(points, sel);
           },
           py::arg("losses"), py::arg("max_points") = 500, py::arg("device") = "cuda")
      .def("__len__", &nx::VoxelIndex::size)
      .def("__contains__", &nx::VoxelIndex::contains);
  n.def("activate", [](torch::Tensor s, torch::Tensor r, torch::Tensor o, torch::Tensor dc, torch::Tensor rest) {
    const nx::Activated a = nx::activate(s, r, o, dc, rest);
    return std::make_tuple(a.scaling, a.rotation, a.opacity, a.features);
  });
  py::class_<nx::FusedAdam>(n, "FusedAdam")
      .def(py::init<std::vector<torch::Tensor>, std::vector<double>, double, double, double>(), py::arg("params"),
           py::arg("lrs"), py::arg("beta1") = 0.9, py::arg("beta2") = 0.999, py::arg("eps") = 1e-15)
      .def("step", &nx::FusedAdam::step, py::arg("zero_grad") = true)
      .def("step_model",
           [](nx::FusedAdam& self, torch::Tensor gx, torch::Tensor gs, torch::Tensor gr, torch::Tensor go,
              torch::Tensor gf) {
             const nx::Activated a = self.step_model(gx, gs, gr, go, gf);
             return std::make_tuple(a.scaling, a.rotation, a.opacity, a.features);
           })
      .def("replace_param", &nx::FusedAdam::replace_param)
      .def("step_count", &nx::FusedAdam::step_count)
      .def("params", &nx::FusedAdam::params)
      .def("exp_avg", &nx::FusedAdam::exp_avg)
      .def("exp_avg_sq", &nx::FusedAdam::exp_avg_sq);
  n.def("init_gaussians", &nx::init_gaussians);
  n.def("pack_ply_rows", &nx::pack_ply_rows);
  n.def("write_ply", &nx::write_ply);
  n.def("ply_attribute_names", &nx::ply_attribute_names);
}
#endif
```

### gs-livm_amd/rasterizer.py

```python
from typing import NamedTuple, Optional

import torch

from . import _capi


class GaussianRasterizationSettings(NamedTuple):
    image_height: int
    image_width: int
    tanfovx: float
    tanfovy: float
    bg: torch.Tensor
    scale_modifier: float
    viewmatrix: torch.Tensor
    projmatrix: torch.Tensor
    sh_degree: int
    camera_center: torch.Tensor
    prefiltered: bool = False
    depth_gradient: bool = False


def _empty(device):
    return torch.empty(0, device=device)


class _RasterizeGaussians(torch.autograd.Function):

    @staticmethod
    def forward(ctx, means3D, means2D, sh, colors_precomp, opacities, scales, rotations, cov3Ds_precomp, settings):
        s = settings
        R, color, depth, acc, radii, geom, binning, img = _capi.rasterize_forward(
            s.bg, means3D.contiguous(), colors_precomp.contiguous(), opacities.contiguous(), scales.contiguous(),
            rotations.contiguous(), s.scale_modifier, cov3Ds_precomp.contiguous(), s.viewmatrix.contiguous(),
            s.projmatrix.contiguous(), s.tanfovx, s.tanfovy, s.image_height, s.image_width, sh.contiguous(),
            s.sh_degree, s.camera_center.contiguous(), s.prefiltered, False)
        ctx.settings, ctx.num_rendered = s, R
        ctx.save_for_backward(colors_precomp, means3D, scales, rotations, cov3Ds_precomp, radii, sh, geom, binning,
                              img)
        ctx.mark_non_differentiable(radii)
        ctx.set_materialize_grads(False)
        return color, radii, depth, acc

    @staticmethod
    def backward(ctx, grad_color, _grad_radii, _grad_depth, grad_acc):
        s = ctx.settings
        grad_depth = _grad_depth if s.depth_gradient else None
        colors_precomp, means3D, scales, rotations, cov3Ds_precomp, radii, sh, geom, binning, img = ctx.saved_tensors
        if grad_color is None:
            grad_color = torch.zeros((3, s.image_height, s.image_width), device=means3D.device)
        if grad_acc is None:
            grad_acc = torch.zeros((1, s.image_height, s.image_width), device=means3D.device)
        (g_means2D, g_colors, g_opac, g_means3D, g_cov3D, g_sh, g_scales, g_rot) = _capi.rasterize_backward(
            s.bg, means3D.contiguous(), radii, colors_precomp.contiguous(), scales.contiguous(),
            rotations.contiguous(), s.scale_modifier, cov3Ds_precomp.contiguous(), s.viewmatrix.contiguous(),
            s.projmatrix.contiguous(), s.tanfovx, s.tanfovy, grad_color, grad_acc, sh.contiguous(), s.sh_degree,
            s.camera_center.contiguous(), geom, ctx.num_rendered, binning, img, False,
            want_cov3D=cov3Ds_precomp.numel() != 0, grad_depth=grad_depth)[:8]
        none_if_empty = lambda g, x: g if x.numel() else None
        return (g_means3D, g_means2D, none_if_empty(g_sh, sh), none_if_empty(g_colors, colors_precomp), g_opac,
                none_if_empty(g_scales, scales), none_if_empty(g_rot, rotations),
                none_if_empty(g_cov3D, cov3Ds_precomp), None)


def rasterize_gaussians(means3D, means2D, sh, colors_precomp, opacities, scales, rotations, cov3Ds_precomp,
                        raster_settings):
    dev = means3D.device if means3D.is_cuda else torch.device("cuda")
    mv = lambda t: t if t.device == dev else t.to(dev)
    s = raster_settings._replace(bg=mv(raster_settings.bg), viewmatrix=mv(raster_settings.viewmatrix),
                                 projmatrix=mv(raster_settings.projmatrix),
                                 camera_center=mv(raster_settings.camera_center))
    return _RasterizeGaussians.apply(mv(means3D), mv(means2D), mv(sh), mv(colors_precomp), mv(opacities), mv(scales),
                                     mv(rotations), mv(cov3Ds_precomp), s)


class GaussianRasterizer(torch.nn.Module):

    def __init__(self, raster_settings: GaussianRasterizationSettings):
        super().__init__()
        self.raster_settings = raster_settings

    def mark_visible(self, positions):
        with torch.no_grad():
            s = self.raster_settings
            return _capi.mark_visible(positions.contiguous(), s.viewmatrix.contiguous(), s.projmatrix.contiguous())

    def forward(self, means3D, means2D, opacities, shs: Optional[torch.Tensor] = None,
                colors_precomp: Optional[torch.Tensor] = None, scales: Optional[torch.Tensor] = None,
                rotations: Optional[torch.Tensor] = None, cov3D_precomp: Optional[torch.Tensor] = None):
        if (shs is None) == (colors_precomp is None):
            raise ValueError("Please provide exactly one of either SHs or precomputed colors!")
        if ((scales is not None or rotations is not None) and cov3D_precomp is not None) or \
                (scales is None and rotations is None and cov3D_precomp is None):
            raise ValueError("Please provide exactly one of either scale/rotation pair or precomputed 3D covariance!")
        dev = means3D.device
        shs = _empty(dev) if shs is None else shs
        colors_precomp = _empty(dev) if colors_precomp is None else colors_precomp
        scales = _empty(dev) if scales is None else scales
        rotations = _empty(dev) if rotations is None else rotations
        cov3D_precomp = _empty(dev) if cov3D_precomp is None else cov3D_precomp
        return rasterize_gaussians(means3D, means2D, shs, colors_precomp, opacities, scales, rotations, cov3D_precomp,
                                   self.raster_settings)
```

Before: 1216 Mpixels/s.

## Drop conic/colour gradient buffers and stage Gaussian-backward outputs through LDS

New measurement: 1192 Mpixels/s. -2.0%, worse.

```diff
diff --git a/gs-livm_amd/_capi.py b/gs-livm_amd/_capi.py
--- a/gs-livm_amd/_capi.py
+++ b/gs-livm_amd/_capi.py
@@ -234,7 +234,7 @@
 def rasterize_backward(background, means3D, radii, colors, scales, rotations, scale_modifier, cov3D_precomp,
                        viewmatrix, projmatrix, tan_fovx, tan_fovy, dL_dout_color, dL_dout_acc, sh, degree, campos,
                        geomBuffer, R, binningBuffer, imageBuffer, debug=False, return_conic=False, want_cov3D=True,
-                       grad_depth=None):
+                       grad_depth=None, want_colors=True):
     dev = means3D.device
     P = int(means3D.size(0))
     H, W = int(dL_dout_color.size(1)), int(dL_dout_color.size(2))
@@ -243,8 +243,10 @@
     mk = torch.zeros if P == 0 else torch.empty
     dL_dmeans3D = mk((P, 3), **f32)
     dL_dmeans2D = mk((P, 3), **f32)
-    dL_dcolors = mk((P, 3), **f32)
-    dL_dconic = mk((P, 2, 2), **f32)
+    if not want_colors and colors is not None and colors.numel() != 0:
+        raise ValueError("want_colors=False with precomputed colours: dL_dcolors is their gradient")
+    dL_dcolors = mk((P, 3), **f32) if want_colors else None
+    dL_dconic = mk((P, 2, 2), **f32) if return_conic else None
     dL_dopacity = mk((P, 1), **f32)
     dL_dcov3D = mk((P, 6), **f32) if want_cov3D else None
     dL_dsh = mk((P, M, 3), **f32)
diff --git a/gs-livm_amd/csrc/api.hip b/gs-livm_amd/csrc/api.hip
--- a/gs-livm_amd/csrc/api.hip
+++ b/gs-livm_amd/csrc/api.hip
@@ -1188,8 +1188,10 @@
   if (!geom_buffer || !binning_buffer || !image_buffer) return fail(GSR_ERR_INVALID_ARGUMENT, "null state blob");
   if (!means3D || !background || !viewmatrix || !projmatrix || !campos || !dL_dpix || !dL_dacc)
     return fail(GSR_ERR_INVALID_ARGUMENT, "null required input");
-  if (!dL_dmean2D || !dL_dconic || !dL_dopacity || !dL_dcolor || !dL_dmean3D || (!dL_dcov3D && cov3D_precomp) ||
-      !dL_dscale || !dL_drot || (M > 0 && !dL_dsh))
+  if (!dL_dcolor && colors_precomp)
+    return fail(GSR_ERR_INVALID_ARGUMENT, "null dL_dcolor with colors_precomp given: it is an output of the caller's graph");
+  if (!dL_dmean2D || !dL_dopacity || !dL_dmean3D || (!dL_dcov3D && cov3D_precomp) || !dL_dscale || !dL_drot ||
+      (M > 0 && !dL_dsh))
     return fail(GSR_ERR_INVALID_ARGUMENT, "null gradient output");
   if (with_depth && !dL_ddepth) return fail(GSR_ERR_INVALID_ARGUMENT, "null dL_ddepth");
   if (with_depth && !dL_ddepths) return fail(GSR_ERR_INVALID_ARGUMENT, "null dL_ddepths");
@@ -1206,8 +1208,8 @@
     const unsigned notes = frame_notes(image_buffer);
     STAGE(launch_blend_backward(fp, g, b, im, background, dL_dpix, dL_dacc, dL_ddepth, (notes & NOTE_ORDER) != 0u,
                                 stream));
-    STAGE(launch_gather_records(fp, g, b, dL_dmean2D, dL_dconic, dL_dopacity, dL_dcolor, dL_ddepths,
-                                (notes & NOTE_SPLIT) != 0u, stream));
+    STAGE(launch_gather_records(fp, g, b, dL_dmean2D, dL_dconic ? dL_dconic : dL_drot, dL_dopacity,
+                                dL_dcolor ? dL_dcolor : dL_dscale, dL_ddepths, (notes & NOTE_SPLIT) != 0u, stream));
   }
   STAGE(launch_gaussian_backward(fp, g, b, radii, means3D, scales, rotations, colors_precomp ? nullptr : shs,
                                  cov3D_precomp, viewmatrix, projmatrix, campos, colors_precomp != nullptr, dL_dmean2D,
diff --git a/gs-livm_amd/csrc/preprocess.hip b/gs-livm_amd/csrc/preprocess.hip
--- a/gs-livm_amd/csrc/preprocess.hip
+++ b/gs-livm_amd/csrc/preprocess.hip
@@ -144,20 +144,20 @@
   }
 }
 
-__device__ __forceinline__ void listed_rows_to_lds(float* lds, const float* __restrict__ src, const uint32_t* list,
+__device__ __forceinline__ void listed_rows_to_lds(float* lds, const float* __restrict__ src, const uint16_t* list,
                                                    const int nlist, const int C) {
   const int S = sh_row_stride(C);
   if ((C & 3) == 0 && (reinterpret_cast<uintptr_t>(src) & 15u) == 0) {
     const int C4 = C >> 2;
     for (int k = threadIdx.x; k < nlist * C4; k += PRE_BLOCK) {
-      const int r = (int)list[k / C4], c4 = k % C4;
+      const int r = (int)(list[k / C4] & 0xFFu), c4 = k % C4;
       const float4 v = reinterpret_cast<const float4*>(src + (size_t)r * C)[c4];
       float* d = lds + r * S + 4 * c4;
       d[0] = v.x; d[1] = v.y; d[2] = v.z; d[3] = v.w;
     }
   } else {
     for (int k = threadIdx.x; k < nlist * C; k += PRE_BLOCK) {
-      const int r = (int)list[k / C], c = k % C;
+      const int r = (int)(list[k / C] & 0xFFu), c = k % C;
       lds[r * S + c] = src[(size_t)r * C + c];
     }
   }
@@ -1292,53 +1292,21 @@
 
 template <bool DEPTH>
 __device__ __forceinline__ void gaussian_backward_one(
-    const int idx, float* row,
-    const FrameParams& fp, GeomState& g, const int* __restrict__ radii, const float* __restrict__ means3D, const float* __restrict__ scales,
+    const int idx, const bool rec, const float* sh, float* gs,
+    const FrameParams& fp, GeomState& g, const float* __restrict__ means3D, const float* __restrict__ scales,
     const float* __restrict__ rotations, const float* __restrict__ shs, const float* __restrict__ cov3D_precomp,
     const float* __restrict__ V, const float* __restrict__ Pm, const float* __restrict__ campos,
-    const int colors_are_precomp, float* dL_dmean2D, float* dL_dconic, float* dL_dopacity, float* dL_dcolor,
-    float* __restrict__ dL_dmean3D,
-    float* __restrict__ dL_dcov3D, float* __restrict__ dL_dsh, float* __restrict__ dL_dscale,
-    float* __restrict__ dL_drot, float* dL_ddepths, const bool skip_recordless) {
-  const int rad_in = radii[idx];
-  const uint8_t touched_in = g.touched[idx];
-  const bool vis = rad_in > 0;
+    const int colors_are_precomp, const float* mean2D_in, const float* conic_in, const float* color_in,
+    float* dL_dcov3D, const float* dL_ddepths, float* o_mean2D, float* o_mean3D, float* o_scale, float* o_rot) {
   const int M = fp.M;
-  float* gs = row ? row : dL_dsh + (size_t)idx * fp.M * 3;
-  if (idx == 0) g.total[2] = 0u;
-  const bool was_touched = touched_in != 0;
-  if (was_touched) g.touched[idx] = 0;
-  const bool rec = vis && was_touched;
-  if (!rec && (skip_recordless || !vis)) {
-    dL_dmean2D[3 * idx] = 0.f; dL_dmean2D[3 * idx + 1] = 0.f; dL_dmean2D[3 * idx + 2] = 0.f;
-    dL_dconic[4 * idx] = 0.f; dL_dconic[4 * idx + 1] = 0.f; dL_dconic[4 * idx + 2] = 0.f; dL_dconic[4 * idx + 3] = 0.f;
-    dL_dopacity[idx] = 0.f;
-    if constexpr (DEPTH) dL_ddepths[idx] = 0.f;
-    dL_dcolor[3 * idx] = 0.f; dL_dcolor[3 * idx + 1] = 0.f; dL_dcolor[3 * idx + 2] = 0.f;
-    dL_dmean3D[3 * idx] = 0.f; dL_dmean3D[3 * idx + 1] = 0.f; dL_dmean3D[3 * idx + 2] = 0.f;
-    if (dL_dcov3D) {
-#pragma unroll
-      for (int k = 0; k < 6; k++) dL_dcov3D[6 * (size_t)idx + k] = 0.f;
-    }
-    for (int k = 0; k < 3 * M; k++) gs[k] = 0.f;
-    dL_dscale[3 * idx] = 0.f; dL_dscale[3 * idx + 1] = 0.f; dL_dscale[3 * idx + 2] = 0.f;
-    dL_drot[4 * idx] = 0.f; dL_drot[4 * idx + 1] = 0.f; dL_drot[4 * idx + 2] = 0.f; dL_drot[4 * idx + 3] = 0.f;
-    return;
-  }
-  const float gcol0 = rec ? dL_dcolor[3 * idx] : 0.f, gcol1 = rec ? dL_dcolor[3 * idx + 1] : 0.f, gcol2 = rec ? dL_dcolor[3 * idx + 2] : 0.f;
-  const float gmx = rec ? dL_dmean2D[3 * idx] : 0.f, gmy = rec ? dL_dmean2D[3 * idx + 1] : 0.f;
-  const float gca = rec ? dL_dconic[4 * idx] : 0.f, gcb = rec ? dL_dconic[4 * idx + 1] : 0.f, gcc = rec ? dL_dconic[4 * idx + 3] : 0.f;
+  const float gcol0 = rec ? color_in[3 * idx] : 0.f, gcol1 = rec ? color_in[3 * idx + 1] : 0.f, gcol2 = rec ? color_in[3 * idx + 2] : 0.f;
+  const float gmx = rec ? mean2D_in[3 * idx] : 0.f, gmy = rec ? mean2D_in[3 * idx + 1] : 0.f;
+  const float gca = rec ? conic_in[4 * idx] : 0.f, gcb = rec ? conic_in[4 * idx + 1] : 0.f, gcc = rec ? conic_in[4 * idx + 3] : 0.f;
   float gz = 0.f;
   if constexpr (DEPTH) {
     if (rec) gz = dL_ddepths[idx];
-    else dL_ddepths[idx] = 0.f;
-  }
-  if (!rec) {
-    dL_dmean2D[3 * idx] = 0.f; dL_dmean2D[3 * idx + 1] = 0.f;
-    dL_dconic[4 * idx] = 0.f; dL_dconic[4 * idx + 1] = 0.f; dL_dconic[4 * idx + 3] = 0.f;
-    dL_dopacity[idx] = 0.f;
-    dL_dcolor[3 * idx] = 0.f; dL_dcolor[3 * idx + 1] = 0.f; dL_dcolor[3 * idx + 2] = 0.f;
-  }
+  }
+  o_mean2D[0] = gmx; o_mean2D[1] = gmy; o_mean2D[2] = 0.f;
   const float mx = means3D[3 * idx], my = means3D[3 * idx + 1], mz = means3D[3 * idx + 2];
   const uint8_t clamped_in = g.clamped[idx];
   float4 q_in = make_float4(0.f, 0.f, 0.f, 0.f);
@@ -1354,9 +1322,6 @@
   } else {
     cov3d_from_scale_rot(fp.scale_modifier * sc_in[0], fp.scale_modifier * sc_in[1], fp.scale_modifier * sc_in[2], q_in, c6);
   }
-  const float* sh = row ? row : shs + (size_t)idx * fp.M * 3;
-  dL_dmean2D[3 * idx + 2] = 0.f;
-  dL_dconic[4 * idx + 2] = 0.f;
   const Ewa e = ewa_project(mx, my, mz, fp, c6, V);
   const float limx = 1.3f * fp.tan_fovx, limy = 1.3f * fp.tan_fovy;
   const float xmul = (e.txtz < -limx || e.txtz > limx) ? 0.f : 1.f;
@@ -1483,7 +1448,7 @@
   if constexpr (DEPTH) {
     dm0 += V[2] * gz; dm1 += V[6] * gz; dm2 += V[10] * gz;
   }
-  dL_dmean3D[3 * idx] = dm0; dL_dmean3D[3 * idx + 1] = dm1; dL_dmean3D[3 * idx + 2] = dm2;
+  o_mean3D[0] = dm0; o_mean3D[1] = dm1; o_mean3D[2] = dm2;
   if (scales) {
     const float4 q = q_in;
     const float r = q.x, x = q.y, y = q.z, z = q.w;
@@ -1507,7 +1472,7 @@
     float ds[3];
 #pragma unroll
     for (int k = 0; k < 3; k++) ds[k] = R[0][k] * dMt[k][0] + R[1][k] * dMt[k][1] + R[2][k] * dMt[k][2];
-    dL_dscale[3 * idx] = ds[0]; dL_dscale[3 * idx + 1] = ds[1]; dL_dscale[3 * idx + 2] = ds[2];
+    o_scale[0] = ds[0]; o_scale[1] = ds[1]; o_scale[2] = ds[2];
 #pragma unroll
     for (int k = 0; k < 3; k++)
 #pragma unroll
@@ -1521,10 +1486,46 @@
     const float dq3 = 2 * r * (Dm(0, 1) - Dm(1, 0)) + 2 * x * (Dm(2, 0) + Dm(0, 2)) + 2 * y * (Dm(1, 2) + Dm(2, 1)) -
                       4 * z * (Dm(1, 1) + Dm(0, 0));
 #undef Dm
-    dL_drot[4 * idx] = dq0; dL_drot[4 * idx + 1] = dq1; dL_drot[4 * idx + 2] = dq2; dL_drot[4 * idx + 3] = dq3;
+    o_rot[0] = dq0; o_rot[1] = dq1; o_rot[2] = dq2; o_rot[3] = dq3;
   } else {
-    dL_dscale[3 * idx] = 0.f; dL_dscale[3 * idx + 1] = 0.f; dL_dscale[3 * idx + 2] = 0.f;
-    dL_drot[4 * idx] = 0.f; dL_drot[4 * idx + 1] = 0.f; dL_drot[4 * idx + 2] = 0.f; dL_drot[4 * idx + 3] = 0.f;
+    o_scale[0] = 0.f; o_scale[1] = 0.f; o_scale[2] = 0.f;
+    o_rot[0] = 0.f; o_rot[1] = 0.f; o_rot[2] = 0.f; o_rot[3] = 0.f;
+  }
+}
+
+constexpr int GBWD_IMAGE_WORDS = 13, GBWD_IMAGE_WORDS_SH = 16;
+static inline size_t gbwd_lds_bytes(size_t stage, bool sh_in_image) {
+  return (size_t)PRE_BLOCK * (sh_in_image ? GBWD_IMAGE_WORDS_SH : GBWD_IMAGE_WORDS) * sizeof(float) + stage + 32 +
+         2 * PRE_BLOCK + 16;
+}
+
+__device__ __forceinline__ bool gb_row_bit(const unsigned long long* m, const int r) { return (m[r >> 6] >> (r & 63)) & 1ull; }
+
+template <int W>
+__device__ __forceinline__ void gb_store_span(float* dst, const float* img, const int n, const unsigned long long* m,
+                                              const bool from_image, const int t, const int nt) {
+  int done = 0;
+  if ((reinterpret_cast<uintptr_t>(dst) & 15u) == 0) {
+    const int n4 = n >> 2;
+    for (int j = t; j < n4; j += nt) {
+      const int e = 4 * j;
+      const bool b0 = gb_row_bit(m, e / W), b1 = gb_row_bit(m, (e + 1) / W), b2 = gb_row_bit(m, (e + 2) / W),
+                 b3 = gb_row_bit(m, (e + 3) / W);
+      if ((b0 || b1 || b2 || b3) != from_image) continue;
+      float4 v = make_float4(0.f, 0.f, 0.f, 0.f);
+      if (from_image) {
+        if (b0) v.x = img[e];
+        if (b1) v.y = img[e + 1];
+        if (b2) v.z = img[e + 2];
+        if (b3) v.w = img[e + 3];
+      }
+      reinterpret_cast<float4*>(dst)[j] = v;
+    }
+    done = n4 << 2;
+  }
+  for (int e = done + t; e < n; e += nt) {
+    if (gb_row_bit(m, e / W) != from_image) continue;
+    dst[e] = from_image ? img[e] : 0.f;
   }
 }
 
@@ -1534,31 +1535,98 @@
     const float* __restrict__ rotations, const float* __restrict__ shs, const float* __restrict__ cov3D_precomp,
     const float* __restrict__ V, const float* __restrict__ Pm, const float* __restrict__ campos,
     const int colors_are_precomp, float* dL_dmean2D, float* dL_dconic, float* dL_dopacity, float* dL_dcolor,
-    float* __restrict__ dL_dmean3D,
-    float* __restrict__ dL_dcov3D, float* __restrict__ dL_dsh, float* __restrict__ dL_dscale,
-    float* __restrict__ dL_drot, const bool skip_recordless, float* dL_ddepths) {
-  extern __shared__ float sh_rows[];
-  __shared__ uint32_t s_rec[PRE_BLOCK];
-  __shared__ uint32_t s_nrec;
-  const int row0 = blockIdx.x * PRE_BLOCK, idx = row0 + threadIdx.x;
-  const int C = fp.M * 3, nrows = min(PRE_BLOCK, fp.P - row0);
+    float* dL_dmean3D, float* dL_dcov3D, float* dL_dsh, float* dL_dscale, float* dL_drot, const bool skip_recordless,
+    float* dL_ddepths) {
+  extern __shared__ __attribute__((aligned(16))) float gb_lds[];
+  const int tid = threadIdx.x, lane = tid & 63, w = tid >> 6, P = fp.P, C = fp.M * 3;
+  const int row0 = blockIdx.x * PRE_BLOCK, idx = row0 + tid, nrows = min(PRE_BLOCK, P - row0);
+  const bool sh_in_image = !STAGED && shs && fp.M == 1;
+  float* const i_mean2D = gb_lds;
+  float* const i_mean3D = gb_lds + 3 * PRE_BLOCK;
+  float* const i_scale = gb_lds + 6 * PRE_BLOCK;
+  float* const i_rot = gb_lds + 9 * PRE_BLOCK;
+  float* const i_sh = gb_lds + GBWD_IMAGE_WORDS * PRE_BLOCK;
+  float* const sh_rows = gb_lds + (sh_in_image ? GBWD_IMAGE_WORDS_SH : GBWD_IMAGE_WORDS) * PRE_BLOCK;
+  unsigned long long* const s_mask = reinterpret_cast<unsigned long long*>(sh_rows + (STAGED ? PRE_BLOCK * sh_row_stride(C) : 0));
+  uint16_t* const s_rec = reinterpret_cast<uint16_t*>(s_mask + PRE_BLOCK / 64);
+  uint32_t* const s_nrec = reinterpret_cast<uint32_t*>(s_rec + PRE_BLOCK);
+  const float* const conic_in = dL_dconic ? dL_dconic : dL_drot;
+  const float* const color_in = dL_dcolor ? dL_dcolor : dL_dscale;
+  if (tid == 0) *s_nrec = 0u;
+  if (idx == 0) g.total[2] = 0u;
+  int rad_in = 0;
+  uint8_t touched_in = 0;
+  if (idx < P) {
+    rad_in = radii[idx];
+    touched_in = g.touched[idx];
+  }
+  __syncthreads();
+  const bool vis = rad_in > 0, was_touched = touched_in != 0;
+  const bool rec = vis && was_touched;
+  const bool chain = idx < P && (rec || (vis && !skip_recordless));
+  if (idx < P) {
+    if (was_touched) g.touched[idx] = 0;
+    if (!rec) {
+      dL_dopacity[idx] = 0.f;
+      if constexpr (DEPTH) dL_ddepths[idx] = 0.f;
+      if (dL_dconic) { dL_dconic[4 * idx] = 0.f; dL_dconic[4 * idx + 1] = 0.f; dL_dconic[4 * idx + 2] = 0.f; dL_dconic[4 * idx + 3] = 0.f; }
+      if (dL_dcolor) { dL_dcolor[3 * idx] = 0.f; dL_dcolor[3 * idx + 1] = 0.f; dL_dcolor[3 * idx + 2] = 0.f; }
+    } else if (dL_dconic) {
+      dL_dconic[4 * idx + 2] = 0.f;
+    }
+    if (!chain) {
+      if (dL_dcov3D) {
+#pragma unroll
+        for (int k = 0; k < 6; k++) dL_dcov3D[6 * (size_t)idx + k] = 0.f;
+      }
+      if (!STAGED && !sh_in_image)
+        for (int k = 0; k < C; k++) dL_dsh[(size_t)idx * C + k] = 0.f;
+    }
+  }
+  if (STAGED && !chain)
+    for (int k = 0; k < C; k++) sh_rows[tid * sh_row_stride(C) + k] = 0.f;
+  const unsigned long long chain_wave = __ballot(chain);
+  if (lane == 0) s_mask[w] = chain_wave;
+  if (chain) s_rec[atomicAdd(s_nrec, 1u)] = (uint16_t)(tid | (rec ? 0x100 : 0));
+  __syncthreads();
+  const int nrec = (int)*s_nrec;
+  gb_store_span<3>(dL_dmean2D + (size_t)row0 * 3, i_mean2D, nrows * 3, s_mask, false, tid, PRE_BLOCK);
+  gb_store_span<3>(dL_dmean3D + (size_t)row0 * 3, i_mean3D, nrows * 3, s_mask, false, tid, PRE_BLOCK);
+  gb_store_span<3>(dL_dscale + (size_t)row0 * 3, i_scale, nrows * 3, s_mask, false, tid, PRE_BLOCK);
+  gb_store_span<4>(dL_drot + (size_t)row0 * 4, i_rot, nrows * 4, s_mask, false, tid, PRE_BLOCK);
+  if (sh_in_image) gb_store_span<3>(dL_dsh + (size_t)row0 * 3, i_sh, nrows * 3, s_mask, false, tid, PRE_BLOCK);
+  if (nrec == 0) {
+    if (STAGED) lds_to_rows(dL_dsh + (size_t)row0 * C, sh_rows, nrows, C);
+    return;
+  }
+  const bool one_wave = !STAGED && nrec <= 64;
+  if (one_wave && w != 0) return;
   if (STAGED) {
-    if (threadIdx.x == 0) s_nrec = 0u;
+    listed_rows_to_lds(sh_rows, shs + (size_t)row0 * C, s_rec, nrec, C);
     __syncthreads();
-    if (idx < fp.P && radii[idx] > 0 && (g.touched[idx] != 0 || !skip_recordless)) s_rec[atomicAdd(&s_nrec, 1u)] = threadIdx.x;
+  }
+  if (tid < nrec) {
+    const int entry = s_rec[tid], r = entry & 0xFF, ridx = row0 + r;
+    float* const lrow = sh_rows + r * sh_row_stride(C);
+    gaussian_backward_one<DEPTH>(ridx, (entry & 0x100) != 0, STAGED ? lrow : shs + (size_t)ridx * C,
+                                 STAGED ? lrow : sh_in_image ? i_sh + 3 * r : dL_dsh + (size_t)ridx * C, fp, g, means3D,
+                                 scales, rotations, shs, cov3D_precomp, V, Pm, campos, colors_are_precomp, dL_dmean2D,
+                                 conic_in, color_in, dL_dcov3D, dL_ddepths, i_mean2D + 3 * r, i_mean3D + 3 * r,
+                                 i_scale + 3 * r, i_rot + 4 * r);
+  }
+  if (one_wave) {
+    __builtin_amdgcn_fence(__ATOMIC_ACQ_REL, "wavefront");
+    __builtin_amdgcn_wave_barrier();
+  } else {
     __syncthreads();
-    listed_rows_to_lds(sh_rows, shs + (size_t)row0 * C, s_rec, (int)s_nrec, C);
-    __syncthreads();
-  }
-  if (idx < fp.P)
-    gaussian_backward_one<DEPTH>(idx, STAGED ? sh_rows + threadIdx.x * sh_row_stride(C) : nullptr, fp, g, radii, means3D,
-                                 scales, rotations, shs, cov3D_precomp, V, Pm, campos, colors_are_precomp, dL_dmean2D,
-                                 dL_dconic, dL_dopacity, dL_dcolor, dL_dmean3D, dL_dcov3D, dL_dsh, dL_dscale, dL_drot,
-                                 dL_ddepths, skip_recordless);
-  if (STAGED) {
-    __syncthreads();
-    lds_to_rows(dL_dsh + (size_t)row0 * C, sh_rows, nrows, C);
-  }
+  }
+  const int t = one_wave ? lane : tid, nt = one_wave ? 64 : PRE_BLOCK;
+  gb_store_span<3>(dL_dmean2D + (size_t)row0 * 3, i_mean2D, nrows * 3, s_mask, true, t, nt);
+  gb_store_span<3>(dL_dmean3D + (size_t)row0 * 3, i_mean3D, nrows * 3, s_mask, true, t, nt);
+  gb_store_span<3>(dL_dscale + (size_t)row0 * 3, i_scale, nrows * 3, s_mask, true, t, nt);
+  gb_store_span<4>(dL_drot + (size_t)row0 * 4, i_rot, nrows * 4, s_mask, true, t, nt);
+  if (sh_in_image) gb_store_span<3>(dL_dsh + (size_t)row0 * 3, i_sh, nrows * 3, s_mask, true, t, nt);
+  if (STAGED) lds_to_rows(dL_dsh + (size_t)row0 * C, sh_rows, nrows, C);
 }
 
 __global__ __launch_bounds__(PRE_BLOCK) void k_mark_visible(int P, const float* __restrict__ means3D,
@@ -1718,24 +1786,26 @@
   const int nb = (fp.P + PRE_BLOCK - 1) / PRE_BLOCK;
   ProfScope ps_k_gaussian_bwd(K_GAUSSIAN_BWD, s);
   const size_t stage = (shs && !colors_precomp) ? sh_stage_bytes(fp.M) : 0;
+  const size_t lds = gbwd_lds_bytes(stage, !stage && shs && fp.M == 1);
   const bool skip_recordless = !env().gbwd_all;
+  const dim3 grid(nb);
   if (dL_ddepths) {
     if (stage)
-      hipLaunchKernelGGL((k_gaussian_backward<true, true>), dim3(nb), dim3(PRE_BLOCK), stage, s, fp, g, radii, means3D,
+      hipLaunchKernelGGL((k_gaussian_backward<true, true>), grid, dim3(PRE_BLOCK), lds, s, fp, g, radii, means3D,
                          scales, rotations, shs, cov3D_precomp, view, proj, campos, 0, dL_dmean2D, dL_dconic, dL_dopacity,
                          dL_dcolor, dL_dmean3D, dL_dcov3D, dL_dsh, dL_dscale, dL_drot, skip_recordless, dL_ddepths);
     else
-      hipLaunchKernelGGL((k_gaussian_backward<false, true>), dim3(nb), dim3(PRE_BLOCK), 0, s, fp, g, radii, means3D,
+      hipLaunchKernelGGL((k_gaussian_backward<false, true>), grid, dim3(PRE_BLOCK), lds, s, fp, g, radii, means3D,
                          scales, rotations, shs, cov3D_precomp, view, proj, campos, colors_precomp ? 1 : 0, dL_dmean2D,
                          dL_dconic, dL_dopacity, dL_dcolor, dL_dmean3D, dL_dcov3D, dL_dsh, dL_dscale, dL_drot,
                          skip_recordless, dL_ddepths);
   } else if (stage)
-    hipLaunchKernelGGL(k_gaussian_backward<true>, dim3(nb), dim3(PRE_BLOCK), stage, s, fp, g, radii,
+    hipLaunchKernelGGL(k_gaussian_backward<true>, grid, dim3(PRE_BLOCK), lds, s, fp, g, radii,
                        means3D, scales, rotations, shs, cov3D_precomp, view, proj, campos, 0,
                        dL_dmean2D, dL_dconic, dL_dopacity, dL_dcolor, dL_dmean3D, dL_dcov3D, dL_dsh, dL_dscale, dL_drot,
                        skip_recordless, nullptr);
   else
-    hipLaunchKernelGGL(k_gaussian_backward<false>, dim3(nb), dim3(PRE_BLOCK), 0, s, fp, g, radii,
+    hipLaunchKernelGGL(k_gaussian_backward<false>, grid, dim3(PRE_BLOCK), lds, s, fp, g, radii,
                        means3D, scales, rotations, shs, cov3D_precomp, view, proj, campos, colors_precomp ? 1 : 0,
                        dL_dmean2D, dL_dconic, dL_dopacity, dL_dcolor, dL_dmean3D, dL_dcov3D, dL_dsh, dL_dscale, dL_drot,
                        skip_recordless, nullptr);
diff --git a/gs-livm_amd/csrc/torch_binding.cpp b/gs-livm_amd/csrc/torch_binding.cpp
--- a/gs-livm_amd/csrc/torch_binding.cpp
+++ b/gs-livm_amd/csrc/torch_binding.cpp
@@ -92,7 +92,8 @@
                         const torch::Tensor& dL_dout_color, const torch::Tensor& dL_dout_acc, const torch::Tensor& sh,
                         const int degree, const torch::Tensor& campos, const torch::Tensor& geomBuffer, const int R,
                         const torch::Tensor& binningBuffer, const torch::Tensor& imageBuffer, const bool debug,
-                        const bool want_cov3D, const torch::Tensor& dL_dout_depth = torch::Tensor()) {
+                        const bool want_cov3D, const bool want_colors,
+                        const torch::Tensor& dL_dout_depth = torch::Tensor()) {
   const int P = means3D.size(0);
   const int H = dL_dout_color.size(1);
   const int W = dL_dout_color.size(2);
@@ -102,8 +103,7 @@
   auto mk = [&](std::initializer_list<int64_t> shape) { return P ? torch::empty(shape, o) : torch::zeros(shape, o); };
   torch::Tensor dL_dmeans3D = mk({P, 3});
   torch::Tensor dL_dmeans2D = mk({P, 3});
-  torch::Tensor dL_dcolors = mk({P, 3});
-  torch::Tensor dL_dconic = mk({P, 2, 2});
+  torch::Tensor dL_dcolors = want_colors ? mk({P, 3}) : torch::Tensor();
   torch::Tensor dL_dopacity = mk({P, 1});
   torch::Tensor dL_dcov3D = want_cov3D ? mk({P, 6}) : torch::Tensor();
   torch::Tensor dL_dsh = mk({P, M, 3});
@@ -126,8 +126,8 @@
                                rad.data_ptr<int>(), reinterpret_cast<char*>(geomBuffer.data_ptr()),
                                reinterpret_cast<char*>(binningBuffer.data_ptr()),
                                reinterpret_cast<char*>(imageBuffer.data_ptr()), fptr(dpix), fptr(dacc), fptr(ddep),
-                               dL_dmeans2D.data_ptr<float>(), dL_dconic.data_ptr<float>(),
-                               dL_dopacity.data_ptr<float>(), dL_dcolors.data_ptr<float>(),
+                               dL_dmeans2D.data_ptr<float>(), nullptr, dL_dopacity.data_ptr<float>(),
+                               dL_dcolors.defined() ? dL_dcolors.data_ptr<float>() : nullptr,
                                dL_dmeans3D.data_ptr<float>(),
                                dL_dcov3D.defined() ? dL_dcov3D.data_ptr<float>() : nullptr,
                                M ? dL_dsh.data_ptr<float>() : nullptr, dL_dscales.data_ptr<float>(),
@@ -140,8 +140,8 @@
                        rad.data_ptr<int>(), reinterpret_cast<char*>(geomBuffer.data_ptr()),
                        reinterpret_cast<char*>(binningBuffer.data_ptr()),
                        reinterpret_cast<char*>(imageBuffer.data_ptr()), fptr(dpix), fptr(dacc),
-                       dL_dmeans2D.data_ptr<float>(), dL_dconic.data_ptr<float>(), dL_dopacity.data_ptr<float>(),
-                       dL_dcolors.data_ptr<float>(), dL_dmeans3D.data_ptr<float>(),
+                       dL_dmeans2D.data_ptr<float>(), nullptr, dL_dopacity.data_ptr<float>(),
+                       dL_dcolors.defined() ? dL_dcolors.data_ptr<float>() : nullptr, dL_dmeans3D.data_ptr<float>(),
                        dL_dcov3D.defined() ? dL_dcov3D.data_ptr<float>() : nullptr,
                        M ? dL_dsh.data_ptr<float>() : nullptr, dL_dscales.data_ptr<float>(),
                        dL_drotations.data_ptr<float>(), debug ? 1 : 0, current_stream()),
@@ -164,7 +164,7 @@
   auto [g0, g1, g2, g3, g4, g5, g6, g7, unused] =
       rasterize_backward_impl(background, means3D, radii, colors, scales, rotations, scale_modifier, cov3D_precomp,
                               viewmatrix, projmatrix, tan_fovx, tan_fovy, dL_dout_color, dL_dout_acc, sh, degree, campos,
-                              geomBuffer, R, binningBuffer, imageBuffer, debug, true);
+                              geomBuffer, R, binningBuffer, imageBuffer, debug, true, true);
   (void)unused;
   return std::make_tuple(g0, g1, g2, g3, g4, g5, g6, g7);
 }
@@ -184,7 +184,7 @@
   if (!dL_dout_depth.defined()) AT_ERROR("dL_dout_depth must be defined");
   return rasterize_backward_impl(background, means3D, radii, colors, scales, rotations, scale_modifier, cov3D_precomp,
                                  viewmatrix, projmatrix, tan_fovx, tan_fovy, dL_dout_color, dL_dout_acc, sh, degree, campos,
-                                 geomBuffer, R, binningBuffer, imageBuffer, debug, true, dL_dout_depth);
+                                 geomBuffer, R, binningBuffer, imageBuffer, debug, true, true, dL_dout_depth);
 }
 
 torch::Tensor markVisible(torch::Tensor& means3D, torch::Tensor& viewmatrix, torch::Tensor& projmatrix) {
@@ -258,7 +258,7 @@
           ctx->saved_data["tanfovx"].to<double>(), ctx->saved_data["tanfovy"].to<double>(), grad_out_color, grad_acc,
           sh, ctx->saved_data["sh_degree"].to<int>(), ctx->saved_data["camera_center"].to<torch::Tensor>(),
           geomBuffer, num_rendered, binningBuffer, imgBuffer, false, cov3Ds_precomp.numel() != 0,
-          grad_depth);
+          colors_precomp.numel() != 0, grad_depth);
   (void)grad_depths;
   auto opt = [](const torch::Tensor& g, const torch::Tensor& x) { return x.numel() ? g : torch::Tensor(); };
   return {grad_means3D,
diff --git a/gs-livm_amd/rasterizer.py b/gs-livm_amd/rasterizer.py
--- a/gs-livm_amd/rasterizer.py
+++ b/gs-livm_amd/rasterizer.py
@@ -55,7 +55,8 @@
             rotations.contiguous(), s.scale_modifier, cov3Ds_precomp.contiguous(), s.viewmatrix.contiguous(),
             s.projmatrix.contiguous(), s.tanfovx, s.tanfovy, grad_color, grad_acc, sh.contiguous(), s.sh_degree,
             s.camera_center.contiguous(), geom, ctx.num_rendered, binning, img, False,
-            want_cov3D=cov3Ds_precomp.numel() != 0, grad_depth=grad_depth)[:8]
+            want_cov3D=cov3Ds_precomp.numel() != 0, grad_depth=grad_depth,
+            want_colors=colors_precomp.numel() != 0)[:8]
         none_if_empty = lambda g, x: g if x.numel() else None
         return (g_means3D, g_means2D, none_if_empty(g_sh, sh), none_if_empty(g_colors, colors_precomp), g_opac,
                 none_if_empty(g_scales, scales), none_if_empty(g_rot, rotations),
```
